# jgaeddert/liquid-usrp

Measured on AMD Instinct MI355X. Metric: complex Msamples/s through multichannelrx, higher is better.
Workload: dtype f32

## Files before the change

include/mcrx_hip.h:

```cpp
#ifndef MCRX_HIP_H
#define MCRX_HIP_H

#include <stddef.h>
#include <stdint.h>

#ifdef __cplusplus
extern "C" {
#endif

#define MCRX_OK          0
#define MCRX_EINVAL     -1
#define MCRX_ENOMEM     -2
#define MCRX_EHIP       -3
#define MCRX_EUNSUPP    -4
#define MCRX_EOVERFLOW  -5
#define MCRX_EBUSY      -6

#define MCRX_TILE 16

typedef struct mcrx_hip_s *mcrx_hip_t;

typedef struct {
    uint32_t struct_size;
    uint32_t max_payload_len;
    uint32_t max_frames;
    uint32_t payload_soft;
    uint32_t slab_blocks;
    uint32_t channel_first;
    uint32_t channel_count;
    uint32_t batch_samples;
    uint32_t single_channel;
    uint32_t serial;
    uint32_t chunk_blocks;
    uint32_t defer_samples;
    uint32_t front_end;
    uint32_t skip_framesyms;
    uint32_t worker_build;
    uint32_t acquisition;
    uint32_t scout_build;
    uint32_t conv_scratch;
    uint32_t input_format;
} mcrx_hip_config;

typedef struct {
    uint32_t channel;
    int32_t  header_valid;
    int32_t  payload_valid;
    uint32_t payload_len;
    uint8_t  header[8];
    float    evm, rssi, cfo;
    uint32_t mod_scheme, mod_bps, check, fec0, fec1;
    uint32_t num_framesyms;
    uint64_t end_sample;
    const uint8_t *payload;
    const float   *framesyms;
} mcrx_frame;

int  mcrx_hip_create(mcrx_hip_t *out, unsigned num_channels, unsigned M, unsigned cp_len,
                     unsigned taper_len, const unsigned char *p, const mcrx_hip_config *cfg);
int  mcrx_hip_destroy(mcrx_hip_t q);
int  mcrx_hip_reset(mcrx_hip_t q);
#define MCRX_POSITION_MAX (1ll << 48)
int  mcrx_hip_reset_at(mcrx_hip_t q, uint64_t chan_position);
unsigned mcrx_hip_num_channels(mcrx_hip_t q);

int  mcrx_hip_execute_host(mcrx_hip_t q, const float *iq, size_t nsamples);
int  mcrx_hip_execute_device(mcrx_hip_t q, const void *d_iq, size_t nsamples, void *stream);
int  mcrx_hip_execute_host_sc16(mcrx_hip_t q, const int16_t *iq, size_t nsamples);
int  mcrx_hip_execute_device_sc16(mcrx_hip_t q, const void *d_iq, size_t nsamples, void *stream);
unsigned mcrx_hip_input_format(mcrx_hip_t q);

int  mcrx_hip_flush(mcrx_hip_t q);
int  mcrx_hip_poll(mcrx_hip_t q);
int  mcrx_hip_discard(mcrx_hip_t q);
int  mcrx_hip_stream_wait(mcrx_hip_t q, void *stream);
uint64_t mcrx_hip_launches(mcrx_hip_t q);
unsigned mcrx_hip_history_tiles(mcrx_hip_t q);
int  mcrx_hip_stream_wait_launch(mcrx_hip_t q, uint64_t launch, void *stream);
int  mcrx_hip_spec_stats(mcrx_hip_t q, uint64_t *walked, uint64_t *adopted, int reset);
int  mcrx_hip_viterbi_stats(mcrx_hip_t q, uint64_t *frames, uint64_t *forward_repeats, uint64_t *traceback_repeats, int reset);
size_t mcrx_hip_frames_pending(mcrx_hip_t q);
int  mcrx_hip_next_frame(mcrx_hip_t q, mcrx_frame *out);
int  mcrx_hip_drain_count(mcrx_hip_t q, uint64_t *frames, uint64_t *valid, uint64_t *payload_bytes);
uint64_t mcrx_hip_frames_dropped(mcrx_hip_t q);

typedef struct {
    uint32_t struct_size;
    uint32_t nfft;
    uint32_t window;
} mcrx_hip_monitor_config;
int  mcrx_hip_monitor_enable(mcrx_hip_t q, const mcrx_hip_monitor_config *cfg);
int  mcrx_hip_monitor_disable(mcrx_hip_t q);
int  mcrx_hip_monitor_read(mcrx_hip_t q, double *level, float *peak, double *psd, uint64_t *nseg, uint64_t *nsamp, int reset);
unsigned mcrx_hip_monitor_nfft(mcrx_hip_t q);

int  mcrx_hip_channelize(mcrx_hip_t q, const void *d_iq, size_t nblocks, uint64_t first_sample,
                         const void *d_halo, void *d_out, unsigned groups, void *stream);
int  mcrx_hip_sync(mcrx_hip_t q, const void *d_chan, uint64_t first_sample, size_t nsamples, void *stream);

int  mcrx_hip_restart(mcrx_hip_t q, void *stream);

int  mcrx_hip_get_taps(mcrx_hip_t q, float *h, size_t n);
uint32_t mcrx_hip_nco_step(mcrx_hip_t q);
unsigned mcrx_hip_history_blocks(mcrx_hip_t q);
int  mcrx_hip_kernel_time_ms(mcrx_hip_t q, float *channelizer_ms, float *sync_ms);
#define MCRX_NKERNELS 5
int  mcrx_hip_kernel_stats(mcrx_hip_t q, double ms_total[MCRX_NKERNELS], uint64_t launches[MCRX_NKERNELS], int reset);
int  mcrx_hip_kernel_timing(mcrx_hip_t q, int on);

const char *mcrx_hip_last_error(void);

int  mcrx_hip_device(mcrx_hip_t q);
int  mcrx_hip_selftest_device_table(void);

typedef struct msresamp_hip_s *msresamp_hip_t;
int    msresamp_hip_create(msresamp_hip_t *out, float rate, float As);
int    msresamp_hip_destroy(msresamp_hip_t q);
int    msresamp_hip_reset(msresamp_hip_t q);
int    msresamp_hip_reset_at(msresamp_hip_t q, uint64_t input_position);
float  msresamp_hip_get_delay(msresamp_hip_t q);
size_t msresamp_hip_max_output(msresamp_hip_t q, size_t nin);
int    msresamp_hip_execute_device(msresamp_hip_t q, const void *d_in, size_t nin, void *d_out,
                                   size_t out_cap, size_t *nout, void *stream);
int      msresamp_hip_set_input_format(msresamp_hip_t q, unsigned format);
unsigned msresamp_hip_input_format(msresamp_hip_t q);
int      msresamp_hip_execute_device_sc16(msresamp_hip_t q, const void *d_in, size_t nin, void *d_out,
                                          size_t out_cap, size_t *nout, void *stream);
int      msresamp_hip_set_output_format(msresamp_hip_t q, unsigned format);
unsigned msresamp_hip_output_format(msresamp_hip_t q);
int      msresamp_hip_set_output_gain(msresamp_hip_t q, float gain);
float    msresamp_hip_output_gain(msresamp_hip_t q);
int      msresamp_hip_clipped(msresamp_hip_t q, uint64_t *samples, int reset);
int      msresamp_hip_time_first_stage(msresamp_hip_t q, int enable);
int      msresamp_hip_first_stage_ms(msresamp_hip_t q, float *ms);
const char *msresamp_hip_last_error(void);

typedef struct mcrx_hip_pfb2_s *mcrx_hip_pfb2_t;
int    mcrx_hip_pfb2_create(mcrx_hip_pfb2_t *out, unsigned num_channels, unsigned m, float As);
int    mcrx_hip_pfb2_destroy(mcrx_hip_pfb2_t q);
int    mcrx_hip_pfb2_get_taps(mcrx_hip_pfb2_t q, float *h, size_t n);
int    mcrx_hip_pfb2_analyze(mcrx_hip_pfb2_t q, const void *d_x, size_t lead_samples, size_t nsteps,
                             uint64_t first_step, void *d_out, void *stream);
const char *mcrx_hip_pfb2_last_error(void);

typedef struct mcrx_hip_pipeline_s *mcrx_hip_pipeline_t;
int      mcrx_hip_pipeline_unique_id(void *id128);
int      mcrx_hip_pipeline_create(mcrx_hip_pipeline_t *out, mcrx_hip_t rx, int rank, int world, const void *unique_id128,
                                  size_t sub_blocks, unsigned nbuf );
#define MCRX_STREAM_READY ((void *)(intptr_t)-1)
int      mcrx_hip_pipeline_push(mcrx_hip_pipeline_t p, const void *d_iq_sub, const void *d_halo, void *after_stream);
int      mcrx_hip_pipeline_push_host(mcrx_hip_pipeline_t p, const float *iq_with_halo);
int      mcrx_hip_pipeline_host_buffer(mcrx_hip_pipeline_t p, float **buf, size_t *nsamples);
int      mcrx_hip_pipeline_reset(mcrx_hip_pipeline_t p, int64_t extra_samples);
int      mcrx_hip_pipeline_comm_count(mcrx_hip_pipeline_t p);
int      mcrx_hip_pipeline_wait(mcrx_hip_pipeline_t p);
int      mcrx_hip_pipeline_time_exchange(mcrx_hip_pipeline_t p, int on);
int      mcrx_hip_pipeline_exchange_ms(mcrx_hip_pipeline_t p, double *total_ms, uint64_t *rounds, int reset);
uint64_t mcrx_hip_pipeline_bytes_sent_per_round(mcrx_hip_pipeline_t p);
int      mcrx_hip_pipeline_destroy(mcrx_hip_pipeline_t p);
const char *mcrx_hip_pipeline_last_error(void);

typedef struct mctx_hip_s *mctx_hip_t;
int    mctx_hip_create(mctx_hip_t *out, unsigned num_channels, unsigned M, unsigned cp_len,
                       unsigned taper_len, const unsigned char *p);
int    mctx_hip_destroy(mctx_hip_t q);
int      mctx_hip_set_output_format(mctx_hip_t q, unsigned format);
unsigned mctx_hip_output_format(mctx_hip_t q);
int      mctx_hip_clipped(mctx_hip_t q, uint64_t *samples, int reset);
int      mctx_hip_selftest_quantise(const float *in, int16_t *out, size_t n);
size_t mctx_hip_blocks_for(mctx_hip_t q, unsigned frames_per_channel, unsigned payload_len,
                           int mod, int fec0, int fec1);
int    mctx_hip_generate(mctx_hip_t q, void *d_iq, size_t nblocks, unsigned frames_per_channel,
                         unsigned payload_len, int mod, int fec0, int fec1, float gain, uint32_t seed,
                         uint8_t *hdr, uint8_t *pay, void *stream);
int    mctx_hip_generate_ragged(mctx_hip_t q, void *d_iq, size_t nblocks, unsigned max_frames, unsigned len_lo, unsigned len_hi,
                                unsigned gap_max, unsigned long_every, unsigned long_max, int mod, int fec0, int fec1,
                                float gain, uint32_t seed, uint32_t *count, uint8_t *hdr, uint32_t *len, uint8_t *pay,
                                uint64_t *start, void *stream);
typedef struct mctx_hip_traffic_s *mctx_hip_traffic_t;
int    mctx_hip_traffic_create(mctx_hip_t q, mctx_hip_traffic_t *out, unsigned ch_first, unsigned ch_count,
                               unsigned frames_per_channel, unsigned payload_len, int mod, int fec0, int fec1,
                               uint32_t seed, uint8_t *hdr, uint8_t *pay, void *stream);
int    mctx_hip_traffic_destroy(mctx_hip_traffic_t t);
int    mctx_hip_traffic_tiles(mctx_hip_traffic_t t, long long first_block, size_t nblocks, void *d_tiles, void *stream);
int    mctx_hip_synthesize_tiles(mctx_hip_t q, const void *d_tiles, unsigned groups, long long first_block,
                                 size_t nblocks, size_t lead_blocks, size_t keep_blocks, float gain, void *d_iq,
                                 void *stream);
size_t mctx_hip_frame_len(mctx_hip_t q, unsigned payload_len, int mod, int fec0, int fec1);
int    mctx_hip_frame(mctx_hip_t q, const uint8_t *header8, const uint8_t *payload, unsigned payload_len,
                      int mod, int fec0, int fec1, float gain, float *out, size_t out_cap_samples);
int    mctx_hip_stream_begin(mctx_hip_t q, unsigned max_payload_len);
int    mctx_hip_stream_ready(mctx_hip_t q, unsigned channel);
int    mctx_hip_stream_update(mctx_hip_t q, unsigned channel, const uint8_t *header8, const uint8_t *payload,
                              unsigned payload_len, int mod, int fec0, int fec1);
// ... 187 lines not shown
```

liquid-usrp_amd/__init__.py:

```python
import ctypes as C
import math
import os
import subprocess

import numpy as np

_HERE = os.path.dirname(os.path.abspath(__file__))
_LIBPATH = os.environ.get("MCRX_LIB") or os.path.join(_HERE, "lib", "libmcrx_hip.so")

MCRX_OK, MCRX_EINVAL, MCRX_ENOMEM, MCRX_EHIP, MCRX_EUNSUPP, MCRX_EOVERFLOW, MCRX_EBUSY = 0, -1, -2, -3, -4, -5, -6
TILE = 16
POSITION_MAX = 1 << 48
TX_TILE = 8

LIQUID_CRC_NONE, LIQUID_CRC_32 = 1, 6
LIQUID_FEC_NONE, LIQUID_FEC_HAMMING128, LIQUID_FEC_GOLAY2412, LIQUID_FEC_CONV_V27 = 1, 6, 7, 11
LIQUID_FEC_REP3, LIQUID_FEC_REP5, LIQUID_FEC_HAMMING74, LIQUID_FEC_HAMMING84 = 2, 3, 4, 5
LIQUID_MODEM_QAM16, LIQUID_MODEM_QAM64, LIQUID_MODEM_BPSK, LIQUID_MODEM_QPSK = 27, 29, 39, 40


def build(force=False):
    src = os.path.join(_HERE, "csrc")
    deps = [os.path.join(src, f) for f in os.listdir(src) if f.endswith((".hip", ".h", ".hpp"))]
    deps.append(os.path.join(_HERE, "..", "include", "mcrx_hip.h"))
    stale = (not os.path.exists(_LIBPATH)) or any(os.path.getmtime(d) > os.path.getmtime(_LIBPATH) for d in deps)
    if force or stale:
        subprocess.check_call(["make", "-C", src, "-s", "-j4"])
    return _LIBPATH


class Config(C.Structure):
    _fields_ = [("struct_size", C.c_uint32), ("max_payload_len", C.c_uint32), ("max_frames", C.c_uint32),
                ("payload_soft", C.c_uint32), ("slab_blocks", C.c_uint32), ("channel_first", C.c_uint32),
                ("channel_count", C.c_uint32), ("batch_samples", C.c_uint32), ("single_channel", C.c_uint32),
                ("serial", C.c_uint32), ("chunk_blocks", C.c_uint32), ("defer_samples", C.c_uint32), ("front_end", C.c_uint32), ("skip_framesyms", C.c_uint32),
                ("worker_build", C.c_uint32), ("acquisition", C.c_uint32), ("scout_build", C.c_uint32), ("conv_scratch", C.c_uint32),
                ("input_format", C.c_uint32)]


INPUT_FORMATS = {"cf32": 0, "sc16": 1}
OUTPUT_FORMATS = {"cf32": 0, "sc16": 1}


class FrameC(C.Structure):
    _fields_ = [("channel", C.c_uint32), ("header_valid", C.c_int32), ("payload_valid", C.c_int32),
                ("payload_len", C.c_uint32), ("header", C.c_uint8 * 8),
                ("evm", C.c_float), ("rssi", C.c_float), ("cfo", C.c_float),
                ("mod_scheme", C.c_uint32), ("mod_bps", C.c_uint32), ("check", C.c_uint32),
                ("fec0", C.c_uint32), ("fec1", C.c_uint32), ("num_framesyms", C.c_uint32),
                ("end_sample", C.c_uint64), ("payload", C.c_void_p), ("framesyms", C.c_void_p)]


_EXPORTS = {
    "mcrx_hip_create": (C.c_int, [C.POINTER(C.c_void_p), C.c_uint, C.c_uint, C.c_uint, C.c_uint, C.c_void_p, C.c_void_p]),
    "mcrx_hip_destroy": (C.c_int, [C.c_void_p]),
    "mcrx_hip_reset": (C.c_int, [C.c_void_p]),
    "mcrx_hip_reset_at": (C.c_int, [C.c_void_p, C.c_uint64]),
    "mcrx_hip_num_channels": (C.c_uint, [C.c_void_p]),
    "mcrx_hip_execute_host": (C.c_int, [C.c_void_p, C.c_void_p, C.c_size_t]),
    "mcrx_hip_execute_device": (C.c_int, [C.c_void_p, C.c_void_p, C.c_size_t, C.c_void_p]),
    "mcrx_hip_execute_host_sc16": (C.c_int, [C.c_void_p, C.c_void_p, C.c_size_t]),
    "mcrx_hip_execute_device_sc16": (C.c_int, [C.c_void_p, C.c_void_p, C.c_size_t, C.c_void_p]),
    "mcrx_hip_input_format": (C.c_uint, [C.c_void_p]),
    "mcrx_hip_flush": (C.c_int, [C.c_void_p]),
    "mcrx_hip_poll": (C.c_int, [C.c_void_p]),
    "mcrx_hip_discard": (C.c_int, [C.c_void_p]),
    "mcrx_hip_stream_wait": (C.c_int, [C.c_void_p, C.c_void_p]),
    "mcrx_hip_launches": (C.c_uint64, [C.c_void_p]),
    "mcrx_hip_history_tiles": (C.c_uint, [C.c_void_p]),
    "mcrx_hip_stream_wait_launch": (C.c_int, [C.c_void_p, C.c_uint64, C.c_void_p]),
    "mcrx_hip_spec_stats": (C.c_int, [C.c_void_p, C.POINTER(C.c_uint64), C.POINTER(C.c_uint64), C.c_int]),
    "mcrx_hip_viterbi_stats": (C.c_int, [C.c_void_p, C.POINTER(C.c_uint64), C.POINTER(C.c_uint64), C.POINTER(C.c_uint64), C.c_int]),
    "mcrx_hip_frames_pending": (C.c_size_t, [C.c_void_p]),
    "mcrx_hip_next_frame": (C.c_int, [C.c_void_p, C.POINTER(FrameC)]),
    "mcrx_hip_drain_count": (C.c_int, [C.c_void_p, C.POINTER(C.c_uint64), C.POINTER(C.c_uint64), C.POINTER(C.c_uint64)]),
    "mcrx_hip_frames_dropped": (C.c_uint64, [C.c_void_p]),
    "mcrx_hip_channelize": (C.c_int, [C.c_void_p, C.c_void_p, C.c_size_t, C.c_uint64, C.c_void_p, C.c_void_p, C.c_uint, C.c_void_p]),
    "mcrx_hip_sync": (C.c_int, [C.c_void_p, C.c_void_p, C.c_uint64, C.c_size_t, C.c_void_p]),
    "mcrx_hip_restart": (C.c_int, [C.c_void_p, C.c_void_p]),
    "mcrx_hip_get_taps": (C.c_int, [C.c_void_p, C.c_void_p, C.c_size_t]),
    "mcrx_hip_nco_step": (C.c_uint32, [C.c_void_p]),
    "mcrx_hip_history_blocks": (C.c_uint, [C.c_void_p]),
    "mcrx_hip_device": (C.c_int, [C.c_void_p]),
    "mcrx_hip_selftest_device_table": (C.c_int, []),
    "mcrx_hip_kernel_time_ms": (C.c_int, [C.c_void_p, C.POINTER(C.c_float), C.POINTER(C.c_float)]),
    "mcrx_hip_kernel_stats": (C.c_int, [C.c_void_p, C.POINTER(C.c_double), C.POINTER(C.c_uint64), C.c_int]),
    "mcrx_hip_kernel_timing": (C.c_int, [C.c_void_p, C.c_int]),
    "mcrx_hip_monitor_enable": (C.c_int, [C.c_void_p, C.c_void_p]),
    "mcrx_hip_monitor_disable": (C.c_int, [C.c_void_p]),
    "mcrx_hip_monitor_read": (C.c_int, [C.c_void_p, C.c_void_p, C.c_void_p, C.c_void_p, C.POINTER(C.c_uint64), C.POINTER(C.c_uint64), C.c_int]),
    "mcrx_hip_monitor_nfft": (C.c_uint, [C.c_void_p]),
    "mcrx_hip_last_error": (C.c_char_p, []),
    "msresamp_hip_create": (C.c_int, [C.POINTER(C.c_void_p), C.c_float, C.c_float]),
    "msresamp_hip_destroy": (C.c_int, [C.c_void_p]),
    "msresamp_hip_reset": (C.c_int, [C.c_void_p]),
    "msresamp_hip_reset_at": (C.c_int, [C.c_void_p, C.c_uint64]),
    "msresamp_hip_get_delay": (C.c_float, [C.c_void_p]),
    "msresamp_hip_max_output": (C.c_size_t, [C.c_void_p, C.c_size_t]),
    "msresamp_hip_execute_device": (C.c_int, [C.c_void_p, C.c_void_p, C.c_size_t, C.c_void_p, C.c_size_t,
                                              C.POINTER(C.c_size_t), C.c_void_p]),
    "msresamp_hip_set_input_format": (C.c_int, [C.c_void_p, C.c_uint]),
    "msresamp_hip_input_format": (C.c_uint, [C.c_void_p]),
    "msresamp_hip_execute_device_sc16": (C.c_int, [C.c_void_p, C.c_void_p, C.c_size_t, C.c_void_p, C.c_size_t,
                                                   C.POINTER(C.c_size_t), C.c_void_p]),
    "msresamp_hip_set_output_format": (C.c_int, [C.c_void_p, C.c_uint]),
    "msresamp_hip_output_format": (C.c_uint, [C.c_void_p]),
    "msresamp_hip_set_output_gain": (C.c_int, [C.c_void_p, C.c_float]),
    "msresamp_hip_output_gain": (C.c_float, [C.c_void_p]),
    "msresamp_hip_clipped": (C.c_int, [C.c_void_p, C.POINTER(C.c_uint64), C.c_int]),
    "msresamp_hip_time_first_stage": (C.c_int, [C.c_void_p, C.c_int]),
    "msresamp_hip_first_stage_ms": (C.c_int, [C.c_void_p, C.POINTER(C.c_float)]),
    "msresamp_hip_last_error": (C.c_char_p, []),
    "mcrx_hip_pfb2_create": (C.c_int, [C.POINTER(C.c_void_p), C.c_uint, C.c_uint, C.c_float]),
    "mcrx_hip_pfb2_destroy": (C.c_int, [C.c_void_p]),
    "mcrx_hip_pfb2_get_taps": (C.c_int, [C.c_void_p, C.c_void_p, C.c_size_t]),
    "mcrx_hip_pfb2_analyze": (C.c_int, [C.c_void_p, C.c_void_p, C.c_size_t, C.c_size_t, C.c_uint64, C.c_void_p, C.c_void_p]),
    "mcrx_hip_pfb2_last_error": (C.c_char_p, []),
    "mcrx_hip_pipeline_unique_id": (C.c_int, [C.c_void_p]),
    "mcrx_hip_pipeline_create": (C.c_int, [C.POINTER(C.c_void_p), C.c_void_p, C.c_int, C.c_int, C.c_void_p, C.c_size_t, C.c_uint]),
    "mcrx_hip_pipeline_push": (C.c_int, [C.c_void_p, C.c_void_p, C.c_void_p, C.c_void_p]),
    "mcrx_hip_pipeline_push_host": (C.c_int, [C.c_void_p, C.c_void_p]),
    "mcrx_hip_pipeline_wait": (C.c_int, [C.c_void_p]),
    "mcrx_hip_pipeline_host_buffer": (C.c_int, [C.c_void_p, C.POINTER(C.c_void_p), C.POINTER(C.c_size_t)]),
    "mcrx_hip_pipeline_reset": (C.c_int, [C.c_void_p, C.c_int64]),
    "mcrx_hip_pipeline_comm_count": (C.c_int, [C.c_void_p]),
    "mcrx_hip_pipeline_time_exchange": (C.c_int, [C.c_void_p, C.c_int]),
    "mcrx_hip_pipeline_exchange_ms": (C.c_int, [C.c_void_p, C.POINTER(C.c_double), C.POINTER(C.c_uint64), C.c_int]),
    "mcrx_hip_pipeline_bytes_sent_per_round": (C.c_uint64, [C.c_void_p]),
    "mcrx_hip_pipeline_destroy": (C.c_int, [C.c_void_p]),
    "mcrx_hip_pipeline_last_error": (C.c_char_p, []),
    "mctx_hip_create": (C.c_int, [C.POINTER(C.c_void_p), C.c_uint, C.c_uint, C.c_uint, C.c_uint, C.c_void_p]),
    "mctx_hip_destroy": (C.c_int, [C.c_void_p]),
    "mctx_hip_set_output_format": (C.c_int, [C.c_void_p, C.c_uint]),
    "mctx_hip_output_format": (C.c_uint, [C.c_void_p]),
    "mctx_hip_clipped": (C.c_int, [C.c_void_p, C.POINTER(C.c_uint64), C.c_int]),
    "mctx_hip_selftest_quantise": (C.c_int, [C.c_void_p, C.c_void_p, C.c_size_t]),
    "mctx_hip_blocks_for": (C.c_size_t, [C.c_void_p, C.c_uint, C.c_uint, C.c_int, C.c_int, C.c_int]),
    "mctx_hip_generate_ragged": (C.c_int, [C.c_void_p, C.c_void_p, C.c_size_t, C.c_uint, C.c_uint, C.c_uint, C.c_uint, C.c_uint, C.c_uint,
                                           C.c_int, C.c_int, C.c_int, C.c_float, C.c_uint32, C.c_void_p, C.c_void_p, C.c_void_p,
                                           C.c_void_p, C.c_void_p, C.c_void_p]),
    "mctx_hip_generate": (C.c_int, [C.c_void_p, C.c_void_p, C.c_size_t, C.c_uint, C.c_uint, C.c_int, C.c_int, C.c_int,
                                    C.c_float, C.c_uint32, C.c_void_p, C.c_void_p, C.c_void_p]),
    "mctx_hip_traffic_create": (C.c_int, [C.c_void_p, C.POINTER(C.c_void_p), C.c_uint, C.c_uint, C.c_uint, C.c_uint, C.c_int, C.c_int,
                                          C.c_int, C.c_uint32, C.c_void_p, C.c_void_p, C.c_void_p]),
    "mctx_hip_traffic_destroy": (C.c_int, [C.c_void_p]),
    "mctx_hip_traffic_tiles": (C.c_int, [C.c_void_p, C.c_longlong, C.c_size_t, C.c_void_p, C.c_void_p]),
    "mctx_hip_synthesize_tiles": (C.c_int, [C.c_void_p, C.c_void_p, C.c_uint, C.c_longlong, C.c_size_t, C.c_size_t, C.c_size_t,
                                            C.c_float, C.c_void_p, C.c_void_p]),
    "mctx_hip_frame_len": (C.c_size_t, [C.c_void_p, C.c_uint, C.c_int, C.c_int, C.c_int]),
    "mctx_hip_frame": (C.c_int, [C.c_void_p, C.c_void_p, C.c_void_p, C.c_uint, C.c_int, C.c_int, C.c_int, C.c_float,
                                 C.c_void_p, C.c_size_t]),
    "mctx_hip_stream_begin": (C.c_int, [C.c_void_p, C.c_uint]),
    "mctx_hip_stream_ready": (C.c_int, [C.c_void_p, C.c_uint]),
    "mctx_hip_stream_update": (C.c_int, [C.c_void_p, C.c_uint, C.c_void_p, C.c_void_p, C.c_uint, C.c_int, C.c_int, C.c_int]),
    "mctx_hip_stream_generate": (C.c_int, [C.c_void_p, C.c_void_p]),
    "mctx_hip_stream_reset": (C.c_int, [C.c_void_p]),
    "mctx_hip_last_error": (C.c_char_p, []),
    "mcrx_hip_chanemu_create": (C.c_int, [C.POINTER(C.c_void_p), C.c_void_p]),
    "mcrx_hip_chanemu_destroy": (C.c_int, [C.c_void_p]),
    "mcrx_hip_chanemu_reset": (C.c_int, [C.c_void_p]),
    "mcrx_hip_chanemu_reset_at": (C.c_int, [C.c_void_p, C.c_uint64]),
    "mcrx_hip_chanemu_position": (C.c_uint64, [C.c_void_p]),
    "mcrx_hip_chanemu_output_format": (C.c_uint, [C.c_void_p]),
    "mcrx_hip_chanemu_execute_device": (C.c_int, [C.c_void_p, C.c_void_p, C.c_size_t, C.c_void_p, C.c_void_p]),
    "mcrx_hip_chanemu_clipped": (C.c_int, [C.c_void_p, C.POINTER(C.c_uint64), C.c_int]),
    "mcrx_hip_chanemu_selftest_words": (C.c_int, [C.c_uint64, C.c_uint64, C.POINTER(C.c_uint32)]),
    "mcrx_hip_chanemu_last_error": (C.c_char_p, []),
    "mcrx_hip_chanfade_set": (C.c_int, [C.c_void_p, C.c_void_p]),
    "mcrx_hip_chanfade_on": (C.c_int, [C.c_void_p]),
    "mcrx_hip_chanfade_gains": (C.c_int, [C.c_void_p, C.c_uint64, C.c_uint32, C.c_void_p, C.c_void_p]),
    "mcrx_hip_chanfade_selftest": (C.c_int, [C.c_void_p, C.c_uint, C.POINTER(C.c_int64), C.POINTER(C.c_uint32), C.POINTER(C.c_float)]),
    "mcrx_hip_userchan_create": (C.c_int, [C.POINTER(C.c_void_p), C.c_uint, C.c_void_p, C.c_size_t]),
    "mcrx_hip_userchan_destroy": (C.c_int, [C.c_void_p]),
    "mcrx_hip_userchan_num_channels": (C.c_uint, [C.c_void_p]),
    "mcrx_hip_userchan_lead_blocks": (C.c_uint, [C.c_void_p]),
    "mcrx_hip_userchan_apply_tiles": (C.c_int, [C.c_void_p, C.c_void_p, C.c_longlong, C.c_size_t, C.c_size_t, C.c_void_p, C.c_void_p]),
    "mcrx_hip_userchan_last_error": (C.c_char_p, []),
    "mcrx_hip_userfade_set": (C.c_int, [C.c_void_p, C.c_void_p, C.c_void_p]),
    "mcrx_hip_userfade_on": (C.c_int, [C.c_void_p]),
    "mcrx_hip_userfade_selftest": (C.c_int, [C.c_void_p, C.c_void_p, C.c_uint, C.POINTER(C.c_int64), C.POINTER(C.c_uint32),
                                             C.POINTER(C.c_float)]),
    "mcrx_hip_userfade_gains": (C.c_int, [C.c_void_p, C.c_longlong, C.c_uint32, C.c_void_p, C.c_void_p]),
    "mcrx_hip_userclock_set": (C.c_int, [C.c_void_p, C.c_void_p, C.c_void_p]),
    "mcrx_hip_userclock_on": (C.c_int, [C.c_void_p]),
    "mcrx_hip_userclock_lead_blocks": (C.c_uint, [C.c_void_p]),
    "mcrx_hip_userclock_selftest": (C.c_int, [C.c_void_p, C.c_void_p, C.c_longlong, C.POINTER(C.c_int64), C.POINTER(C.c_float)]),
    "mcrx_hip_userclock_table": (C.c_int, [C.POINTER(C.c_float)]),
    "mcrx_hip_userclock_apply_tiles": (C.c_int, [C.c_void_p, C.c_void_p, C.c_longlong, C.c_size_t, C.c_size_t, C.c_void_p, C.c_void_p]),
    "mcrx_hip_rfchain_create": (C.c_int, [C.POINTER(C.c_void_p), C.c_void_p]),
    "mcrx_hip_rfchain_destroy": (C.c_int, [C.c_void_p]),
# ... 12 lines not shown
    "mcrx_hip_rfcal_update": (C.c_int, [C.c_void_p, C.c_void_p]),
    "mcrx_hip_rfcal_hold": (C.c_int, [C.c_void_p, C.c_int]),
    "mcrx_hip_rfcal_set": (C.c_int, [C.c_void_p, C.c_float, C.c_float, C.c_float, C.c_float, C.c_void_p]),
    "mcrx_hip_rfcal_read": (C.c_int, [C.c_void_p, C.c_void_p, C.c_void_p]),
    "mcrx_hip_rfcal_clipped": (C.c_int, [C.c_void_p, C.POINTER(C.c_uint64), C.c_int]),
    "mcrx_hip_rfcal_selftest": (C.c_int, [C.c_void_p, C.c_uint64, C.c_uint64, C.POINTER(C.c_uint64), C.POINTER(C.c_uint32), C.c_size_t,
                                          C.POINTER(C.c_uint64)]),
    "mcrx_hip_rfcal_last_error": (C.c_char_p, []),
    "mcrx_hip_cfr_create": (C.c_int, [C.POINTER(C.c_void_p), C.c_void_p]),
    "mcrx_hip_cfr_destroy": (C.c_int, [C.c_void_p]),
    "mcrx_hip_cfr_halo": (C.c_uint, [C.c_void_p]),
    "mcrx_hip_cfr_output_format": (C.c_uint, [C.c_void_p]),
    "mcrx_hip_cfr_execute_device": (C.c_int, [C.c_void_p, C.c_void_p, C.c_size_t, C.c_void_p, C.c_void_p]),
    "mcrx_hip_cfr_clipped": (C.c_int, [C.c_void_p, C.POINTER(C.c_uint64), C.c_int]),
    "mcrx_hip_cfr_stats": (C.c_int, [C.c_void_p, C.POINTER(C.c_uint64), C.POINTER(C.c_float), C.c_int]),
    "mcrx_hip_cfr_design": (C.c_int, [C.c_uint32, C.c_double, C.c_double, C.POINTER(C.c_float)]),
    "mcrx_hip_cfr_last_error": (C.c_char_p, []),
}

_lib = None


def exported_symbols():
    return sorted(_EXPORTS)


def lib():
    global _lib
    if _lib is None:
        if not os.path.exists(_LIBPATH):
            raise RuntimeError("libmcrx_hip.so is not built (run __graft_entry__.build()); "
                               "liquid_usrp_amd has no CPU fallback")
        try:
            import torch
        except ImportError:
            pass
        L = C.CDLL(_LIBPATH)
        for name, (res, args) in _EXPORTS.items():
            fn = getattr(L, name)
            fn.restype, fn.argtypes = res, args
        _lib = L
    return _lib


class McrxError(RuntimeError):
    pass


def _check(rc, allow=()):
    if rc != MCRX_OK and rc not in allow:
        msg = lib().mcrx_hip_last_error()
        raise McrxError("mcrx_hip error %d: %s" % (rc, msg.decode() if msg else ""))
    return rc


def _raise_rc(rc, name, last_error, einval_is_value_error=True):
    if rc == MCRX_OK:
        return
    msg = last_error()
    msg = msg.decode() if msg else ""
    if rc == MCRX_EINVAL and einval_is_value_error:
        raise ValueError(msg)
    raise McrxError("%s failed (%d): %s" % (name, rc, msg))


def _format_code(value, table, what):
    code = table.get(value) if isinstance(value, str) else next((c for c in table.values() if c == value), None)
    if code is None:
        raise ValueError("%s must be one of %s or %s, not %r" % (what, sorted(table), sorted(table.values()), value))
    return code


def _empty_samples(n, fmt, device):
    import torch
    if fmt == OUTPUT_FORMATS["sc16"]:
        return torch.empty((n, 2), dtype=torch.int16, device=device)
    return torch.empty(n, dtype=torch.complex64, device=device)


def _sc16_device_samples(x, what):
    import torch
    if x.dtype != torch.int16:
        raise TypeError("this %s takes int16 device tensors (interleaved re, im), not %s" % (what, x.dtype))
    if not x.is_contiguous():
        raise ValueError("device samples must be contiguous")
    if x.numel() % 2:
        raise ValueError("an sc16 buffer holds (re, im) pairs: odd number of int16")
    return int(x.numel()) // 2


class Frame(object):
    __slots__ = ("channel", "header", "header_valid", "payload", "payload_valid", "evm", "rssi", "cfo",
                 "framesyms", "mod_scheme", "mod_bps", "check", "fec0", "fec1", "end_sample")

    def __repr__(self):
        return "Frame(ch=%d hv=%d pv=%d len=%d evm=%.2f end=%d)" % (
            self.channel, self.header_valid, self.payload_valid, len(self.payload), self.evm, self.end_sample)


def _dptr(t):
    if t is None:
        return None
    if isinstance(t, int):
        return C.c_void_p(t)
    return C.c_void_p(t.data_ptr())


def _stream_ptr(stream):
    if stream is None:
        return None
    if isinstance(stream, int):
        return C.c_void_p(stream)
    return C.c_void_p(stream.cuda_stream)


class MonitorConfig(C.Structure):
    _fields_ = [("struct_size", C.c_uint32), ("nfft", C.c_uint32), ("window", C.c_uint32)]


MONITOR_WINDOWS = {"rect": 0, "rectangular": 0, "hann": 1, "hamming": 2}


def monitor_omega(num_channels, nfft, channel, kp):
    N = float(num_channels)
    return np.pi * (np.asarray(channel, np.float64) - (N - 1.0) / 2.0) / N + 2.0 * np.pi * np.asarray(kp, np.float64) / (nfft * 2.0 * N)


class MonitorReading(object):

    def __init__(self, level, peak, psd, nseg, nsamp, num_channels, channel_first=0):
        self.level, self.peak, self.psd = np.asarray(level, np.float64), np.asarray(peak, np.float32), np.asarray(psd, np.float64)
        self.nseg, self.nsamp, self.N, self.channel_first = int(nseg), int(nsamp), int(num_channels), int(channel_first)

    def level_db(self):
        return 10.0 * np.log10(np.maximum(self.level, 1e-300))

    def occupied(self, threshold_db):
        return self.level_db() > threshold_db

    def wideband(self):
        nch, nfft = self.psd.shape
        kp = np.arange(-nfft // 2 + 1, nfft // 2 + 1)
        row = self.psd[:, kp % nfft].reshape(-1)
        ch = self.channel_first + np.arange(nch)
        return row, monitor_omega(self.N, nfft, ch[:, None], kp[None, :]).reshape(-1)


class multichannelrx(object):

    def __init__(self, num_channels, M, cp_len, taper_len, p=None, userdata=None, callback=None, **cfg):
        self._h = C.c_void_p()
        self.N, self.K, self.M, self.cp = num_channels, 2 * num_channels, M, cp_len
        parr = None if p is None else np.ascontiguousarray(np.frombuffer(bytes(bytearray(p)), np.uint8))
        c = Config()
        c.struct_size = C.sizeof(Config)
        c.payload_soft = 1
        for k, v in cfg.items():
            setattr(c, k, _format_code(v, INPUT_FORMATS, "input_format") if k == "input_format" else v)
        rc = lib().mcrx_hip_create(C.byref(self._h), num_channels, M, cp_len, taper_len,
                                   None if parr is None else parr.ctypes.data, C.addressof(c))
        if rc != MCRX_OK:
            self._h = C.c_void_p()
            _raise_rc(rc, "mcrx_hip_create", lib().mcrx_hip_last_error)
        self.userdata = list(userdata) if userdata is not None else [None] * num_channels
        self.callback = list(callback) if callback is not None else [None] * num_channels
        self.frames = []
        self.channel_first = int(c.channel_first)
        self.nch = int(c.channel_count) if c.channel_count else num_channels - self.channel_first
        self.input_format = int(c.input_format)

    def GetNumChannels(self):
        return self.N

    def Execute(self, x, num_samples=None, stream=None):
        sc16 = self.input_format == INPUT_FORMATS["sc16"]
        if hasattr(x, "is_cuda") and x.is_cuda:
            import torch
            if sc16:
                n = _sc16_device_samples(x, "receiver")
                n = n if num_samples is None else int(num_samples)
                _check(lib().mcrx_hip_execute_device_sc16(self._h, _dptr(x), n, _stream_ptr(stream)))
                return
            if x.dtype == torch.int16:
                raise TypeError("int16 samples need a receiver made with input_format=\"sc16\"")
            n = int(x.numel()) if num_samples is None else int(num_samples)
            _check(lib().mcrx_hip_execute_device(self._h, _dptr(x), n, _stream_ptr(stream)))
            return
        if sc16:
            a = np.asarray(x)
            if a.dtype != np.int16:
                raise TypeError("this receiver takes int16 samples (interleaved re, im), not %s" % a.dtype)
            a = np.ascontiguousarray(a)
            if a.size % 2:
                raise ValueError("an sc16 buffer holds (re, im) pairs: odd number of int16")
            n = a.size // 2 if num_samples is None else int(num_samples)
            _check(lib().mcrx_hip_execute_host_sc16(self._h, a.ctypes.data, n), allow=(MCRX_EOVERFLOW,))
            self._deliver(flush=False)
            return
        if getattr(x, "dtype", None) == np.int16:
            raise TypeError("int16 samples need a receiver made with input_format=\"sc16\"")
        a = np.ascontiguousarray(x, np.complex64)
        n = a.size if num_samples is None else int(num_samples)
        _check(lib().mcrx_hip_execute_host(self._h, a.ctypes.data, n), allow=(MCRX_EOVERFLOW,))
        self._deliver(flush=False)

    def Reset(self):
        _check(lib().mcrx_hip_reset(self._h))
        self._deliver(flush=False)

    def reset_at(self, pos):
        rc = lib().mcrx_hip_reset_at(self._h, int(pos))
        if rc == MCRX_EINVAL:
            raise ValueError(lib().mcrx_hip_last_error().decode())
        _check(rc)
        self._deliver(flush=False)

    def Flush(self):
        rc = lib().mcrx_hip_flush(self._h)
        _check(rc, allow=(MCRX_EOVERFLOW,))
        self._deliver(flush=False)
        return rc

    def Poll(self, deliver=True):
        rc = lib().mcrx_hip_poll(self._h)
        _check(rc, allow=(MCRX_EOVERFLOW,))
        if deliver:
            self._deliver(flush=False)
        return rc

    def Discard(self):
        _check(lib().mcrx_hip_discard(self._h))

    def frames_pending(self):
        return int(lib().mcrx_hip_frames_pending(self._h))

    def drain_count(self):
        n, ok, nb = C.c_uint64(0), C.c_uint64(0), C.c_uint64(0)
        _check(lib().mcrx_hip_drain_count(self._h, C.byref(n), C.byref(ok), C.byref(nb)))
        return int(n.value), int(ok.value), int(nb.value)

    def stream_wait(self, stream=None, launch=None):
        if launch is None:
            _check(lib().mcrx_hip_stream_wait(self._h, _stream_ptr(stream)))
        else:
            _check(lib().mcrx_hip_stream_wait_launch(self._h, launch, _stream_ptr(stream)))

    def spec_stats(self, reset=False):
        a, b = C.c_uint64(0), C.c_uint64(0)
        _check(lib().mcrx_hip_spec_stats(self._h, C.byref(a), C.byref(b), 1 if reset else 0))
        return int(a.value), int(b.value)

    def viterbi_stats(self, reset=False):
        a, b, c = C.c_uint64(0), C.c_uint64(0), C.c_uint64(0)
        _check(lib().mcrx_hip_viterbi_stats(self._h, C.byref(a), C.byref(b), C.byref(c), 1 if reset else 0))
        return int(a.value), int(b.value), int(c.value)

    def _deliver(self, flush):
        f = FrameC()
        while lib().mcrx_hip_next_frame(self._h, C.byref(f)) == 1:
            fr = Frame()
            fr.channel = int(f.channel)
            fr.header = bytes(bytearray(f.header))
            fr.header_valid, fr.payload_valid = int(f.header_valid), int(f.payload_valid)
            fr.payload = C.string_at(f.payload, f.payload_len) if f.payload and f.payload_len else b""
            fr.evm, fr.rssi, fr.cfo = float(f.evm), float(f.rssi), float(f.cfo)
            if f.framesyms and f.num_framesyms:
                buf = (C.c_float * (2 * f.num_framesyms)).from_address(f.framesyms)
                fr.framesyms = np.frombuffer(buf, np.float32).copy().view(np.complex64)
            else:
                fr.framesyms = np.zeros(0, np.complex64)
            fr.mod_scheme, fr.mod_bps = int(f.mod_scheme), int(f.mod_bps)
            fr.check, fr.fec0, fr.fec1 = int(f.check), int(f.fec0), int(f.fec1)
            fr.end_sample = int(f.end_sample)
            self.frames.append(fr)
            cb = self.callback[fr.channel] if fr.channel < len(self.callback) else None
            if cb is not None:
                cb(fr.header, fr.header_valid, fr.payload, len(fr.payload), fr.payload_valid, fr,
                   self.userdata[fr.channel])

    def taps(self):
        h = np.zeros(14 * self.K, np.float32)
        _check(lib().mcrx_hip_get_taps(self._h, h.ctypes.data, h.size))
        return h

    def nco_step(self):
        return int(lib().mcrx_hip_nco_step(self._h))

    def history_blocks(self):
        return int(lib().mcrx_hip_history_blocks(self._h))

    def channelize(self, d_iq, nblocks, first_sample, d_out, groups=1, d_halo=None, stream=None):
        _check(lib().mcrx_hip_channelize(self._h, _dptr(d_iq), nblocks, first_sample, _dptr(d_halo),
                                         _dptr(d_out), groups, _stream_ptr(stream)))

    def sync(self, d_chan, first_sample, nsamples, stream=None):
        _check(lib().mcrx_hip_sync(self._h, _dptr(d_chan), first_sample & 0xFFFFFFFFFFFFFFFF, nsamples, _stream_ptr(stream)))
        return int(lib().mcrx_hip_launches(self._h)) - 1

    @property
    def hist_tiles(self):
        return int(lib().mcrx_hip_history_tiles(self._h))

    def restart(self, stream=None):
        _check(lib().mcrx_hip_restart(self._h, _stream_ptr(stream)))

    def kernel_time_ms(self):
        a, b = C.c_float(0), C.c_float(0)
        _check(lib().mcrx_hip_kernel_time_ms(self._h, C.byref(a), C.byref(b)))
# ... 1261 lines not shown
```

liquid-usrp_amd/csrc/kernels.h:

```cpp
#pragma once
#include <hip/hip_runtime.h>
#include <stdint.h>
#include "acq_shared.h"
#include "sync_plan.hpp"

namespace mcrx {

#define MCRX_TILE_S 16
#define MCRX_TILE_SH 4
#define MCRX_HDR_ENC 36
#define MCRX_HDR_DEC 14

struct ChanArgs {
    const void *x;
    const void *halo;
    const float *taps;
    float2 *out;
    uint32_t nblocks;
    uint32_t slab_blocks;
    uint32_t first_sample_lo;
    uint32_t dtheta;
    uint32_t ntiles;
    uint32_t cg;
    uint32_t col_shift;
// ... 5 lines not shown
int channelizer_carries(unsigned K);
uint32_t channelizer_auto_slab(unsigned K, size_t nblocks, unsigned ncu);
hipError_t channelizer_launch(unsigned K, unsigned P, unsigned in_fmt, const ChanArgs &a, hipStream_t st);

#ifndef MCRX_S1_BACKOFF_CORRECTION
#define MCRX_S1_BACKOFF_CORRECTION 0
#endif
#ifndef MCRX_S1_METRIC_G0_NORMALISED
#define MCRX_S1_METRIC_G0_NORMALISED 1
#endif
enum { SY_SEEK = 0, SY_S0A, SY_S0B, SY_S1, SY_RX };
enum { FX_HEADER = 0, FX_PAYLOAD };

struct CodingDev {
    const uint32_t *crc_byte;
    const uint32_t *crc_zadv;
    const uint8_t *qam16_nb;
    const uint8_t *qam64_nb;
};

struct SyncConsts {
    int M, M2, cp, L, backoff, M_pilot, M_data, Nen, M_S0, M_S1;
    int E;
    int log2M;
    float detect_thresh, sync_thresh;
    const uint8_t *sctype;
    const float *S0, *S1;
    const float2 *s0t;
    const float *smk, *smn;
    float2 backoff_rot;
    const float *Pfit;
    const int16_t *data_rank, *pilot_rank, *en_rank;
    const uint8_t *pilot_seq;
    const uint16_t *hdr_map;
    const float2 *dft_tw;
    CodingDev cod;
    uint32_t max_payload_len, max_enc_len, max_syms;
    const uint32_t *crc_pos;
    uint32_t crc_pos_n;
    const uint32_t *il_off;
    const uint16_t *il_map;
    uint32_t il_n;
    int payload_soft;
};

struct ChanState {
    int32_t state; uint32_t timer;
    int64_t cur;
    uint32_t nco_theta_ref, nco_dtheta; int64_t nco_t_ref;
    float g0; float2 s_hat_0;
    uint32_t num_symbols, pilot_count;
    float phi_prime, p1_prime;
    int32_t fstate; uint32_t header_symbol_index, payload_symbol_index;
    float evm_hat, evm;
    uint32_t payload_len, mod_scheme, bps, check, fec0, fec1, enc_len, mod_len;
    int32_t header_valid;
    uint32_t hw[4];
    uint32_t period_hint;
    int64_t last_fresh;
    uint32_t burst_hint;
    uint32_t burst_pad;
};

struct FrameRec {
    uint32_t channel; int32_t header_valid, payload_valid; uint32_t payload_len;
    uint8_t header[8];
    float evm, rssi, cfo;
    uint32_t mod_scheme, mod_bps, check, fec0, fec1, num_framesyms;
    int64_t end_sample;
    uint64_t payload_off, syms_off;
};

struct PayloadJob {
    ChanState s;
    uint32_t ch;
    uint32_t pad;
    uint64_t arena_off;
    uint64_t syms_off;
};

struct SpecSlot {
    int64_t start;
    int64_t t_last;
    int32_t status;
    uint32_t pad;
};

struct SyncArgs {
    SyncConsts c;
    const float2 *chan;
    uint32_t chan_stride, chan_off;
    int64_t buf_first;
    int64_t end;
    uint32_t nch;
    uint32_t ch_first;
    ChanState *st;
    uint8_t *hbits;
    float2 *R;
    uint8_t *soft;
    uint8_t *tmpa, *tmpb;
    float2 *syms;
    FrameRec *rec; uint8_t *arena; uint8_t *sarena;
    uint32_t *nrec;
    unsigned long long *arena_used;
    uint64_t arena_cap, sarena_cap;
    uint32_t max_rec;
    int scout;
    PayloadJob *jobs; uint32_t *njobs; uint32_t max_jobs;
    uint32_t *gen_list;
    uint32_t dec_lds_soft;
    uint32_t *njobs_next;
    float2 *jR;
    uint8_t *jsoft;
    uint8_t *jtmp;
    int debug;
    uint2 *vit_scratch;
    uint32_t vit_rows, vit_waves;
    uint32_t *vit_passes;
    uint32_t *qam_list;
    uint32_t *qam_next;
    uint32_t *live, *live_next;
    uint32_t frames_hint;
    uint32_t live_off;
    uint32_t *list_hint;
    uint32_t grid_hint[3];
    uint32_t payload_lds_pad;
    int seek_burst;
    SpecSlot *spec; float2 *spec_R;
    int64_t *pred; uint32_t *pred_n;
    uint32_t spec_cap;
    uint32_t spec_stride;
    uint32_t nseg;
    uint32_t seg_jobs;
    int no_syms;
    int split_rest;
    int dec_phase;
    int seg_walker;
    int seg_phase;
    int64_t *anchor;
    int64_t *seekst;
    uint32_t *spec_hint;
    uint32_t *walk_hint;
    uint32_t *hint;
    uint32_t enc_hint;
    int round_idx;
    int burst_limit;
    int stop_after_walk;
    int64_t defer_limit;
    int tail_only;
    uint32_t *stats;
    int no_fast;
    int payload_fr, payload_lean, payload_xb;
    uint32_t vit_off;
};
hipError_t sync_launch(const SyncArgs &a, hipStream_t st);
hipError_t sync_launch_tail(const SyncArgs &a, hipStream_t st);
hipError_t ilmap_build_launch(const uint32_t *d_lens, const uint32_t *d_offs, uint32_t nlen, uint8_t *d_lo, uint8_t *d_hi, uint16_t *d_map, hipStream_t st);
hipError_t sync_launch_walk(const SyncArgs &a, hipStream_t st);
hipError_t sync_launch_lean(const SyncArgs &a, hipStream_t st);
int acq_lean_waves(const SyncConsts &c);
hipError_t sync_launch_spec(const SyncArgs &a, hipStream_t st);
hipError_t sync_launch_payload(const SyncArgs &a, SyncStage stage, hipStream_t st);
bool sync_payload_splits(const SyncArgs &a);
hipError_t sync_reset_launch(ChanState *st, uint32_t nch, int64_t cur, float2 *hist0, float2 *hist1, size_t hist_n,
                             uint32_t *nrec, unsigned long long *arena_used, uint32_t *pred_n, hipStream_t stream);

struct MonArgs {
    const float2 *chan;
    uint32_t stride, off, t0, ntiles;
    uint32_t nch, nfft, window;
    uint32_t carry_len, carry_cap;
    const float2 *carry_in; float2 *carry_out;
    uint32_t nsplit;
    double *part_psd, *part_level; float *part_peak;
    double *psd, *level; float *peak;
};
hipError_t monitor_launch(const MonArgs &a, hipStream_t st);

}
```

liquid-usrp_amd/csrc/mcrx_hip.hip:

```cpp
#include "../../include/mcrx_hip.h"
#include "acq_plan.hpp"
#include "config_read.hpp"
#include "design.hpp"
#include "devel.h"
#include "devmath.h"
#include "devscope.hpp"
#include "kernels.h"
#include "rx_plan.hpp"
#include "sc16.hpp"
#include "txcode.hpp"

#include <algorithm>
#include <chrono>
#include <cstdio>
#include <cstdlib>
#include <cstring>
#include <mutex>
#include <string>
#include <vector>

using namespace mcrx;

#define MCRX_GENS 4

static thread_local std::string g_err;
static void set_err(const char *what, hipError_t e, const char *file, int line)
{
    char buf[512];
    snprintf(buf, sizeof(buf), "%s: %s (%s:%d)", what, hipGetErrorString(e), file, line);
    g_err = buf;
}
static int fail(int code, const char *msg) { g_err = msg; return code; }
#define HIPCHK(x) do { hipError_t e_ = (x); if (e_ != hipSuccess) { set_err(#x, e_, __FILE__, __LINE__); return MCRX_EHIP; } } while (0)
#define RC(x) do { int rc_ = (x); if (rc_ != MCRX_OK) return rc_; } while (0)

extern "C" const char *mcrx_hip_last_error(void) { return g_err.c_str(); }

static std::mutex g_cod_mu;
static bool g_cod_ready = false;
static CodingDev g_cod;

template <class T> static int upload_raw(T **dst, const T *src, size_t n)
{
    HIPCHK(hipMalloc((void **)dst, std::max<size_t>(n, 1) * sizeof(T)));
    if (n) HIPCHK(hipMemcpy(*dst, src, n * sizeof(T), hipMemcpyHostToDevice));
    return MCRX_OK;
}
static int coding_tables(CodingDev *out)
{
    std::lock_guard<std::mutex> lk(g_cod_mu);
    if (!g_cod_ready) {
        CodingTables *t = new CodingTables();
        uint8_t *f, *g; uint32_t *d, *e;
        RC(upload_raw(&d, t->crc_byte, 256));
        RC(upload_raw(&e, &t->crc_zadv[0][0][0], 16 * 4 * 256));
        RC(upload_raw(&f, &t->qam16_nb[0][0], 64));
        RC(upload_raw(&g, &t->qam64_nb[0][0], 256));
        g_cod.crc_byte = d; g_cod.crc_zadv = e;
        g_cod.qam16_nb = f; g_cod.qam64_nb = g;
        delete t;
        g_cod_ready = true;
    }
    *out = g_cod;
    return MCRX_OK;
}

template <class T>
__global__ void hist_update_kernel(const T *old_hist, const T *x, uint64_t nx, T *new_hist, uint64_t nh)
{
    uint64_t i = (uint64_t)blockIdx.x * blockDim.x + threadIdx.x;
    if (i >= nh) return;
    uint64_t pos = nx + i;
    new_hist[i] = (pos < nh) ? old_hist[pos] : x[pos - nh];
}

__global__ void nco_mix_kernel(const float2 *x, float2 *y, uint64_t n, uint32_t first_lo, uint32_t dtheta)
{
    const uint64_t i = (uint64_t)blockIdx.x * blockDim.x + threadIdx.x;
    if (i >= n) return;
    y[i] = mix_down_hw(x[i], (first_lo + (uint32_t)i) * dtheta);
}
__global__ void halfband_adapter_kernel(const float2 *Y, uint32_t M, uint32_t N, uint32_t ntiles, const float *h1, float2 *out)
{
    const uint32_t c = blockIdx.x * blockDim.x + threadIdx.x, tile = blockIdx.y;
    if (c >= N || tile >= ntiles) return;
    float h[14];
#pragma unroll
    for (int i = 0; i < 14; i++) h[i] = h1[i];
    constexpr int TS = MCRX_TILE_S;
    const long long k0 = (long long)tile * TS;
    float2 ev[13 + TS];
#pragma unroll
    for (int i = 0; i < 13 + TS; i++) ev[i] = Y[(2 * (k0 - 13 + i)) * (long long)M + c];
    float4 *dst = reinterpret_cast<float4 *>(out + ((size_t)tile * N + c) * TS);
    float2 y[TS];
#pragma unroll
    for (int t = 0; t < TS; t++) {
        float2 acc = make_float2(0.f, 0.f);
#pragma unroll
        for (int i = 0; i < 14; i++) { acc.x += h[i] * ev[t + i].x; acc.y += h[i] * ev[t + i].y; }
        const float2 d = Y[(2 * (k0 + t) - 13) * (long long)M + c];
        y[t] = make_float2(0.5f * (d.x + acc.x), 0.5f * (d.y + acc.y));
    }
#pragma unroll
    for (int t = 0; t < TS; t += 2) dst[t / 2] = make_float4(y[t].x, y[t].y, y[t + 1].x, y[t + 1].y);
}

struct HostArena {
    uint8_t *p = nullptr; size_t size = 0, cap = 0;
    int grow_to(size_t n)
    {
        if (n <= cap) { size = n; return MCRX_OK; }
        size_t ncap = std::max<size_t>(n, cap + cap / 2);
        uint8_t *np = nullptr;
        if (hipHostMalloc((void **)&np, ncap, hipHostMallocDefault) != hipSuccess) return MCRX_ENOMEM;
        if (size) memcpy(np, p, size);
        if (p) (void)hipHostFree(p);
        p = np; cap = ncap; size = n;
        return MCRX_OK;
    }
    void clear() { size = 0; }
    void release() { if (p) (void)hipHostFree(p); p = nullptr; size = cap = 0; }
};

struct mcrx_hip_s : RxPlan {
    int device = -1;
    unsigned N = 0, M = 0, cp = 0, taper = 0;
    OfdmDesign od;
    mcrx_hip_config cfg{};
    std::vector<float> taps;
    uint32_t dtheta = 0, ncu = 256;
    const float *d_taps = nullptr;
    SyncConsts sc{};
    std::vector<void *> owned; std::vector<hipEvent_t> owned_events; std::vector<hipStream_t> owned_streams;
    ChanState *d_st = nullptr; uint8_t *d_hbits = nullptr; float2 *d_R = nullptr;
    uint8_t *d_soft = nullptr, *d_tmpa = nullptr, *d_tmpb = nullptr; float2 *d_syms = nullptr;
    FrameRec *d_rec[MCRX_GENS] = {}; uint8_t *d_arena[MCRX_GENS] = {}, *d_sarena[MCRX_GENS] = {};
    uint32_t *d_nrec[MCRX_GENS] = {}; unsigned long long *d_arena_used[MCRX_GENS] = {};
    int gen = 0; bool gen_used[MCRX_GENS] = {}, gen_closed[MCRX_GENS] = {}, gen_abandoned[MCRX_GENS] = {};
    int debug = 0, no_fast = 0, seek_burst = 1; bool free_run = false;
    hipStream_t acq_stream = nullptr;
    uint64_t gen_close_seq[MCRX_GENS] = {}, close_counter = 0;
    hipEvent_t ev_gen[MCRX_GENS] = {};
    hipEvent_t ev_clean[MCRX_GENS] = {};
    bool clean_pending[MCRX_GENS] = {};
    PayloadJob *d_jobs[MCRX_SLOTS] = {}; uint32_t *d_njobs = nullptr; float2 *d_jR[MCRX_SLOTS] = {};
    uint32_t *d_gen[MCRX_SLOTS] = {}, *d_qam[MCRX_SLOTS] = {}, *d_live[MCRX_SLOTS] = {};
    uint2 *d_vit_scratch = nullptr; uint32_t *d_vit_passes = nullptr;
    uint64_t seq = 0;
    uint32_t *d_stats = nullptr;
    hipStream_t s_scout = nullptr, s_work = nullptr, s_copy = nullptr;
    hipStream_t s_side = nullptr; hipEvent_t ev_side[MCRX_SLOTS] = {}, ev_side_last = nullptr; bool side_last = false;

    hipEvent_t ev_ready[MCRX_SLOTS] = {}, ev_scout[MCRX_SLOTS] = {}, ev_done[MCRX_SLOTS] = {}, ev_in = nullptr, ev_consumed = nullptr, ev_tmp[4] = {};
    int last_slot = -1; size_t last_ntiles = 0;
    bool carried = false; uint64_t carried_seq = 0;
    uint32_t spec_stride = MCRX_SPEC_MAX;
    SpecSlot *d_spec = nullptr; float2 *d_spec_R = nullptr; int64_t *d_anchor = nullptr, *d_seekst = nullptr;
    uint32_t *h_hint = nullptr, *d_hint = nullptr;
    uint8_t *d_jsoft[MCRX_SLOTS] = {}, *d_jtmp[MCRX_SLOTS] = {};
    bool scout_tables = true, il_tried = false;
    bool acq_prio = true;
    AcqPolicy acq;
    uint64_t total_samples = 0;
    uint64_t stage_first = 0;
    int64_t chan_samples = 0;
    char *d_hist[2] = { nullptr, nullptr }; int hist_cur = 0;
    char *d_in = nullptr;
    char *h_stage = nullptr; size_t stage_fill = 0;
    float2 *d_chan[MCRX_SLOTS] = {}; size_t chan_cap_tiles = 0;
    mcrx_hip_pfb2_t pfb2 = nullptr; const float *d_h1 = nullptr;
    float2 *d_pfin[2] = { nullptr, nullptr }, *d_pfout[2] = { nullptr, nullptr }; size_t pf_cap_blocks = 0; int pf_cur = 0;
    uint64_t pf_in_valid = 0, pf_steps = 0; size_t pf_last_blocks = 0; bool pf_have_last = false;
    hipStream_t stream = nullptr;
    char *d_direct[2] = { nullptr, nullptr }; size_t direct_cap = 0; int direct_idx = 0; bool direct_used[2] = { false, false };
    hipStream_t copy_stream = nullptr; hipEvent_t ev_dcopy[2] = { nullptr, nullptr }, ev_ddone[2] = { nullptr, nullptr };
    uint64_t pending_bound = 0;
    uint64_t drain_touch = 0;
    double t_copy = 0, t_harvest = 0, t_run = 0, t_wait = 0, t_d2h = 0, b_d2h = 0, t_grow = 0, t_cnt = 0, t_post = 0;
    std::vector<hipEvent_t> evring[MCRX_NKERNELS];
    size_t ev_used[MCRX_NKERNELS] = {};
    double ev_ms_total[MCRX_NKERNELS] = {}; uint64_t ev_count[MCRX_NKERNELS] = {};
    float ev_last[MCRX_NKERNELS] = {};

    bool ev_on = false;
    hipEvent_t ev_base = nullptr; bool ev_dump = false;
    int ev_begin(int which, hipStream_t st)
    {
        if (!ev_on) return MCRX_OK;
        if (ev_dump && !ev_base) { RC(new_event(&ev_base, hipEventDefault)); HIPCHK(hipEventRecord(ev_base, st)); }
        if (ev_used[which] + 2 > evring[which].size()) RC(ev_resolve(which, evring[which].size() / 2));
        HIPCHK(hipEventRecord(evring[which][ev_used[which]], st));
        return MCRX_OK;
    }
    int ev_end(int which, hipStream_t st)
    {
        if (!ev_on) return MCRX_OK;
        HIPCHK(hipEventRecord(evring[which][ev_used[which] + 1], st));
        ev_used[which] += 2;
        return MCRX_OK;
    }
    int ev_resolve(int which, size_t upto = ~(size_t)0)
    {
        const size_t n = std::min(upto & ~(size_t)1, ev_used[which]);
        for (size_t i = 0; i < n; i += 2) {
            float ms = 0;
            HIPCHK(hipEventSynchronize(evring[which][i + 1]));
            HIPCHK(hipEventElapsedTime(&ms, evring[which][i], evring[which][i + 1]));
            if (ev_dump && ev_base) {
                float t0 = 0;
                if (hipEventElapsedTime(&t0, ev_base, evring[which][i]) == hipSuccess) fprintf(stderr, "[evt] %d %.1f %.1f\n", which, t0 * 1e3f, (t0 + ms) * 1e3f);
                else (void)hipGetLastError();
            }
            ev_ms_total[which] += ms; ev_count[which]++; ev_last[which] = ms;
        }
        std::rotate(evring[which].begin(), evring[which].begin() + n, evring[which].end());
        ev_used[which] -= n;
        return MCRX_OK;
    }
    struct Monitor {
        bool on = false, allocated = false, clear_pending = false, used = false;
        uint32_t nfft = 0, window = 0, max_split = 1;
        double wss = 1.0;
        float2 *d_carry[2] = { nullptr, nullptr }; int carry_cur = 0; uint32_t carry_len = 0;
        double *d_sums = nullptr;
        size_t sums_bytes = 0;
        double *d_part = nullptr;
        int64_t next = 0, origin = 0;
        uint64_t nseg = 0, nsamp = 0;
        hipStream_t s_mon = nullptr; hipEvent_t ev_in = nullptr, ev_out = nullptr, ev_last = nullptr;
    } mon;
    std::vector<FrameRec> recs; HostArena arena_host, sarena_host; size_t next_frame = 0;
    uint64_t dropped = 0;

    template <class T> int upload(const T **dst, const T *src, size_t n)
    {
        T *p = nullptr;
        RC(upload_raw(&p, src, n));
        owned.push_back(p); *dst = p;
        return MCRX_OK;
    }
    template <class T> int alloc_raw(T **dst, size_t n)
    {
        HIPCHK(hipMalloc((void **)dst, std::max<size_t>(n, 1) * sizeof(T)));
        owned.push_back(*dst);
        return MCRX_OK;
    }
    template <class T> int alloc(T **dst, size_t n)
    {
        HIPCHK(hipMalloc((void **)dst, std::max<size_t>(n, 1) * sizeof(T)));
        HIPCHK(hipMemset(*dst, 0, std::max<size_t>(n, 1) * sizeof(T)));
        owned.push_back(*dst);
        return MCRX_OK;
    }
    int new_event(hipEvent_t *e, unsigned flags)
    {
        HIPCHK(hipEventCreateWithFlags(e, flags));
        owned_events.push_back(*e);
        return MCRX_OK;
    }
    int new_stream(hipStream_t *st, unsigned flags = hipStreamDefault, const int *prio = nullptr)
    {
        HIPCHK(prio ? hipStreamCreateWithPriority(st, flags, *prio) : flags ? hipStreamCreateWithFlags(st, flags) : hipStreamCreate(st));
        owned_streams.push_back(*st);
        return MCRX_OK;
    }
};

static unsigned pow2ceil(unsigned v) { unsigned p = 1; while (p < v) p <<= 1; return p; }

struct IlShared { int dev; uint32_t max_payload, cap; uint16_t *d_map; uint32_t *d_off; uint32_t n; int refs; };
static std::mutex g_il_mu;
static std::vector<IlShared> g_il;

static int il_tables_acquire(uint32_t max_payload, uint32_t max_enc, const uint16_t **map, const uint32_t **off, uint32_t *n, hipStream_t st)
{
    *map = nullptr; *off = nullptr; *n = 0;
    int dev = 0;
    HIPCHK(hipGetDevice(&dev));
    const uint32_t cap = std::min<uint32_t>(max_enc, 56u * 1024u / 8u);
    auto find_shared = [&]() -> bool {
        for (auto &t : g_il)
            if (t.dev == dev && t.max_payload == max_payload && t.cap == cap) { t.refs++; *map = t.d_map; *off = t.d_off; *n = t.n; return true; }
        return false;
    };
    { std::lock_guard<std::mutex> lk(g_il_mu); if (find_shared()) return MCRX_OK; }
    std::vector<uint32_t> offv(cap + 1, ~0u), lens, offs;
    uint64_t total = 0;
    static const int outer[3] = { FEC_HAMMING128, FEC_GOLAY2412, FEC_CONV_V27 };
    for (int oc = 0; oc < 3; oc++)
        for (uint32_t np = 0; np <= max_payload; np++) {
            const uint32_t e = packet_enc_len(np, CRC_32, FEC_NONE, outer[oc]);
            if (e == 0 || e > cap || offv[e] != ~0u || e >= 65536u) continue;
            offv[e] = (uint32_t)total; lens.push_back(e); offs.push_back((uint32_t)total); total += e;
        }
    if (lens.empty() || total * 8 >= (1ull << 32)) return MCRX_OK;
    uint16_t *d_map = nullptr; uint8_t *d_lo = nullptr, *d_hi = nullptr; uint32_t *d_lens = nullptr, *d_offs = nullptr, *d_off = nullptr;
    hipError_t e = hipSuccess;
    auto step = [&](hipError_t r) { if (e == hipSuccess) e = r; return e == hipSuccess; };
    if (step(hipMalloc((void **)&d_map, (size_t)total * 8 * sizeof(uint16_t))) &&
        step(hipMalloc((void **)&d_lo, (size_t)total * 8)) && step(hipMalloc((void **)&d_hi, (size_t)total * 8)) &&
// ... 354 lines not shown
    if (q->h_stage) (void)hipHostFree(q->h_stage);
    if (q->h_hint) (void)hipHostFree(q->h_hint);
    q->arena_host.release(); q->sarena_host.release();
    for (hipEvent_t e : q->owned_events) (void)hipEventDestroy(e);
    for (size_t i = q->owned_streams.size(); i-- > 0;) (void)hipStreamDestroy(q->owned_streams[i]);
    delete q;
    return MCRX_OK;
}

extern "C" unsigned mcrx_hip_num_channels(mcrx_hip_t q) { return q ? q->N : 0; }
extern "C" unsigned mcrx_hip_input_format(mcrx_hip_t q) { return q ? q->in_fmt : 0; }
extern "C" uint32_t mcrx_hip_nco_step(mcrx_hip_t q) { return q ? q->dtheta : 0; }
extern "C" unsigned mcrx_hip_history_blocks(mcrx_hip_t q) { return q ? q->hist_blocks : 0; }
extern "C" int mcrx_hip_get_taps(mcrx_hip_t q, float *h, size_t n)
{
    if (!q || !h || n < q->taps.size()) return fail(MCRX_EINVAL, "taps buffer too small");
    memcpy(h, q->taps.data(), q->taps.size() * sizeof(float));
    return MCRX_OK;
}

static int launch_channelizer(mcrx_hip_t q, const void *x, size_t nblocks, uint64_t first_sample,
                              const void *halo, float2 *out, unsigned groups, size_t ntiles_stride, hipStream_t st,
                              float2 *out2 = nullptr, size_t out2_first_tile = 0, void *hist_out = nullptr)
{
    if (nblocks == 0) return MCRX_OK;
    if (nblocks % MCRX_TILE) return fail(MCRX_EINVAL, "nblocks must be a multiple of MCRX_TILE (16)");
    if (groups == 0 || q->N % groups) return fail(MCRX_EINVAL, "groups must divide the channel count");
    ChanArgs a;
    a.x = x; a.halo = halo; a.taps = q->d_taps; a.out = out;
    a.nblocks = (uint32_t)nblocks;
    a.slab_blocks = q->slab_blocks ? q->slab_blocks : channelizer_auto_slab(q->K, nblocks, q->ncu);
    a.first_sample_lo = (uint32_t)first_sample; a.dtheta = q->dtheta;
    a.ntiles = (uint32_t)ntiles_stride; a.cg = q->N / groups; a.col_shift = q->col_shift;
    if (out2 && groups != 1) return fail(MCRX_EINVAL, "a second copy of the last tiles needs a one-group launch");
    a.out2 = out2; a.out2_first = (uint32_t)(out2_first_tile * a.cg * (MCRX_TILE / 2)); a.hist_out = hist_out;
    RC(q->ev_begin(0, st));
    HIPCHK(channelizer_launch(q->K, q->chan_P, q->in_fmt, a, st));
    RC(q->ev_end(0, st));
    return MCRX_OK;
}
static int sync_lazy_allocs(mcrx_hip_t q, const AcqPlan &plan)
{
    if (!q->il_tried) {
        q->il_tried = true;
        if (q->scout_tables && devel_env("MCRX_NO_ILMAP") == nullptr &&
            il_tables_acquire(q->max_payload, q->max_enc, &q->sc.il_map, &q->sc.il_off, &q->sc.il_n, q->stream) != MCRX_OK) {
            (void)hipGetLastError();
            q->sc.il_map = nullptr; q->sc.il_off = nullptr; q->sc.il_n = 0;
            if (q->debug) fprintf(stderr, "[mcrx] de-interleaver gather tables not built (%s): decoding without them\n", mcrx_hip_last_error());
        }
    }
    if (!q->d_vit_scratch && q->vit_mode == 0 && q->vit_rows && plan.want_k7) {
        const size_t vit_bytes = (size_t)q->vit_waves * q->vit_rows * 64 * sizeof(uint2);
        if (hipMalloc((void **)&q->d_vit_scratch, vit_bytes) != hipSuccess) {
            (void)hipGetLastError(); q->d_vit_scratch = nullptr; q->vit_mode = 2;
            if (q->debug) fprintf(stderr, "[mcrx] the K = 7 decoder's scratch (%zu MB) could not be allocated: the block decoder stays\n", vit_bytes >> 20);
        } else q->owned.push_back(q->d_vit_scratch);
    }
    if (plan.spec_stride > q->spec_stride) {
        uint32_t ns = q->spec_stride; while (ns < plan.spec_stride) ns *= 2;
        SpecSlot *nb = nullptr;
        HIPCHK(hipDeviceSynchronize());
        RC(q->alloc(&nb, (size_t)q->nch * ns));
        q->d_spec = nb; q->spec_stride = ns;
    }
    return MCRX_OK;
}

static SyncArgs sync_args(mcrx_hip_t q, const float2 *chan, unsigned stride, unsigned off, int64_t buf_first, int64_t end, const AcqPlan &plan)
{
    const unsigned slot = (unsigned)(q->seq % q->nslots), next = (unsigned)((q->seq + 1) % q->nslots);
    const int g = q->gen;
    SyncArgs a{};
    a.c = q->sc; a.chan = chan; a.chan_stride = stride; a.chan_off = off;
    a.buf_first = buf_first; a.end = end; a.nch = q->nch; a.ch_first = q->ch_first;
    a.st = q->d_st; a.hbits = q->d_hbits; a.R = q->d_R; a.soft = q->d_soft; a.tmpa = q->d_tmpa; a.tmpb = q->d_tmpb;
    a.syms = q->d_syms; a.rec = q->d_rec[g]; a.arena = q->d_arena[g]; a.sarena = q->d_sarena[g];
    a.nrec = q->d_nrec[g]; a.arena_used = q->d_arena_used[g];
    a.arena_cap = q->arena_cap; a.sarena_cap = q->sarena_cap; a.max_rec = q->max_rec;
    a.debug = q->debug; a.no_fast = q->no_fast; a.seek_burst = q->seek_burst;
    a.payload_fr = q->payload_fr; a.payload_lean = q->payload_lean; a.payload_xb = q->payload_xb;
    a.payload_lds_pad = q->acq_mode == 2 ? q->walk_lds_pad : q->round_lds_pad;
    a.scout = q->scout ? 1 : 0;
    a.jobs = q->d_jobs[slot]; a.njobs = q->d_njobs + slot; a.njobs_next = q->d_njobs + next; a.max_jobs = q->max_jobs;
    a.gen_list = q->d_gen[slot];
    a.vit_scratch = q->d_vit_scratch; a.vit_rows = q->vit_rows; a.vit_waves = q->vit_waves; a.vit_passes = q->d_vit_passes;
    a.qam_list = q->d_qam[slot]; a.qam_next = q->d_qam[next];
    a.live = q->d_live[slot]; a.live_next = q->d_live[next];
    a.jR = q->d_jR[slot]; a.jsoft = q->d_jsoft[slot]; a.jtmp = q->d_jtmp[slot];
    a.stats = q->d_stats;
    a.hint = q->d_hint;
    if (q->h_hint && q->d_hint) a.list_hint = q->d_hint + HINT_LIST_BASE;
    a.frames_hint = plan.frames_hint; a.enc_hint = plan.enc_hint;
    for (int i = 0; i < 3; i++) a.grid_hint[i] = plan.grid_hint[i];
    a.spec = q->d_spec; a.spec_stride = q->spec_stride; a.spec_R = q->d_spec_R;
    a.seg_jobs = plan.seg_jobs; a.seekst = q->d_seekst; a.seg_walker = q->seg_walker;
    if (q->spec) { a.nseg = plan.nseg; a.spec_cap = plan.spec_cap; a.walk_hint = q->d_hint + HINT_WALK_BASE; a.anchor = q->d_anchor; }
    a.no_syms = q->cfg.skip_framesyms == 2 ? 1 : 0;
    a.defer_limit = (int64_t)q->defer;
    return a;
}

static int launch_acquisition(mcrx_hip_t q, SyncArgs &a, const AcqPlan &plan, hipStream_t st, hipStream_t sa)
{
    const unsigned slot = (unsigned)(q->seq % q->nslots), next = (unsigned)((q->seq + 1) % q->nslots);
    const int g = q->gen;
    if (q->pipelined && q->scout) {
        HIPCHK(hipEventRecord(q->ev_ready[slot], st));
        HIPCHK(hipStreamWaitEvent(sa, q->ev_ready[slot], 0));
        if (q->seq + 1 >= q->nslots) HIPCHK(hipStreamWaitEvent(sa, q->ev_done[next], 0));
    }
    if (!q->scout) HIPCHK(hipMemsetAsync(a.njobs, 0, sizeof(uint32_t), sa));
    q->acq_stream = sa;
    if (q->clean_pending[g]) { HIPCHK(hipStreamWaitEvent(sa, q->ev_clean[g], 0)); q->clean_pending[g] = false; }
    RC(q->ev_begin(1, sa));
    if (q->spec) {
        SyncArgs t = a;
        t.tail_only = 1; t.spec_cap = 0; t.nseg = 0; t.seg_jobs = 1; t.walk_hint = nullptr; t.anchor = nullptr; t.stats = nullptr;
        HIPCHK(sync_launch_tail(t, sa));
        if (a.debug & 4) fprintf(stderr, "[host] launch %llu: %u segments per channel, %.1f frames per channel and push expected\n", (unsigned long long)q->seq, plan.nseg, q->acq.frames_per_push);
        for (int i = 0; i < plan.nphase; i++) { a.seg_phase = plan.phase[i].seg_phase; a.seg_jobs = plan.phase[i].seg_jobs; HIPCHK(sync_launch_spec(a, sa)); }
        a.seg_phase = 0; a.seg_jobs = plan.seg_jobs;
        if (q->lean_build == 1) HIPCHK(sync_launch_walk(a, sa)); else HIPCHK(sync_launch_lean(a, sa));
        HIPCHK(sync_launch_tail(t, sa));
    } else {
        HIPCHK(sync_launch(a, sa));
    }
    RC(q->ev_end(1, sa));
    return MCRX_OK;
}

static int launch_workers(mcrx_hip_t q, SyncArgs &a, hipStream_t sa, hipStream_t &sw)
{
    const unsigned slot = (unsigned)(q->seq % q->nslots);
    RC(q->ev_begin(2, sa));
    HIPCHK(sync_launch_payload(a, SYNC_PLACE, sa));
    RC(q->ev_end(2, sa));
    if (sw != sa) {
        HIPCHK(hipEventRecord(q->ev_scout[slot], sa));
        HIPCHK(hipStreamWaitEvent(sw, q->ev_scout[slot], 0));
    }
    const bool side = sw == q->s_work && q->s_side && q->h_hint && q->d_hint && q->seq >= 8;
    const bool split = side && q->acq.list_seen[0] == 0 && q->acq.list_seen[2] == 0 &&
                       a.frames_hint != ~0u && a.frames_hint < 2048u && sync_payload_splits(a);
    const bool gen_side = !split && side && q->acq.list_seen[2] != 0 && !devel_env("MCRX_NO_GEN_SIDE");
    hipStream_t sd = sw;
    if (split) { a.split_rest = 1; a.dec_phase = 1; sd = q->s_side; }
    else if (gen_side) sd = q->s_side;
    else if (q->side_last) HIPCHK(hipStreamWaitEvent(sw, q->ev_side_last, 0));
    RC(q->ev_begin(3, sw));
    HIPCHK(sync_launch_payload(a, SYNC_WORKERS, sw));
    RC(q->ev_end(3, sw));
    RC(q->ev_begin(4, sw));
    HIPCHK(sync_launch_payload(a, SYNC_DECODE, sw));
    if (split) {
        HIPCHK(hipEventRecord(q->ev_side[slot], sw));
        HIPCHK(hipStreamWaitEvent(sd, q->ev_side[slot], 0));
        HIPCHK(sync_launch_payload(a, SYNC_BEHIND, sd));
        a.dec_phase = 2;
        HIPCHK(sync_launch_payload(a, SYNC_DECODE, sd));
    } else if (gen_side) {
        HIPCHK(hipEventRecord(q->ev_side[slot], sw));
        HIPCHK(hipStreamWaitEvent(sd, q->ev_side[slot], 0));
    }
    HIPCHK(sync_launch_payload(a, SYNC_DECODE_GENERAL, sd));
    RC(q->ev_end(4, sd));
    if (split || gen_side) HIPCHK(hipEventRecord(q->ev_side_last, sd));
    q->side_last = split || gen_side;
    sw = sd;
    return MCRX_OK;
}

static int launch_sync(mcrx_hip_t q, const float2 *chan, unsigned stride, unsigned off, int64_t buf_first, int64_t end, hipStream_t st)
{
    const unsigned slot = (unsigned)(q->seq % q->nslots);
    const int g = q->gen;
    const bool own_streams = q->pipelined && q->scout;
    q->mon.used = false;
    if (q->mon.on) RC(launch_monitor(q, chan, stride, off, buf_first, end, st));
    if (own_streams && q->spec && q->seq >= q->nslots && slot == 0 && !q->free_run) HIPCHK(hipEventSynchronize(q->ev_done[slot]));
    const bool have_hints = q->h_hint && q->d_hint;
    uint32_t hints[HINT_WORDS] = {};
    if (have_hints) for (int i = 0; i < HINT_WORDS; i++) hints[i] = ((volatile uint32_t *)q->h_hint)[i];
    const AcqInputs in = { (uint64_t)(end - buf_first), q->hist_tiles, q->nch, q->max_jobs, q->acq_mode, q->seg_walker,
                           q->seg_walker ? 0 : acq_lean_waves(q->sc), have_hints, q->spec };
    const AcqPlan plan = acq_plan(q->acq, hints, in);
    RC(sync_lazy_allocs(q, plan));
    SyncArgs a = sync_args(q, chan, stride, off, buf_first, end, plan);
    hipStream_t sa = own_streams ? q->s_scout : st, sw = own_streams ? q->s_work : st;
    RC(launch_acquisition(q, a, plan, st, sa));
    if (q->scout) RC(launch_workers(q, a, sa, sw));
    if (q->mon.used) {
        HIPCHK(hipEventRecord(q->mon.ev_out, q->mon.s_mon));
        HIPCHK(hipStreamWaitEvent(sw, q->mon.ev_out, 0));
    }
    HIPCHK(hipEventRecord(q->ev_done[slot], sw));
    HIPCHK(hipEventRecord(q->ev_gen[g], sw));
    q->gen_used[g] = true;
    q->seq++;
    return MCRX_OK;
}

extern "C" int mcrx_hip_channelize(mcrx_hip_t q, const void *d_iq, size_t nblocks, uint64_t first_sample,
                                   const void *d_halo, void *d_out, unsigned groups, void *stream)
{
    DevScope dev_scope_(q ? q->device : -1);
    if (q && q->bypass) return fail(MCRX_EUNSUPP, "single_channel handle has no channelizer");
    if (q && q->oversampled) return fail(MCRX_EUNSUPP, "front_end = 2 (the oversampled front end stage by stage) runs inside execute_host / execute_device only");
    if (!q || !d_iq || !d_out) return fail(MCRX_EINVAL, "null argument");
    hipStream_t st = stream ? (hipStream_t)stream : q->stream;
    return launch_channelizer(q, d_iq, nblocks, first_sample, d_halo,
                              (float2 *)d_out, groups, nblocks / MCRX_TILE, st);
}
extern "C" int mcrx_hip_sync(mcrx_hip_t q, const void *d_chan, uint64_t first_sample, size_t nsamples, void *stream)
{
    DevScope dev_scope_(q ? q->device : -1);
    if (!q || !d_chan) return fail(MCRX_EINVAL, "null argument");
    if ((int64_t)first_sample + (int64_t)nsamples >= MCRX_POSITION_MAX) return fail(MCRX_EINVAL, "channel-rate positions must stay below MCRX_POSITION_MAX = 2^48");
    hipStream_t st = stream ? (hipStream_t)stream : q->stream;
    return launch_sync(q, (const float2 *)d_chan, q->nch, 0, (int64_t)first_sample, (int64_t)(first_sample + nsamples), st);
}
extern "C" int mcrx_hip_restart(mcrx_hip_t q, void *stream)
{
    DevScope dev_scope_(q ? q->device : -1);
    if (!q) return fail(MCRX_EINVAL, "null handle");
    return restart_async(q, stream ? (hipStream_t)stream : q->stream, true);
}
extern "C" int mcrx_hip_kernel_time_ms(mcrx_hip_t q, float *ch_ms, float *sy_ms)
{
    DevScope dev_scope_(q ? q->device : -1);
    if (!q) return fail(MCRX_EINVAL, "null handle");
    for (int w = 0; w < MCRX_NKERNELS; w++) RC(q->ev_resolve(w));
    if (ch_ms) *ch_ms = q->ev_last[0];
    if (sy_ms) *sy_ms = q->ev_last[1] + q->ev_last[2] + q->ev_last[3] + q->ev_last[4];
    return MCRX_OK;
}
extern "C" int mcrx_hip_kernel_stats(mcrx_hip_t q, double ms_total[MCRX_NKERNELS], uint64_t launches[MCRX_NKERNELS], int reset)
{
    DevScope dev_scope_(q ? q->device : -1);
    if (!q) return fail(MCRX_EINVAL, "null handle");
    for (int w = 0; w < MCRX_NKERNELS; w++) {
        RC(q->ev_resolve(w));
        if (ms_total) ms_total[w] = q->ev_ms_total[w];
        if (launches) launches[w] = q->ev_count[w];
        if (reset) { q->ev_ms_total[w] = 0; q->ev_count[w] = 0; }
    }
    return MCRX_OK;
}

extern "C" int mcrx_hip_kernel_timing(mcrx_hip_t q, int on)
{
    if (!q) return -1;
    const int was = q->ev_on ? 1 : 0;
    q->ev_on = on != 0;
    return was;
}

static int ensure_chan(mcrx_hip_t q, size_t tiles)
{
    if (tiles <= q->chan_cap_tiles) return MCRX_OK;
    HIPCHK(hipDeviceSynchronize());
    float2 *nb[MCRX_SLOTS] = {};
    const size_t n = tiles * (size_t)q->N * MCRX_TILE, tile_elems = (size_t)q->N * MCRX_TILE;
    for (unsigned i = 0; i < q->nslots; i++) {
        HIPCHK(hipMalloc((void **)&nb[i], n * sizeof(float2)));
        HIPCHK(hipMemset(nb[i], 0, n * sizeof(float2)));
    }
    if (q->last_slot >= 0)
        HIPCHK(hipMemcpy(nb[q->last_slot] + q->last_ntiles * tile_elems, q->d_chan[q->last_slot] + q->last_ntiles * tile_elems,
                         (size_t)q->hist_tiles * tile_elems * sizeof(float2), hipMemcpyDeviceToDevice));
    for (int i = 0; i < MCRX_SLOTS; i++) { if (q->d_chan[i]) (void)hipFree(q->d_chan[i]); q->d_chan[i] = nb[i]; }
    q->chan_cap_tiles = tiles;
    q->carried = false;
    return MCRX_OK;
}

static int run_oversampled(mcrx_hip_t q, const float2 *x, size_t nblocks, uint64_t first_abs, float2 *tiles, hipStream_t sc)
{
    const size_t M = q->K, N = q->N, lead = (size_t)28 * N, hsteps = 32, nsteps = 2 * nblocks, nin = nblocks * q->K;
    if (nblocks > q->pf_cap_blocks) {
        HIPCHK(hipDeviceSynchronize());
        float2 *ni[2] = { nullptr, nullptr }, *no[2] = { nullptr, nullptr };
        for (int i = 0; i < 2; i++) {
            HIPCHK(hipMalloc((void **)&ni[i], (lead + nblocks * q->K) * sizeof(float2)));
            HIPCHK(hipMalloc((void **)&no[i], (hsteps + 2 * nblocks) * M * sizeof(float2)));
            HIPCHK(hipMemset(ni[i], 0, lead * sizeof(float2)));
            HIPCHK(hipMemset(no[i], 0, hsteps * M * sizeof(float2)));
        }
        if (q->pf_have_last) {
            const int c = q->pf_cur;
            HIPCHK(hipMemcpy(ni[c] + q->pf_last_blocks * q->K, q->d_pfin[c] + q->pf_last_blocks * q->K, lead * sizeof(float2), hipMemcpyDeviceToDevice));
            HIPCHK(hipMemcpy(no[c] + 2 * q->pf_last_blocks * M, q->d_pfout[c] + 2 * q->pf_last_blocks * M, hsteps * M * sizeof(float2), hipMemcpyDeviceToDevice));
        }
        for (int i = 0; i < 2; i++) {
            if (q->d_pfin[i]) (void)hipFree(q->d_pfin[i]);
            if (q->d_pfout[i]) (void)hipFree(q->d_pfout[i]);
            q->d_pfin[i] = ni[i]; q->d_pfout[i] = no[i];
        }
        q->pf_cap_blocks = nblocks;
    }
    const int prev = q->pf_cur, cur = prev ^ 1;
    float2 *in = q->d_pfin[cur], *out = q->d_pfout[cur];
    if (q->pf_have_last) {
        HIPCHK(hipMemcpyAsync(in, q->d_pfin[prev] + q->pf_last_blocks * q->K, lead * sizeof(float2), hipMemcpyDeviceToDevice, sc));
        HIPCHK(hipMemcpyAsync(out, q->d_pfout[prev] + 2 * q->pf_last_blocks * M, hsteps * M * sizeof(float2), hipMemcpyDeviceToDevice, sc));
    } else {
// ... 544 lines not shown
```

liquid-usrp_amd/csrc/ofdmsync.hip:

```cpp
#include "devmath.h"
#include "kernels.h"
#include <utility>

namespace mcrx {

#define WV 64
#ifndef SY_PART
#define SY_PART -1
#endif
#ifndef SY_PROFILE
#define SY_PROFILE 0
#endif
#ifndef H128_EARLY_OUT
#define H128_EARLY_OUT 1
#endif
#ifndef SY_RANK
#define SY_RANK 1
#endif
#ifndef SY_SEG_BURST
#define SY_SEG_BURST 1
#endif
#define SY_PROF(a) (SY_PROFILE && ((a).debug & 2) != 0)
#ifdef MCRX_DEVEL
#define MCRX_DEVEL_ABLATE(a) ((unsigned)(a).debug >> 8 << 6)
// ... 2425 lines not shown
                    cur[e] = cadd(u, v); cur[e + J] = rot_down(csub(u, v), rev);
                }
            }
        }
#define SY_QSTAGE(ST, H)                                                                           \
        if constexpr (H < G) {                                                                     \
            _Pragma("unroll") for (int e = 0; e < E; e++) {                                        \
                const float sx = bfly_leg<H>(cur[e].x, sgc[ST]), sy = bfly_leg<H>(cur[e].y, sgc[ST]);  \
                if (H == 1) cur[e] = make_float2(sx, sy);                                          \
                else cur[e] = make_float2(sx * twc[ST].x - sy * twc[ST].y, sx * twc[ST].y + sy * twc[ST].x); \
            }                                                                                      \
        }
        SY_QSTAGE(0, 32) SY_QSTAGE(1, 16) SY_QSTAGE(2, 8) SY_QSTAGE(3, 4) SY_QSTAGE(4, 2) SY_QSTAGE(5, 1)
#undef SY_QSTAGE
#pragma unroll
        for (int e = 0; e < E; e++) {
            cur[e] = cmul(cur[e], R[e]);
            if (pr[e] >= 0) qpil[16 * g + pr[e]] = cur[e];
        }
        wave_sync_lds();
        float2 P = qpil[16 * g + (i < Mp ? i : 0)];
        uint32_t pi_ = pc + (uint32_t)(i < 16 ? i : 0); pi_ = pi_ >= 255u ? pi_ - 255u : pi_;
        const bool pneg = pseq[pi_ < 255u ? pi_ : 0u] == 0;
        wave_sync_lds();
        if (pneg) { P.x = -P.x; P.y = -P.y; }
        const float v = atan2_fast(P.y, P.x);
        const float prev = dpp_mov<0x111, false>(v, v);
        const float turns = rintf((v - prev) * 0.15915494309189535f);
        const float y = fmaf(-TWO_PI_F, row_scan_fast(turns), v);
        const float p0 = group_total(row_scan_fast(pf0 * y));
        float p1 = group_total(row_scan_fast(pf1 * y));
        pc += (uint32_t)Mp; pc = pc >= 255u ? pc - 255u : pc;
        p1 = 0.3f * p1 + (1.0f - 0.3f) * p1_prime;
        p1_prime = p1;
        const float p0r = p0 * 0.15915494309189535f;
        const bool full = (psi + (uint32_t)Md) * bps <= nbits;
        float2 Z[E];
#pragma unroll
        for (int e = 0; e < E; e++) Z[e] = rot_down(cur[e], fmaf(p1, fxr[e], p0r));
        unsigned long long pending = __ballot(live);
        while (pending) {
            const int src = __builtin_ctzll(pending);
            const uint32_t umod = (uint32_t)__builtin_amdgcn_readlane((int)mod, src), ubps = (uint32_t)__builtin_amdgcn_readlane((int)bps, src);
            const bool sel = live && mod == umod;
            pending &= ~__ballot(sel);
            const uint8_t *unbt = reinterpret_cast<const uint8_t *>(umod == 27 ? qnb16 : qnb64);
#pragma unroll
            for (int e = 0; e < E; e++) {
                const uint32_t idx = psi + (uint32_t)dr[e];
                const bool ok = sel && dr[e] >= 0 && idx < mod_len;
                uint8_t sb[6];
                const unsigned hs = demod_soft(unbt, umod, Z[e], sb);
                if (!soft_mode) {
#pragma unroll
                    for (int kb = 0; kb < 6; kb++) sb[kb] = (uint8_t)(((hs >> ((ubps - 1 - kb) & 7)) & 1) ? 255 : 0);
                }
                if (!ok) continue;
                syms[idx] = Z[e];
                uint8_t *dst = soft + (size_t)idx * ubps;
                if (full) {
                    if (ubps == 2)      *reinterpret_cast<uint16_t *>(dst) = (uint16_t)(sb[0] | (sb[1] << 8));
                    else if (ubps == 1) dst[0] = sb[0];
                    else {
                        *reinterpret_cast<uint16_t *>(dst) = (uint16_t)(sb[0] | (sb[1] << 8));
                        *reinterpret_cast<uint16_t *>(dst + 2) = (uint16_t)(sb[2] | (sb[3] << 8));
                        if (ubps == 6) *reinterpret_cast<uint16_t *>(dst + 4) = (uint16_t)(sb[4] | (sb[5] << 8));
                    }
                } else {
                    for (unsigned kb = 0; kb < ubps; kb++) if (idx * ubps + kb < nbits) dst[kb] = sb[kb];
                }
            }
        }
        psi += (uint32_t)Md;
        float dphi = p0 - phi_prime;
        dphi -= TWO_PI_F * rintf(dphi * 0.15915494309189535f);
        phi_prime = p0;
        const uint32_t dnew = dth + uni((uint32_t)__float2int_rn(dphi * (1e-3f * 683565275.5764316f)));
        th_ws += (uint32_t)(L - cb) * dth + (uint32_t)cb * dnew;
        if (live) dth = dnew;
        r_ws += L;
#pragma unroll
        for (int e = 0; e < E; e++) cur[e] = nxt[e];
    }
    if (i == 0 && active) a.jobs[j].s.nco_dtheta = dth;
}

#include "payload_lean.hpp"

#ifndef DK_FUSED
#define DK_FUSED 1
#endif
#ifndef DK_NT_LOAD
#define DK_NT_LOAD 1
#endif
extern __shared__ __attribute__((aligned(16))) unsigned long long dk_soft[];
#define DKP(e) ((e) ^ (((e) >> 5) & 31u))
__device__ __forceinline__ unsigned il_cols_below(unsigned s0, unsigned len, unsigned Ncol, unsigned rem)
{
    auto span = [&](unsigned a0, unsigned b0) { const unsigned lo = a0 < rem ? a0 : rem, hi = b0 < rem ? b0 : rem; return hi - lo; };
    return (s0 + len <= Ncol) ? span(s0, s0 + len) : span(s0, Ncol) + span(0u, s0 + len - Ncol);
}
__device__ __forceinline__ void divmod_small(unsigned a, unsigned b, unsigned &q, unsigned &r)
{
    q = (unsigned)((float)a * __builtin_amdgcn_rcpf((float)b));
    int rr = (int)a - (int)(q * b);
    if (rr < 0) { q--; rr += (int)b; }
    if (rr >= (int)b) { q++; rr -= (int)b; }
    r = (unsigned)rr;
}
__device__ void il_pass_lds(unsigned n, unsigned Mi, unsigned Ncol, unsigned mask, unsigned dummy)
{
    const unsigned n2 = n / 2, c0 = n / 3;
    unsigned long long m64 = 0;
#pragma unroll
    for (int k = 0; k < 8; k++) if ((mask >> (7 - k)) & 1) m64 |= 0xFFull << (8 * k);
    unsigned R, rem, cnt0 = 0, t0, s1, c0r;
    divmod_small(n2, Ncol, R, rem);
    if (c0 < n2) divmod_small(n2 - c0 + Ncol - 1, Ncol, cnt0, t0);
    divmod_small(c0, Ncol, t0, c0r);
    s1 = c0r + 1; s1 -= s1 >= Ncol ? Ncol : 0u;
    const unsigned sa = s1 < rem ? rem - s1 : 0u, sb = Ncol - (s1 > rem ? s1 : rem), sw = rem < s1 ? rem : s1;
    const unsigned B1 = sa * (R + 1), B2 = B1 + sb * R, B3 = B2 + sw * (R + 1);
    constexpr int UN = 4;
    for (unsigned i0 = threadIdx.x; i0 < n2; i0 += UN * DK_T) {
        unsigned ea[UN], eb[UN];
        unsigned long long va[UN], vb[UN];
#pragma unroll
        for (int u = 0; u < UN; u++) {
            const unsigned i = i0 + u * DK_T;
            const unsigned ip = i - cnt0;
            const bool g1 = ip < B1, g2 = ip < B2, g3 = ip < B3;
            unsigned d = (g1 || (!g2 && g3)) ? R + 1 : R;
            d = d ? d : 1u;
            const unsigned off = g1 ? ip : g2 ? ip - B1 : g3 ? ip - B2 : ip - B3;
            const unsigned lbase = g1 ? 0u : g2 ? sa : g3 ? sa + sb : sa + sb + sw;
            unsigned q, m; divmod_small(off, d, q, m);
            const unsigned len = lbase + q;
            unsigned cm = s1 + len; cm -= cm >= Ncol ? Ncol : 0u;
            const bool first = i < cnt0;
            const unsigned j = first ? i * Ncol + c0 : m * Ncol + cm;
            const bool ok = i < n2 && j < n2 && (first || (len < Ncol && m < Mi));
            ea[u] = ok ? DKP(2 * i) : dummy;
            eb[u] = ok ? DKP(2 * j + 1) : dummy;
            va[u] = dk_soft[ea[u]]; vb[u] = dk_soft[eb[u]];
        }
#pragma unroll
        for (int u = 0; u < UN; u++) {
            dk_soft[ea[u]] = (va[u] & ~m64) | (vb[u] & m64);
            dk_soft[eb[u]] = (vb[u] & ~m64) | (va[u] & m64);
        }
    }
    __syncthreads();
}
__device__ uint32_t crc32_tree(const CodingDev cod, uint32_t tab_off, uint32_t msg_off, uint32_t n)
{
    const uint32_t *lds_tab = reinterpret_cast<const uint32_t *>(reinterpret_cast<const uint8_t *>(dk_soft) + tab_off);
    const uint8_t *p = reinterpret_cast<const uint8_t *>(dk_soft) + msg_off;
    const int r = lane_id();
    uint32_t C = 1, lc = 0;
    while (64u * C < n) { C <<= 1; lc++; }
    const int64_t hi = (int64_t)n - (int64_t)r * C, lo0 = hi - (int64_t)C;
    const int64_t lo = lo0 < 0 ? 0 : lo0;
    const uint32_t rmax = n ? (n + C - 1) / C - 1 : 0;
    uint32_t s = ((uint32_t)r == rmax) ? 0xFFFFFFFFu : 0u;
    for (int64_t i = lo; i < hi; i++) s = (s >> 8) ^ lds_tab[(s ^ p[i]) & 0xff];
#pragma unroll
    for (int k = 0; k < 6; k++) {
        const uint32_t v = (uint32_t)__shfl_down((int)s, 1 << k, WV);
        if ((r & ((2 << k) - 1)) == 0 && r + (1 << k) < WV) {
            const uint32_t *A = cod.crc_zadv + (size_t)(lc + k) * 1024;
            s ^= A[v & 0xff] ^ A[256 + ((v >> 8) & 0xff)] ^ A[512 + ((v >> 16) & 0xff)] ^ A[768 + (v >> 24)];
        }
    }
    return ~(uint32_t)__shfl((int)s, 0, WV);
}
__device__ __forceinline__ void decode_frame(SyncArgs &a, const uint32_t j, uint32_t lds_soft_bytes, uint32_t msg_bytes)
{
    const uint32_t ch = a.jobs[j].ch;
    if (ch >= a.nch || a.jobs[j].arena_off == ~0ull) return;
    const SyncConsts &c = a.c;
    const uint32_t n_msg = a.jobs[j].s.payload_len, crc = a.jobs[j].s.check, fec0 = a.jobs[j].s.fec0, fec1 = a.jobs[j].s.fec1;
    const uint32_t e1 = a.jobs[j].s.enc_len;
    uint8_t *soft = a.jsoft + (size_t)j * 8 * c.max_enc_len;
    const uint32_t crc_len = (crc == 6) ? 4u : 0u, n0 = n_msg + crc_len;
    const bool prof = SY_PROF(a) && j == 7;
    long long tk[8]; int ntk = 0;
#define DK_TICK() if (prof) tk[ntk++] = (long long)__builtin_readcyclecounter();
    DK_TICK()
    const bool lds_path = c.payload_soft && fec0 == 1 && (fec1 == 6 || fec1 == 7 || fec1 == 1) && 8u * e1 <= lds_soft_bytes && !(a.no_fast & 8);
    if (!lds_path) {
        const uint32_t moff = (c.il_off && e1 < c.il_n) ? c.il_off[e1] : ~0u;
        const bool conv_pre = c.payload_soft && fec1 == 11 && a.vit_scratch && moff != ~0u && 8u * e1 <= lds_soft_bytes && !(a.no_fast & 8) &&
                              vf::rows_for(8u * fec_enc_len_d(fec0, n0) + 6u) <= a.vit_rows;
        const bool conv_go = conv_pre;
        if (c.payload_soft && fec1 == 11 && !a.vit_scratch && a.hint && threadIdx.x == 0) a.hint[HINT_K7_SEEN] = 1u;
        if (conv_go) {
            const unsigned long long *g64 = reinterpret_cast<const unsigned long long *>(soft);
            for (uint32_t i = threadIdx.x; i < e1; i += DK_T) dk_soft[DKP(i)] = g64[i];
            __syncthreads();
            const uint4 *mp = reinterpret_cast<const uint4 *>(c.il_map + (size_t)moff * 8);
            const uint8_t *sb = reinterpret_cast<const uint8_t *>(dk_soft);
            unsigned long long *o64 = reinterpret_cast<unsigned long long *>(soft);
            for (uint32_t i = threadIdx.x; i < e1; i += DK_T) {
                const uint4 m = mp[i];
                const uint32_t lo = (uint32_t)sb[m.x & 0xffffu] | ((uint32_t)sb[m.x >> 16] << 8) | ((uint32_t)sb[m.y & 0xffffu] << 16) | ((uint32_t)sb[m.y >> 16] << 24);
                const uint32_t hi = (uint32_t)sb[m.z & 0xffffu] | ((uint32_t)sb[m.z >> 16] << 8) | ((uint32_t)sb[m.w & 0xffffu] << 16) | ((uint32_t)sb[m.w >> 16] << 24);
                o64[i] = (unsigned long long)lo | ((unsigned long long)hi << 32);
            }
        }
        if (threadIdx.x == 0 && a.gen_list) {
            uint32_t *gl = as_global(a.gen_list);
            uint32_t tag = j;
            if (conv_go) {
                tag |= 0x80000000u;
            }
            gl[1u + atomicAdd(gl, 1u)] = tag;
        }
        return;
    }
    if (lds_path) {
        const uint32_t moff_h = (fec1 == 6 && c.il_off && e1 < c.il_n) ? c.il_off[e1] : ~0u;
        const bool fused = DK_FUSED && moff_h != ~0u;
        constexpr int SU = 4;
        const uint2 *mp2 = reinterpret_cast<const uint2 *>(c.il_map + (size_t)(fused ? moff_h : 0u) * 8);
        uint2 pm[SU][3];
        if (fused) {
#pragma unroll
            for (int u = 0; u < SU; u++) {
                const uint32_t i = threadIdx.x + u * DK_T, ii = i < n0 ? i : 0u;
#pragma unroll
                for (int k = 0; k < 3; k++) pm[u][k] = mp2[3u * ii + k];
            }
        }
        const unsigned long long *g64 = reinterpret_cast<const unsigned long long *>(soft);
        for (uint32_t b0 = 0; b0 < e1; b0 += 8 * DK_T) {
            unsigned long long v[8];
#pragma unroll
#if DK_NT_LOAD
            for (int u = 0; u < 8; u++) { const uint32_t i = b0 + u * DK_T + threadIdx.x; v[u] = __builtin_nontemporal_load(g64 + (i < e1 ? i : 0)); }
#else
            for (int u = 0; u < 8; u++) { const uint32_t i = b0 + u * DK_T + threadIdx.x; v[u] = g64[i < e1 ? i : 0]; }
#endif
#pragma unroll
            for (int u = 0; u < 8; u++) { const uint32_t i = b0 + u * DK_T + threadIdx.x; if (i < e1) dk_soft[DKP(i)] = v[u]; }
        }
        __syncthreads();
        DK_TICK()
        unsigned long long *cur = dk_soft;
        uint8_t *msg = reinterpret_cast<uint8_t *>(dk_soft) + 2 * lds_soft_bytes;
        if (fused) {
            const uint8_t *sb = reinterpret_cast<const uint8_t *>(dk_soft);
            for (uint32_t b0 = 0; b0 < n0; b0 += SU * DK_T) {
                if (b0) {
#pragma unroll
                    for (int u = 0; u < SU; u++) {
                        const uint32_t i = b0 + threadIdx.x + u * DK_T, ii = i < n0 ? i : 0u;
#pragma unroll
                        for (int k = 0; k < 3; k++) pm[u][k] = mp2[3u * ii + k];
                    }
                }
#pragma unroll
                for (int u = 0; u < SU; u++) {
                    const uint32_t i = b0 + threadIdx.x + u * DK_T;
                    if (i >= n0) break;
                    uint32_t w[3];
#pragma unroll
                    for (int k = 0; k < 3; k++) {
                        const uint2 m = pm[u][k];
                        w[k] = (uint32_t)sb[m.x & 0xffffu] | ((uint32_t)sb[m.x >> 16] << 8) | ((uint32_t)sb[m.y & 0xffffu] << 16) | ((uint32_t)sb[m.y >> 16] << 24);
                    }
                    msg[i] = (uint8_t)h128_dec_soft_words(w[0], w[1], w[2]);
                }
            }
        } else if (fec1 != 1) {
            const uint32_t moff = (c.il_off && e1 < c.il_n) ? c.il_off[e1] : ~0u;
            if (moff != ~0u) {
                const uint4 *mp = reinterpret_cast<const uint4 *>(c.il_map + (size_t)moff * 8);
                const uint8_t *sb = reinterpret_cast<const uint8_t *>(dk_soft);
                unsigned long long *dst = dk_soft + lds_soft_bytes / 8;
                for (uint32_t i0 = threadIdx.x; i0 < e1; i0 += 8 * DK_T) {
                    uint4 mm[8];
#pragma unroll
                    for (int u = 0; u < 8; u++) { const uint32_t i = i0 + u * DK_T; mm[u] = mp[i < e1 ? i : 0]; }
#pragma unroll
                    for (int u = 0; u < 8; u++) {
                        const uint32_t i = i0 + u * DK_T;
                        if (i >= e1) break;
                        const uint4 m = mm[u];
                        const uint32_t lo = (uint32_t)sb[m.x & 0xffffu] | ((uint32_t)sb[m.x >> 16] << 8) | ((uint32_t)sb[m.y & 0xffffu] << 16) | ((uint32_t)sb[m.y >> 16] << 24);
                        const uint32_t hi = (uint32_t)sb[m.z & 0xffffu] | ((uint32_t)sb[m.z >> 16] << 8) | ((uint32_t)sb[m.w & 0xffffu] << 16) | ((uint32_t)sb[m.w >> 16] << 24);
                        dst[DKP(i)] = (unsigned long long)lo | ((unsigned long long)hi << 32);
                    }
                }
                cur = dst;
                __syncthreads();
            } else {
                unsigned Mi, Ni; il_dims(e1, Mi, Ni);
                const unsigned dummy = 2 * (lds_soft_bytes / 8) + msg_bytes / 8;
                il_pass_lds(e1, Mi, Ni + 8, 0x33, dummy);
                il_pass_lds(e1, Mi, Ni + 4, 0x55, dummy);
                il_pass_lds(e1, Mi, Ni + 2, 0x0f, dummy);
                il_pass_lds(e1, Mi, Ni, 0xff, dummy);
            }
        }
        DK_TICK()
        const uint32_t *w32 = reinterpret_cast<const uint32_t *>(cur);
        auto word = [&](uint32_t w) { return w32[2u * DKP(w >> 1) + (w & 1u)]; };
        auto slice = [&](uint32_t g) -> unsigned {
            const unsigned long long v = cur[DKP(g)];
            unsigned b = 0;
#pragma unroll
            for (int kb = 0; kb < 8; kb++) b = (b << 1) | ((((unsigned)(v >> (8 * kb)) & 0xffu) > 127u) ? 1u : 0u);
            return b;
        };
        if (fused) {
        } else if (fec1 == 6) {
            for (uint32_t i = threadIdx.x; i < n0; i += DK_T) msg[i] = (uint8_t)h128_dec_soft_words(word(3 * i), word(3 * i + 1), word(3 * i + 2));
        } else if (fec1 == 7) {
            const uint32_t G = n0 / 3, rr = n0 % 3;
            for (uint32_t g = threadIdx.x; g < G; g += DK_T) {
                const unsigned s0 = golay_dec_sym((slice(6 * g) << 16) | (slice(6 * g + 1) << 8) | slice(6 * g + 2));
                const unsigned s1 = golay_dec_sym((slice(6 * g + 3) << 16) | (slice(6 * g + 4) << 8) | slice(6 * g + 5));
                msg[3 * g]     = (uint8_t)((s0 >> 4) & 0xff);
                msg[3 * g + 1] = (uint8_t)(((s0 << 4) & 0xf0) | ((s1 >> 8) & 0x0f));
                msg[3 * g + 2] = (uint8_t)(s1 & 0xff);
            }
            if (threadIdx.x < rr) {
                const uint32_t b = 6 * G + 3 * threadIdx.x;
                msg[3 * G + threadIdx.x] = (uint8_t)(golay_dec_sym((slice(b) << 16) | (slice(b + 1) << 8) | slice(b + 2)) & 0xff);
            }
        } else {
            for (uint32_t i = threadIdx.x; i < n0; i += DK_T) msg[i] = (uint8_t)slice(i);
        }
        __syncthreads();
        DK_TICK()
        {
            uint32_t *dst = reinterpret_cast<uint32_t *>(a.arena + a.jobs[j].arena_off);
            const uint32_t *src = reinterpret_cast<const uint32_t *>(msg);
            for (uint32_t i = threadIdx.x; i < (n_msg + 3) / 4; i += DK_T) dst[i] = src[i];
        }
        const bool by_pos = crc_len && c.crc_pos && n_msg >= 4 && n_msg <= c.crc_pos_n;
        if (by_pos) {
            uint32_t acc = 0;
            for (uint32_t i0 = threadIdx.x; i0 < n_msg; i0 += 8 * DK_T) {
                uint32_t t[8];
#pragma unroll
                for (int u = 0; u < 8; u++) {
                    const uint32_t i = i0 + u * DK_T, ii = i < n_msg ? i : n_msg - 1;
                    const uint32_t b = (uint32_t)msg[ii] ^ (ii < 4 ? 0xffu : 0u);
                    t[u] = c.crc_pos[(size_t)(n_msg - 1 - ii) * 256 + b];
                }
#pragma unroll
                for (int u = 0; u < 8; u++) if (i0 + u * DK_T < n_msg) acc ^= t[u];
            }
            acc = wave_xor_u32(acc);
            if ((threadIdx.x & (WV - 1)) == 0) reinterpret_cast<uint32_t *>(dk_soft)[256 + threadIdx.x / WV] = acc;
        }
        reinterpret_cast<uint32_t *>(dk_soft)[threadIdx.x] = c.cod.crc_byte[threadIdx.x];
        __syncthreads();
        if (threadIdx.x >= WV) return;
    }
    bool valid = true;
    if (crc_len) {
        const uint8_t *msg = reinterpret_cast<const uint8_t *>(dk_soft) + 2 * lds_soft_bytes;
        const uint32_t key = ((uint32_t)msg[n_msg] << 24) | ((uint32_t)msg[n_msg + 1] << 16) |
                             ((uint32_t)msg[n_msg + 2] << 8) | (uint32_t)msg[n_msg + 3];
        const bool by_pos = c.crc_pos && n_msg >= 4 && n_msg <= c.crc_pos_n;
        if (by_pos) {
            const uint32_t *part = reinterpret_cast<const uint32_t *>(dk_soft) + 256;
            uint32_t tot = 0;
#pragma unroll
            for (int wv = 0; wv < DK_T / WV; wv++) tot ^= part[wv];
            valid = ~tot == key;
        } else valid = crc32_tree(c.cod, 0u, 2 * lds_soft_bytes, n_msg) == key;
    }
    DK_TICK()
    Walker<1> w(a, ch);
    const PayloadJob job = a.jobs[j];
    if (!w.bind_job(j, job)) return;
    const int64_t nsym = (int64_t)((w.s.mod_len + (uint32_t)c.M_data - 1) / (uint32_t)c.M_data);
    w.emit(w.s.cur + (int64_t)w.s.timer - 1 + (nsym - 1) * (int64_t)c.L, true, valid, false, false);
    DK_TICK()
    if (prof && threadIdx.x == 0) printf("[prof] decode wg7 cycles: stage %lld  passes %lld  h128 %lld  crc %lld  emit %lld\n", tk[1]-tk[0], tk[2]-tk[1], tk[3]-tk[2], tk[4]-tk[3], tk[5]-tk[4]);
#undef DK_TICK
}
__global__ __launch_bounds__(DK_T) void decode_kernel(SyncArgs a, uint32_t lds_soft_bytes, uint32_t msg_bytes)
{
    launder(a);
    uint32_t nl = a.live[0];
    if (nl > a.max_jobs) nl = a.max_jobs;
    for (uint32_t k = blockIdx.x; k < nl; k += gridDim.x) {
        const uint32_t j = a.live[1u + k];
        if (a.dec_phase && j < a.max_jobs) {
            const uint32_t mod = a.jobs[j].s.mod_scheme;
            const bool main_frame = k < a.live_off && (mod == 39 || mod == 40);
            if (main_frame != (a.dec_phase == 1)) continue;
        }
        decode_frame(a, j, lds_soft_bytes, msg_bytes);
        __syncthreads();
    }
}

__global__ __launch_bounds__(WV) __attribute__((amdgpu_num_vgpr(128))) void decode_general_kernel(SyncArgs a)
{
    launder(a);
    __shared__ uint16_t vf_ck[2 * 64 * 64];
    const uint32_t *gl = as_global(a.gen_list);
    uint32_t ng = gl[0];
    if (blockIdx.x == 0 && threadIdx.x == 0 && a.list_hint) a.list_hint[2] = ng;
    if (ng > a.max_jobs) ng = a.max_jobs;
    const SyncConsts &c = a.c;
    const bool have_rows = a.vit_scratch && blockIdx.x < a.vit_waves;
    uint2 *rows = a.vit_scratch + (have_rows ? (size_t)blockIdx.x * a.vit_rows * 64u : 0u);
    for (uint32_t k = blockIdx.x; k < ng; k += gridDim.x) {
        const bool pre_done = (gl[1 + k] & 0x80000000u) != 0;
        const uint32_t j = gl[1 + k] & 0x7fffffffu;
        const uint32_t ch = a.jobs[j].ch;
        if (ch >= a.nch || a.jobs[j].arena_off == ~0ull) continue;
        const uint32_t n_msg = a.jobs[j].s.payload_len, crc = a.jobs[j].s.check, fec0 = a.jobs[j].s.fec0, fec1 = a.jobs[j].s.fec1;
        const size_t tstride = (size_t)c.max_enc_len + 16;
        uint8_t *soft = a.jsoft + (size_t)j * 8 * c.max_enc_len;
        uint8_t *tmpa = a.jtmp + (size_t)j * 2 * tstride, *tmpb = tmpa + tstride;
        if (pre_done) {
            const uint32_t e0 = fec_enc_len_d(fec0, n_msg + ((crc == 6) ? 4u : 0u));
            if (have_rows) vf::decode_frame(soft, e0, tmpa, rows, vf_ck, a.vit_passes);
            else conv27_decode_wave(VitSym{ soft, false }, e0, tmpa, reinterpret_cast<uint16_t *>(tmpb), dk_soft);
            __syncthreads();
        }
        const bool valid = packet_decode(c.cod, c.payload_soft != 0, false, n_msg, crc, fec0, fec1, soft, tmpa, tmpb, dk_soft, MCRX_DEVEL_ABLATE(a), pre_done);
        Walker<1> w(a, ch);
        const PayloadJob job = a.jobs[j];
        if (!w.bind_job(j, job)) continue;
        const int64_t nsym = (int64_t)((w.s.mod_len + (uint32_t)c.M_data - 1) / (uint32_t)c.M_data);
        w.emit(w.s.cur + (int64_t)w.s.timer - 1 + (nsym - 1) * (int64_t)c.L, true, valid, false, true);
        __syncthreads();
    }
}

__global__ __launch_bounds__(WV) void place_jobs_kernel(SyncArgs a)
{
    launder(a);
    if (threadIdx.x != 0) return;
    if (a.gen_list) as_global(a.gen_list)[0] = 0;
    uint32_t nj = *a.njobs;
    if (nj > a.max_jobs) nj = a.max_jobs;
    if (a.njobs_next) *a.njobs_next = 0;
    if (a.qam_next) as_global(a.qam_next)[0] = 0;
    if (a.live_next) as_global(a.live_next)[0] = 0;
    { uint32_t nl = a.live[0]; if (nl > a.max_jobs) a.live[0] = a.max_jobs; }
    if (a.qam_list) {
        uint32_t nq = a.qam_list[0];
        if (nq > a.max_jobs) { nq = a.max_jobs; a.qam_list[0] = nq; }
        if (a.list_hint) a.list_hint[0] = nq;
    }
    if (a.stats) {
        const uint32_t maxenc = a.stats[7];
        a.stats[7] = 0;
        if (a.hint && maxenc) *a.hint = maxenc;
    }
    if (a.walk_hint && a.stats) {
        volatile uint32_t *h = a.walk_hint;
        h[0] = a.stats[0]; h[1] = a.stats[1]; h[2] = a.stats[4]; h[3] = a.stats[5]; h[4] = a.stats[2];
        const uint32_t tot = a.stats[0] + a.stats[1], prev = a.stats[6] <= tot ? a.stats[6] : 0u;
        a.stats[6] = tot;
        h[5] = tot - prev;
        __threadfence_system();
    }
}

__global__ __launch_bounds__(WV) void ilmap_build_kernel(const uint32_t *lens, const uint32_t *offs, uint8_t *lo, uint8_t *hi, uint16_t *map)
{
    const uint32_t e = lens[blockIdx.x];
    const size_t o = (size_t)offs[blockIdx.x] * 8;
    uint8_t *xl = lo + o, *xh = hi + o;
    for (uint32_t i = threadIdx.x; i < 8 * e; i += WV) { xl[i] = (uint8_t)((i >> 3) & 0xff); xh[i] = (uint8_t)((i >> 3) >> 8); }
    __syncthreads();
    deinterleave<true>(xl, e, 4);
    deinterleave<true>(xh, e, 4);
    __syncthreads();
    for (uint32_t i = threadIdx.x; i < 8 * e; i += WV) { const unsigned src = xl[i] | ((unsigned)xh[i] << 8); map[o + i] = (uint16_t)(8u * DKP(src) + (i & 7u)); }
}
hipError_t ilmap_build_launch(const uint32_t *d_lens, const uint32_t *d_offs, uint32_t nlen, uint8_t *d_lo, uint8_t *d_hi, uint16_t *d_map, hipStream_t st)
{
    if (!nlen) return hipSuccess;
    hipLaunchKernelGGL(ilmap_build_kernel, dim3(nlen), dim3(WV), 0, st, d_lens, d_offs, d_lo, d_hi, d_map);
    return hipGetLastError();
}

__global__ void sync_reset_kernel(ChanState *st, uint32_t nch, int64_t cur, float4 *z0, float4 *z1, size_t nz,
                                  uint32_t *nrec, unsigned long long *arena_used, uint32_t *pred_n)
{
    const size_t i = (size_t)blockIdx.x * blockDim.x + threadIdx.x;
    if (i < nz) { const float4 z = make_float4(0.f, 0.f, 0.f, 0.f); if (z0) z0[i] = z; if (z1) z1[i] = z; }
    if (i == 0) { if (nrec) { nrec[0] = 0; nrec[1] = 0; } if (arena_used) { arena_used[0] = 0; arena_used[1] = 0; } }
    if (i >= nch) return;
    if (pred_n) pred_n[i] = 0;
    ChanState z;
    memset(&z, 0, sizeof(z));
    z.state = SY_SEEK; z.cur = cur; z.g0 = 1.0f; z.fstate = FX_HEADER;
    st[i] = z;
}

hipError_t sync_reset_launch(ChanState *st, uint32_t nch, int64_t cur, float2 *hist0, float2 *hist1, size_t hist_n,
                             uint32_t *nrec, unsigned long long *arena_used, uint32_t *pred_n, hipStream_t stream)
{
    const size_t nz = hist_n / 2;
    const size_t n = nz > nch ? nz : nch;
    hipLaunchKernelGGL(sync_reset_kernel, dim3((unsigned)((n + 255) / 256)), dim3(256), 0, stream, st, nch, cur,
                       reinterpret_cast<float4 *>(hist0), reinterpret_cast<float4 *>(hist1), nz, nrec, arena_used, pred_n);
    return hipGetLastError();
}

#endif

hipError_t sy_launch_acq_e1(const SyncLaunch &l, const SyncArgs &a, hipStream_t st);
hipError_t sy_launch_acq_e2(const SyncLaunch &l, const SyncArgs &a, hipStream_t st);
template <int EE>
static hipError_t sy_launch_acq_width(const SyncLaunch &l, const SyncArgs &a, hipStream_t st)
{
    if (sync_kernel_in(l.k, SK_SPEC_E1)) hipLaunchKernelGGL((sync_spec_kernel<EE>), dim3(l.grid), dim3(l.block), l.lds, st, a);
    else if (sync_kernel_in(l.k, SK_TAIL_E1, 2)) hipLaunchKernelGGL((sync_tail_kernel<EE>), dim3(l.grid), dim3(l.block), l.lds, st, a);
    else if (sync_kernel_in(l.k, SK_LEAN_E1, 2)) hipLaunchKernelGGL((sync_lean_kernel<EE>), dim3(l.grid), dim3(l.block), l.lds, st, a);
    else return hipErrorInvalidValue;
    return hipSuccess;
}
template <int EE>
static hipError_t sy_launch_width(const SyncLaunch &l, const SyncArgs &a, hipStream_t st)
{
    const dim3 g(l.grid), b(l.block);
    switch (l.k - sync_width_index(EE)) {
    case SK_SYNC_E1:            hipLaunchKernelGGL((sync_kernel<EE>), g, b, l.lds, st, a); break;
    case SK_SPEC_E1: case SK_TAIL_E1: case SK_LEAN_E1:
        if constexpr (EE == 1) return sy_launch_acq_e1(l, a, st);
        else if constexpr (EE == 2) return sy_launch_acq_e2(l, a, st);
        else if (!sync_kernel_in(l.k, SK_SPEC_E1)) return hipErrorInvalidValue;
        else hipLaunchKernelGGL((sync_spec_kernel<EE>), g, b, l.lds, st, a);
        break;
    case SK_WALK_E1:
        if constexpr (EE <= 2) hipLaunchKernelGGL((sync_walk_kernel<EE>), g, b, l.lds, st, a);
        else return hipErrorInvalidValue;
        break;
    case SK_PAYLOAD_FAST_E1:    hipLaunchKernelGGL((payload_kernel<EE, true>), g, b, l.lds, st, a); break;
    case SK_PAYLOAD_GENERAL_E1: hipLaunchKernelGGL((payload_kernel<EE, false>), g, b, l.lds, st, a); break;
    default: return hipErrorInvalidValue;
    }
    return hipSuccess;
}
hipError_t sy_launch_e1(const SyncLaunch &l, const SyncArgs &a, hipStream_t st);
hipError_t sy_launch_e2(const SyncLaunch &l, const SyncArgs &a, hipStream_t st);
hipError_t sy_launch_e4(const SyncLaunch &l, const SyncArgs &a, hipStream_t st);
hipError_t sy_launch_e8(const SyncLaunch &l, const SyncArgs &a, hipStream_t st);
hipError_t sy_launch_e16(const SyncLaunch &l, const SyncArgs &a, hipStream_t st);
#if SY_PART < 0 || SY_PART == 0
hipError_t sy_launch_e1(const SyncLaunch &l, const SyncArgs &a, hipStream_t st) { return sy_launch_width<1>(l, a, st); }
hipError_t sy_launch_e2(const SyncLaunch &l, const SyncArgs &a, hipStream_t st) { return sy_launch_width<2>(l, a, st); }
#endif
#if SY_PART < 0 || SY_PART == 1
hipError_t sy_launch_e4(const SyncLaunch &l, const SyncArgs &a, hipStream_t st) { return sy_launch_width<4>(l, a, st); }
hipError_t sy_launch_e8(const SyncLaunch &l, const SyncArgs &a, hipStream_t st) { return sy_launch_width<8>(l, a, st); }
#endif
#if SY_PART < 0 || SY_PART == 2
hipError_t sy_launch_e16(const SyncLaunch &l, const SyncArgs &a, hipStream_t st) { return sy_launch_width<16>(l, a, st); }
#endif
#if SY_PART < 0 || SY_PART == 3
hipError_t sy_launch_acq_e1(const SyncLaunch &l, const SyncArgs &a, hipStream_t st) { return sy_launch_acq_width<1>(l, a, st); }
hipError_t sy_launch_acq_e2(const SyncLaunch &l, const SyncArgs &a, hipStream_t st) { return sy_launch_acq_width<2>(l, a, st); }
#endif

hipError_t acq_lean_launch(const SyncLaunch &l, const SyncArgs &a, hipStream_t st);
#if SY_PART < 0 || SY_PART == 4
#include "acq_lean.hpp"
hipError_t acq_lean_launch(const SyncLaunch &l, const SyncArgs &a, hipStream_t st)
{
    if (l.k == SK_ACQ_LEAN_M48) hipLaunchKernelGGL((acq_lean_kernel<63, 48>), dim3(l.grid), dim3(l.block), l.lds, st, a);
    else hipLaunchKernelGGL((acq_lean_kernel<63, 64>), dim3(l.grid), dim3(l.block), l.lds, st, a);
    return hipSuccess;
}
#endif

hipError_t payload_wide_launch(const SyncLaunch &l, const SyncArgs &a, hipStream_t st);
#if SY_PART < 0 || SY_PART == 1
#include "payload_wide.hpp"
hipError_t payload_wide_launch(const SyncLaunch &l, const SyncArgs &a, hipStream_t st)
{
    if (l.k == SK_WIDE_E2) hipLaunchKernelGGL((payload_wide_kernel<63, 2>), dim3(l.grid), dim3(l.block), l.lds, st, a);
    else hipLaunchKernelGGL((payload_wide_kernel<63, 4>), dim3(l.grid), dim3(l.block), l.lds, st, a);
    return hipSuccess;
}
#endif

#if SY_PART <= 0
static hipError_t sy_issue(const SyncLaunch &l, const SyncArgs &a, hipStream_t st, uint32_t soft_lds = 0, uint32_t msg_lds = 0)
{
    const dim3 g(l.grid), b(l.block);
    switch (l.k) {
    case SK_PLACE:              hipLaunchKernelGGL(place_jobs_kernel, g, b, l.lds, st, a); break;
    case SK_DECODE:             hipLaunchKernelGGL(decode_kernel, g, b, l.lds, st, a, soft_lds, msg_lds); break;
    case SK_DECODE_GENERAL:     hipLaunchKernelGGL(decode_general_kernel, g, b, l.lds, st, a); break;
    case SK_PLEAN_M48:          hipLaunchKernelGGL((payload_lean_kernel<63, 48>), g, b, l.lds, st, a); break;
    case SK_PLEAN_REST_M48:     hipLaunchKernelGGL((payload_lean_rest_kernel<63, 48>), g, b, l.lds, st, a); break;
    case SK_MULTI_4:            hipLaunchKernelGGL(payload_multi_kernel<4>, g, b, l.lds, st, a); break;
    case SK_MULTI_2:            hipLaunchKernelGGL(payload_multi_kernel<2>, g, b, l.lds, st, a); break;
    case SK_MULTI_1:            hipLaunchKernelGGL(payload_multi_kernel<1>, g, b, l.lds, st, a); break;
    case SK_PLEAN_XB0:          hipLaunchKernelGGL(payload_lean_kernel<0>, g, b, l.lds, st, a); break;
    case SK_PLEAN_REST_XB0:     hipLaunchKernelGGL(payload_lean_rest_kernel<0>, g, b, l.lds, st, a); break;
    case SK_PLEAN_XB63:         hipLaunchKernelGGL(payload_lean_kernel<63>, g, b, l.lds, st, a); break;
    case SK_PLEAN_REST_XB63:    hipLaunchKernelGGL(payload_lean_rest_kernel<63>, g, b, l.lds, st, a); break;
    case SK_ACQ_LEAN_M48: case SK_ACQ_LEAN_M64: return acq_lean_launch(l, a, st);
    case SK_WIDE_E2: case SK_WIDE_E4:           return payload_wide_launch(l, a, st);
    default:
        switch (a.c.E) {
        case 1:  return sy_launch_e1(l, a, st);
        case 2:  return sy_launch_e2(l, a, st);
        case 4:  return sy_launch_e4(l, a, st);
        case 8:  return sy_launch_e8(l, a, st);
        case 16: return sy_launch_e16(l, a, st);
        default: return hipErrorInvalidValue;
        }
    }
    return hipSuccess;
}

static SyncDesign sy_design(const SyncConsts &c) { return { c.M, c.E, c.log2M, c.M_pilot, c.Nen, c.max_enc_len, c.max_payload_len }; }
int acq_lean_waves(const SyncConsts &c) { return sync_lean_waves(sy_design(c)); }

static hipError_t sy_acquire(SyncAcq what, const SyncArgs &a0, hipStream_t st)
{
    const SyncAcqPlan p = sync_acq_plan(what, { sy_design(a0.c), a0.nch, a0.nseg, a0.spec_cap, a0.seg_phase, a0.seg_walker });
    if (p.status != SYNC_LAUNCH) return p.status == SYNC_NOTHING ? hipSuccess : hipErrorInvalidValue;
    SyncArgs a = a0;
    a.vit_off = p.vit_off;
    const hipError_t e = sy_issue(p.l, a, st);
    return e != hipSuccess ? e : hipGetLastError();
}
hipError_t sync_launch(const SyncArgs &a, hipStream_t st) { return sy_acquire(SYNC_ACQ_SCOUT, a, st); }
hipError_t sync_launch_lean(const SyncArgs &a, hipStream_t st) { return sy_acquire(SYNC_ACQ_LEAN, a, st); }
hipError_t sync_launch_walk(const SyncArgs &a, hipStream_t st) { return sy_acquire(SYNC_ACQ_WALK, a, st); }
hipError_t sync_launch_tail(const SyncArgs &a, hipStream_t st) { return sy_acquire(SYNC_ACQ_TAIL, a, st); }
hipError_t sync_launch_spec(const SyncArgs &a, hipStream_t st) { return sy_acquire(SYNC_ACQ_SPEC, a, st); }

static SyncPayloadInputs sy_payload_inputs(const SyncArgs &a)
{
    SyncPayloadInputs in = {};
    in.d = sy_design(a.c);
    in.nch = a.nch; in.max_jobs = a.max_jobs; in.frames_hint = a.frames_hint; in.grid_hint0 = a.grid_hint[0]; in.grid_hint2 = a.grid_hint[2];
    in.vit_waves = a.vit_waves; in.enc_hint = a.enc_hint; in.payload_lds_pad = a.payload_lds_pad;
    in.have_qam_list = a.qam_list != nullptr; in.have_vit_scratch = a.vit_scratch != nullptr;
    in.scout = a.scout; in.no_fast = a.no_fast; in.payload_fr = a.payload_fr; in.payload_lean = a.payload_lean; in.payload_xb = a.payload_xb;
    in.split_rest = a.split_rest; in.dec_phase = a.dec_phase;
    return in;
}
bool sync_payload_splits(const SyncArgs &a) { return sync_payload_splits(sy_payload_inputs(a)); }

hipError_t sync_launch_payload(const SyncArgs &a0, SyncStage stage, hipStream_t st)
{
    const SyncPayloadPlan p = sync_payload_plan(sy_payload_inputs(a0), stage);
    if (p.status != SYNC_LAUNCH) return p.status == SYNC_NOTHING ? hipSuccess : hipErrorInvalidValue;
    SyncArgs a = a0;
    a.live_off = p.live_off; a.split_rest = p.split_rest; a.dec_phase = p.dec_phase; a.dec_lds_soft = p.dec_lds_soft; a.vit_off = p.vit_off;
    if (p.clear_gen_list) a.gen_list = nullptr;
    for (int i = 0; i < p.n; i++) {
        const hipError_t e = sy_issue(p.l[i], a, st, p.soft_lds, p.msg_lds);
        if (e != hipSuccess) return e;
    }
    return hipGetLastError();
}
#endif

}
```

liquid-usrp_amd/csrc/rx_plan.hpp:

```cpp
#pragma once
#include "../../include/mcrx_hip.h"
#include "acq_shared.h"
#include "sync_plan.hpp"
#include "config_read.hpp"

#include <algorithm>
#include <cstdlib>

#define MCRX_SLOTS 8

namespace mcrx {

struct RxDevel {
    const char *serial = nullptr, *slots = nullptr, *no_scout = nullptr, *no_spec = nullptr;
    const char *payload_fr = nullptr, *payload_lean = nullptr, *payload_xb = nullptr;
    const char *acq_mode = nullptr, *lean_build = nullptr;
    const char *walk_lds_pad = nullptr, *payload_lds_pad = nullptr;
};

struct RxInputs {
    unsigned N, M, cp, taper;
    mcrx_hip_config ec;
    unsigned M_data, M_pilot;
    RxDevel devel;
};

struct RxPlan {
    unsigned K = 0;
    bool bypass = false;
    uint32_t in_fmt = 0; size_t ss = 8;
    uint32_t max_payload = 0, max_enc = 0, max_syms = 0;
    unsigned ch_first = 0, nch = 0;
    uint32_t max_rec = 0;
    uint64_t min_frame = 1;
    uint64_t arena_cap = 0, sarena_cap = 0;
    bool pipelined = true;
    uint32_t slab_blocks = 0;
    bool oversampled = false;
    unsigned chan_P = 14, hist_blocks = 13, col_shift = 0;
    uint64_t defer = 0; unsigned hist_tiles = 0;
    int payload_xb = 63, payload_lean = 1, payload_fr = 1;
    int acq_mode = 0;
    bool spec = false;
    int lean_build = 1;
    int seg_walker = 1;
    bool scout = true;
    uint32_t round_lds_pad = 0;
    uint32_t walk_lds_pad = 13312;
    unsigned nslots = 5;
    uint32_t max_jobs = 0;
    uint32_t vit_rows = 0, vit_waves = 0, vit_mode = 0;
    bool lean = false;
    size_t stage_cap = 0;
    size_t hist_bytes = 0;
    bool side_stream = false;
};

static inline int devel_int(const char *v, int dflt) { return v ? atoi(v) : dflt; }

#define MCRX_REFUSE(code, msg) do { *err = (msg); return (code); } while (0)

static inline int plan_frames(const RxInputs &in, RxPlan &r, const char **err)
{
    const unsigned N = in.N, M = in.M, cp = in.cp;
    const mcrx_hip_config &cfg = in.ec;
    r.max_payload = cfg.max_payload_len ? cfg.max_payload_len : 2048;
    r.max_enc = 4 * (r.max_payload + 4) + 16;
    if (r.max_enc < 256) r.max_enc = 256;
    r.max_enc = (r.max_enc + 15) & ~15u;
    r.max_syms = 8 * r.max_enc;
    r.ch_first = cfg.channel_first;
    if (r.ch_first >= N || (uint64_t)r.ch_first + cfg.channel_count > N) MCRX_REFUSE(MCRX_EINVAL, "channel shard outside [0, N)");
    r.nch = cfg.channel_count ? cfg.channel_count : N - r.ch_first;
    r.max_rec = cfg.max_frames ? cfg.max_frames : 16 * r.nch + 64;
    r.min_frame = (uint64_t)(3 + (288 + in.M_data - 1) / in.M_data + 2) * (M + cp);
    if (!cfg.max_frames) {
        const uint64_t batch = cfg.batch_samples ? cfg.batch_samples : ((uint64_t)1 << 20);
        const uint64_t per_ch = (batch / r.K + 8) / r.min_frame + 2;
        r.max_rec = (uint32_t)std::max<uint64_t>(r.max_rec, std::min<uint64_t>(per_ch * r.nch, 1u << 22));
        const uint64_t per_rec = ((((uint64_t)r.max_payload + 15) & ~15ull) + 64ull * (2ull * (r.max_payload + 4) + 8)) +
                                 10ull * r.max_enc + 32 + 8ull * M;
        const uint64_t bulk = std::min<uint64_t>((((uint64_t)16 << 20) / r.K + 8) / r.min_frame + 3, ((uint64_t)2 << 30) / per_rec / r.nch);
        r.max_rec = (uint32_t)std::max<uint64_t>(r.max_rec, bulk * r.nch);
    }
    r.arena_cap = (uint64_t)r.max_rec * (((uint64_t)r.max_payload + 15) & ~15ull);
    r.sarena_cap = (uint64_t)r.max_rec * (8ull * 8ull * (2ull * (r.max_payload + 4) + 8));
    if (r.sarena_cap > (8ull << 30)) r.sarena_cap = 8ull << 30;
    return MCRX_OK;
}

static inline int plan_builds(const mcrx_hip_config &cfg, const RxDevel &dv, RxPlan &r, const char **err)
{
    const uint32_t wb = cfg.worker_build, aq = cfg.acquisition, sb = cfg.scout_build;
    if (wb > 5 || aq > 5) MCRX_REFUSE(MCRX_EINVAL, "worker_build / acquisition out of range");
    if (wb == 1) r.payload_xb = 0;
    if (wb >= 2) { r.payload_lean = 0; r.payload_fr = wb == 2 ? 1 : wb == 3 ? 2 : wb == 4 ? 4 : 0; }
    if ((aq >= 1 && aq <= 3) || aq == 5) r.acq_mode = (int)aq;
    r.spec = aq != 4;
    if (sb > 2) MCRX_REFUSE(MCRX_EINVAL, "scout_build out of range");
    if (sb == 1) r.lean_build = 0;
    if (sb == 2) r.seg_walker = 0;
    if (dv.serial) r.pipelined = false;
    r.scout = dv.no_scout == nullptr;
    if (!r.scout || dv.no_spec) r.spec = false;
    r.payload_fr = devel_int(dv.payload_fr, r.payload_fr);
    r.payload_lean = devel_int(dv.payload_lean, r.payload_lean) != 0;
    r.payload_xb = devel_int(dv.payload_xb, r.payload_xb);
    r.acq_mode = devel_int(dv.acq_mode, r.acq_mode);
    r.lean_build = devel_int(dv.lean_build, r.lean_build);
    r.walk_lds_pad = (uint32_t)devel_int(dv.walk_lds_pad, (int)r.walk_lds_pad);
    r.round_lds_pad = (uint32_t)devel_int(dv.payload_lds_pad, (int)r.round_lds_pad);
    if (dv.slots) r.nslots = (unsigned)std::max(2, std::min(MCRX_SLOTS, atoi(dv.slots)));
    if (!r.pipelined) r.nslots = 2;
    return MCRX_OK;
}

inline int rx_plan(const RxInputs &in, RxPlan *out, const char **err)
{
    const unsigned N = in.N, M = in.M, cp = in.cp;
    const mcrx_hip_config &cfg = in.ec;
    RxPlan r;
    r.bypass = cfg.single_channel != 0;
    r.K = r.bypass ? 1 : 2 * N;
    r.in_fmt = cfg.input_format; r.ss = r.in_fmt == 1 ? 4 : 8;
    if (int rc = plan_frames(in, r, err)) return rc;
    r.pipelined = !cfg.serial;
    r.slab_blocks = cfg.slab_blocks ? ((cfg.slab_blocks + MCRX_TILE - 1) & ~(uint32_t)(MCRX_TILE - 1)) : 0;
    const uint32_t front_end = r.bypass ? 0 : cfg.front_end;
    if (front_end > 2) MCRX_REFUSE(MCRX_EINVAL, "front_end must be 0, 1 or 2");
    r.oversampled = front_end == 2;
    if (front_end && ((r.K & (r.K - 1)) || r.K > 1024 || r.K < 2)) MCRX_REFUSE(MCRX_EUNSUPP, "the oversampled front end needs a power-of-two channel count <= 512");
    if (front_end == 1) { r.chan_P = 28; r.hist_blocks = 27; r.col_shift = r.K / 2 + 1; }
    r.defer = cfg.defer_samples;
    r.hist_tiles = (unsigned)((r.defer + M + cp + 8 + MCRX_TILE - 1) / MCRX_TILE + 1);
    if (int rc = plan_builds(cfg, in.devel, r, err)) return rc;
    unsigned E = 1; while (E < (M + 63) / 64) E <<= 1;
    unsigned log2M = 0;
    if ((M & (M - 1)) == 0) while ((1u << log2M) < M) log2M++;
    r.lean = sync_fast_design({ (int)M, (int)E, (int)log2M, (int)in.M_pilot, 0, 0, 0 });
    if (r.scout) {
        r.max_jobs = 2 * r.max_rec + 4 * r.nch + 1024;
        if (cfg.payload_soft) {
            r.vit_rows = vf::rows_for(4u * r.max_enc + 6u);
            r.vit_waves = (uint32_t)std::max<uint64_t>(64, std::min<uint64_t>(r.max_rec, 2048));
            r.vit_mode = cfg.conv_scratch;
            if (r.vit_mode > 2) MCRX_REFUSE(MCRX_EINVAL, "conv_scratch must be 0, 1 or 2");
        }
    }
    r.spec = r.spec && r.lean;
    r.hist_bytes = ((size_t)r.hist_blocks * r.K * r.ss + 15) & ~(size_t)15;
    const size_t tile_samples = (size_t)MCRX_TILE * r.K;
    const size_t want = cfg.batch_samples ? cfg.batch_samples : ((size_t)1 << 20);
    r.stage_cap = std::max<size_t>(1, (want + tile_samples - 1) / tile_samples) * tile_samples;
    r.side_stream = r.pipelined && r.nch <= 32 && cfg.channel_count == 0;
    *out = r;
    return MCRX_OK;
}

#undef MCRX_REFUSE

}
```

liquid-usrp_amd/csrc/sync_plan.hpp:

```cpp
#pragma once
#include <stddef.h>
#include <stdint.h>
#include "acq_shared.h"

#define SY_MAXM 1024
#define SY_LDS_BYTES(M) ((((size_t)(M) * 8 + (size_t)(M) * 12 + 256 + 3 * MCRX_HDR_SYMS + 32 + 4 * MCRX_SPEC_MAX + 256) + 15) & ~(size_t)15)
#define VIT_B 960u
#define DK_T 256
#define SY_WALK_WPB 1
#ifndef ACQ_LEAN_WAVES
#define ACQ_LEAN_WAVES 3
#endif
#ifndef SY_REST_FLOOR
#define SY_REST_FLOOR 256u
#endif
#ifndef SY_GEN_FLOOR
#define SY_GEN_FLOOR 128u
#endif

namespace mcrx {

struct SyncDesign { int M, E, log2M, M_pilot, Nen; uint32_t max_enc_len, max_payload_len; };
constexpr int SY_WAVE = 64;

inline int sync_width_index(int E) { return E == 1 ? 0 : E == 2 ? 1 : E == 4 ? 2 : E == 8 ? 3 : E == 16 ? 4 : -1; }
inline bool sync_pilots_in_row(const SyncDesign &d) { return d.M_pilot <= 16; }
inline bool sync_fast_design(const SyncDesign &d) { return ((d.log2M >= 6 && d.M == SY_WAVE * d.E) || (d.M == 48 && d.E == 1)) && d.M_pilot <= SY_WAVE; }
inline bool sync_lean_workers(const SyncDesign &d) { return sync_fast_design(d) && (d.M == SY_WAVE || d.M == 48) && sync_pilots_in_row(d); }
inline bool sync_wide_workers(const SyncDesign &d) { return (d.E == 2 || d.E == 4) && d.log2M >= 7 && d.M == SY_WAVE * d.E && d.M_pilot >= 1 && d.M_pilot <= SY_WAVE; }
inline int sync_lean_waves(const SyncDesign &d) { return ((d.M == 64 || d.M == 48) && d.E == 1 && sync_pilots_in_row(d) && d.M_pilot >= 1 && d.Nen <= 64) ? ACQ_LEAN_WAVES : 0; }

enum SyncKernel {
    SK_NONE = 0,
    SK_SYNC_E1, SK_SYNC_E2, SK_SYNC_E4, SK_SYNC_E8, SK_SYNC_E16,
    SK_SPEC_E1, SK_SPEC_E2, SK_SPEC_E4, SK_SPEC_E8, SK_SPEC_E16,
    SK_PAYLOAD_FAST_E1, SK_PAYLOAD_FAST_E2, SK_PAYLOAD_FAST_E4, SK_PAYLOAD_FAST_E8, SK_PAYLOAD_FAST_E16,
    SK_PAYLOAD_GENERAL_E1, SK_PAYLOAD_GENERAL_E2, SK_PAYLOAD_GENERAL_E4, SK_PAYLOAD_GENERAL_E8, SK_PAYLOAD_GENERAL_E16,
    SK_TAIL_E1, SK_TAIL_E2, SK_LEAN_E1, SK_LEAN_E2, SK_WALK_E1, SK_WALK_E2,
    SK_ACQ_LEAN_M48, SK_ACQ_LEAN_M64,
    SK_MULTI_1, SK_MULTI_2, SK_MULTI_4,
    SK_PLEAN_XB0, SK_PLEAN_XB63, SK_PLEAN_M48,
    SK_PLEAN_REST_XB0, SK_PLEAN_REST_XB63, SK_PLEAN_REST_M48,
    SK_WIDE_E2, SK_WIDE_E4,
    SK_PLACE, SK_DECODE, SK_DECODE_GENERAL,
    SK_COUNT
};
inline bool sync_kernel_in(SyncKernel k, SyncKernel family, int n = 5) { return k >= family && k < family + n; }
inline bool sync_kernel_decodes(SyncKernel k) { return sync_kernel_in(k, SK_SYNC_E1) || sync_kernel_in(k, SK_PAYLOAD_GENERAL_E1) || sync_kernel_in(k, SK_TAIL_E1, 2); }

struct SyncLaunch { SyncKernel k = SK_NONE; unsigned grid = 0, block = SY_WAVE; size_t lds = 0; };
enum SyncStatus { SYNC_LAUNCH = 0, SYNC_NOTHING, SYNC_INVALID };

inline SyncLaunch sync_width_launch(SyncKernel family, const SyncDesign &d, unsigned grid, uint32_t *vit_off)
{
    SyncLaunch l;
    l.k = (SyncKernel)(family + sync_width_index(d.E)); l.grid = grid; l.lds = SY_LDS_BYTES(d.M);
    *vit_off = 0;
    if (sync_kernel_decodes(l.k)) {
        *vit_off = (uint32_t)((l.lds + 15) & ~(size_t)15);
        l.lds = *vit_off + (size_t)VIT_B * 8;
    }
    return l;
}

enum SyncAcq { SYNC_ACQ_SCOUT = 0, SYNC_ACQ_LEAN, SYNC_ACQ_WALK, SYNC_ACQ_TAIL, SYNC_ACQ_SPEC };
struct SyncAcqInputs { SyncDesign d; uint32_t nch, nseg, spec_cap; int seg_phase, seg_walker; };
struct SyncAcqPlan { SyncStatus status = SYNC_NOTHING; SyncLaunch l; uint32_t vit_off = 0; };

inline SyncAcqPlan sync_acq_plan(SyncAcq what, const SyncAcqInputs &in)
{
    SyncAcqPlan r;
    const SyncDesign &d = in.d;
    if (in.nch == 0 || (what == SYNC_ACQ_SPEC && (in.spec_cap == 0 || in.nseg == 0))) return r;
    r.status = SYNC_INVALID;
    if (what != SYNC_ACQ_TAIL && what != SYNC_ACQ_SPEC && d.M > SY_MAXM) return r;
    if (what == SYNC_ACQ_SPEC && sync_lean_waves(d) && !in.seg_walker) {
        r.l.k = d.M == 48 ? SK_ACQ_LEAN_M48 : SK_ACQ_LEAN_M64;
    } else {
        if (sync_width_index(d.E) < 0) return r;
        static const SyncKernel narrow[5] = { SK_SYNC_E1, SK_LEAN_E1, SK_WALK_E1, SK_TAIL_E1, SK_SPEC_E1 };
        r.l = sync_width_launch(d.E <= 2 || what == SYNC_ACQ_SPEC ? narrow[what] : SK_SYNC_E1, d, 0, &r.vit_off);
    }
    r.l.grid = what == SYNC_ACQ_SPEC && in.seg_phase != 1 ? in.nch * in.nseg : in.nch;
    if (sync_kernel_in(r.l.k, SK_WALK_E1, 2)) {
        r.l.grid = (in.nch + SY_WALK_WPB - 1) / SY_WALK_WPB; r.l.block = SY_WAVE * SY_WALK_WPB;
        r.l.lds = SY_WALK_WPB * SY_LDS_BYTES(d.E * SY_WAVE);
    }
    r.status = SYNC_LAUNCH;
    return r;
}

enum SyncStage { SYNC_PLACE = 0, SYNC_WORKERS = 1, SYNC_DECODE = 2, SYNC_DECODE_GENERAL = 3, SYNC_BEHIND = 4 };
struct SyncPayloadInputs {
    SyncDesign d;
    uint32_t nch, max_jobs, frames_hint, grid_hint0, grid_hint2, vit_waves, enc_hint, payload_lds_pad;
    bool have_qam_list, have_vit_scratch;
    int scout, no_fast, payload_fr, payload_lean, payload_xb, split_rest, dec_phase;
};
struct SyncPayloadPlan {
    SyncStatus status = SYNC_NOTHING;
    int n = 0; SyncLaunch l[2];
    uint32_t soft_lds = 0, msg_lds = 0;
    uint32_t live_off = 0, dec_lds_soft = 0, vit_off = 0; int split_rest = 0, dec_phase = 0; bool clear_gen_list = false;
};

inline bool sync_fast_path(const SyncPayloadInputs &in) { return sync_fast_design(in.d) && !(in.no_fast & 1); }
inline bool sync_lean_path(const SyncPayloadInputs &in) { return sync_fast_path(in) && !(in.no_fast & 6); }
inline bool sync_payload_splits(const SyncPayloadInputs &in)
{
    return in.scout && sync_lean_path(in) && sync_lean_workers(in.d) && in.payload_fr == 1 && in.payload_lean;
}

inline uint32_t sync_decode_soft_lds(const SyncPayloadInputs &in)
{
    const uint32_t enc_cap = in.enc_hint ? ((in.enc_hint + 127u) & ~127u) : in.d.max_enc_len;
    size_t soft_lds = (size_t)8 * (enc_cap < in.d.max_enc_len ? enc_cap : in.d.max_enc_len);
    if (soft_lds > 56 * 1024) soft_lds = 56 * 1024;
    if (soft_lds < 4096) soft_lds = 4096;
    return (uint32_t)soft_lds;
}

inline void sync_worker_launches(const SyncPayloadInputs &in, SyncStage stage, unsigned ngrid, SyncPayloadPlan &r)
{
    const SyncDesign &d = in.d;
    const unsigned nj = in.max_jobs;
    const int fr = in.payload_fr;
    const bool narrow = sync_lean_path(in) && sync_lean_workers(d);
    if (narrow && in.payload_lean && (d.M == 48 ? fr == 1 : fr > 0 && fr != 2 && fr != 4)) {
        unsigned nq = in.grid_hint0 == ~0u ? nj : 2u * in.grid_hint0;
        nq = nq < SY_REST_FLOOR ? SY_REST_FLOOR : (nq > nj ? nj : nq);
        const SyncKernel k = d.M == 48 ? SK_PLEAN_M48 : in.payload_xb == 0 ? SK_PLEAN_XB0 : SK_PLEAN_XB63;
        if (stage != SYNC_BEHIND) { r.l[r.n].k = k; r.l[r.n].grid = ngrid; r.n++; }
        if (stage == SYNC_BEHIND || !r.split_rest) { r.l[r.n].k = (SyncKernel)(k + 3); r.l[r.n].grid = in.have_qam_list ? nq : nj; r.n++; }
        r.l[0].lds = r.l[1].lds = in.payload_lds_pad;
    } else if (narrow && d.M == SY_WAVE && fr > 0) {
        const unsigned f = fr == 4 ? 4 : fr == 2 ? 2 : 1;
        r.l[0].k = f == 4 ? SK_MULTI_4 : f == 2 ? SK_MULTI_2 : SK_MULTI_1; r.l[0].grid = (nj + f - 1) / f; r.l[0].lds = f == 1 ? in.payload_lds_pad : 0;
        r.n = 1;
    } else if (sync_lean_path(in) && sync_wide_workers(d) && in.payload_lean && fr == 1) {
        r.l[0].k = d.E == 2 ? SK_WIDE_E2 : SK_WIDE_E4; r.l[0].grid = ngrid; r.n = 1;
    } else if (sync_width_index(d.E) < 0) r.status = SYNC_INVALID;
    else { r.l[0] = sync_width_launch(sync_fast_path(in) ? SK_PAYLOAD_FAST_E1 : SK_PAYLOAD_GENERAL_E1, d, nj, &r.vit_off); r.n = 1; }
}

inline SyncPayloadPlan sync_payload_plan(const SyncPayloadInputs &in, SyncStage stage)
{
    SyncPayloadPlan r;
    if (in.nch == 0 || !in.scout || in.max_jobs == 0) return r;
    const unsigned nj = in.max_jobs;
    unsigned ngrid = in.frames_hint == ~0u ? nj : in.frames_hint + in.frames_hint / 4 + 64;
    if (ngrid > nj) ngrid = nj;
    const bool fast = sync_fast_path(in);
    r.live_off = sync_payload_splits(in) ? ngrid : 0;
    if (stage == SYNC_BEHIND && !r.live_off) return r;
    if (r.live_off) { r.split_rest = in.split_rest; r.dec_phase = in.dec_phase; }
    r.dec_lds_soft = fast ? sync_decode_soft_lds(in) : 0u;
    r.clear_gen_list = !fast;
    if ((stage == SYNC_DECODE || stage == SYNC_DECODE_GENERAL) && !fast) return r;
    r.status = SYNC_LAUNCH; r.n = 1;
    if (stage == SYNC_PLACE) { r.l[0].k = SK_PLACE; r.l[0].grid = 1; }
    else if (stage == SYNC_DECODE) {
        r.soft_lds = r.dec_lds_soft; r.msg_lds = (uint32_t)(((size_t)in.d.max_payload_len + 4 + 15) & ~(size_t)15);
        r.l[0].k = SK_DECODE; r.l[0].grid = ngrid; r.l[0].block = DK_T; r.l[0].lds = 2 * (size_t)r.soft_lds + r.msg_lds + 16;
    } else if (stage == SYNC_DECODE_GENERAL) {
        unsigned ggrid = in.grid_hint2 ? (nj < 4096 ? nj : 4096) : SY_GEN_FLOOR;
        if (in.have_vit_scratch && ggrid > in.vit_waves) ggrid = in.vit_waves;
        r.l[0].k = SK_DECODE_GENERAL; r.l[0].grid = ggrid; r.l[0].lds = (size_t)VIT_B * 8;
    } else { r.n = 0; sync_worker_launches(in, stage, ngrid, r); }
    return r;
}

}
```

Before: 192,400.

## Make decode kernel persistent with double-buffered LDS staging of next frame

Restructures decode_kernel into a persistent loop whose grid is capped at the number of workgroups that can be resident, computed from occupancy and register queries. While the current frame is decoded, the next frame's job metadata and soft bits are prefetched into the other LDS half, so global loads overlap with compute. Job fields are made wave-uniform via readfirstlane. The trade-offs are fewer workgroups, more register and LDS pressure, and added host-side occupancy queries whenever the LDS size changes.

```diff
diff --git a/include/mcrx_hip.h b/include/mcrx_hip.h
--- a/include/mcrx_hip.h
+++ b/include/mcrx_hip.h
@@ -40,6 +40,7 @@
     uint32_t scout_build;
     uint32_t conv_scratch;
     uint32_t input_format;
+    uint32_t decoder_build;
 } mcrx_hip_config;
 
 typedef struct {
diff --git a/liquid-usrp_amd/__init__.py b/liquid-usrp_amd/__init__.py
--- a/liquid-usrp_amd/__init__.py
+++ b/liquid-usrp_amd/__init__.py
@@ -36,6 +36,10 @@
                 ("serial", C.c_uint32), ("chunk_blocks", C.c_uint32), ("defer_samples", C.c_uint32), ("front_end", C.c_uint32), ("skip_framesyms", C.c_uint32),
                 ("worker_build", C.c_uint32), ("acquisition", C.c_uint32), ("scout_build", C.c_uint32), ("conv_scratch", C.c_uint32),
                 ("input_format", C.c_uint32)]
+
+
+class ConfigV2(C.Structure):
+    _fields_ = Config._fields_ + [("decoder_build", C.c_uint32)]
 
 
 INPUT_FORMATS = {"cf32": 0, "sc16": 1}
@@ -354,8 +358,8 @@
         self._h = C.c_void_p()
         self.N, self.K, self.M, self.cp = num_channels, 2 * num_channels, M, cp_len
         parr = None if p is None else np.ascontiguousarray(np.frombuffer(bytes(bytearray(p)), np.uint8))
-        c = Config()
-        c.struct_size = C.sizeof(Config)
+        c = ConfigV2()
+        c.struct_size = C.sizeof(ConfigV2)
         c.payload_soft = 1
         for k, v in cfg.items():
             setattr(c, k, _format_code(v, INPUT_FORMATS, "input_format") if k == "input_format" else v)
diff --git a/liquid-usrp_amd/csrc/kernels.h b/liquid-usrp_amd/csrc/kernels.h
--- a/liquid-usrp_amd/csrc/kernels.h
+++ b/liquid-usrp_amd/csrc/kernels.h
@@ -181,6 +181,7 @@
     int no_fast;
     int payload_fr, payload_lean, payload_xb;
     uint32_t vit_off;
+    uint32_t dec_resident;
 };
 hipError_t sync_launch(const SyncArgs &a, hipStream_t st);
 hipError_t sync_launch_tail(const SyncArgs &a, hipStream_t st);
@@ -190,6 +191,7 @@
 int acq_lean_waves(const SyncConsts &c);
 hipError_t sync_launch_spec(const SyncArgs &a, hipStream_t st);
 hipError_t sync_launch_payload(const SyncArgs &a, SyncStage stage, hipStream_t st);
+hipError_t sync_decode_resident(const SyncArgs &a, uint32_t *lds, uint32_t *resident);
 bool sync_payload_splits(const SyncArgs &a);
 hipError_t sync_reset_launch(ChanState *st, uint32_t nch, int64_t cur, float2 *hist0, float2 *hist1, size_t hist_n,
                              uint32_t *nrec, unsigned long long *arena_used, uint32_t *pred_n, hipStream_t stream);
diff --git a/liquid-usrp_amd/csrc/mcrx_hip.hip b/liquid-usrp_amd/csrc/mcrx_hip.hip
--- a/liquid-usrp_amd/csrc/mcrx_hip.hip
+++ b/liquid-usrp_amd/csrc/mcrx_hip.hip
@@ -147,6 +147,7 @@
     PayloadJob *d_jobs[MCRX_SLOTS] = {}; uint32_t *d_njobs = nullptr; float2 *d_jR[MCRX_SLOTS] = {};
     uint32_t *d_gen[MCRX_SLOTS] = {}, *d_qam[MCRX_SLOTS] = {}, *d_live[MCRX_SLOTS] = {};
     uint2 *d_vit_scratch = nullptr; uint32_t *d_vit_passes = nullptr;
+    uint32_t dec_res_lds = 0, dec_res_n = 0;
     uint64_t seq = 0;
     uint32_t *d_stats = nullptr;
     hipStream_t s_scout = nullptr, s_work = nullptr, s_copy = nullptr;
@@ -807,6 +808,12 @@
     HIPCHK(sync_launch_payload(a, SYNC_WORKERS, sw));
     RC(q->ev_end(3, sw));
     RC(q->ev_begin(4, sw));
+    a.dec_resident = 0;
+    if (q->decoder_build != 1) {
+        HIPCHK(sync_decode_resident(a, &q->dec_res_lds, &q->dec_res_n));
+        a.dec_resident = q->dec_res_n;
+        if (q->decoder_build >= 2 && (a.dec_resident == 0 || a.dec_resident > q->decoder_build)) a.dec_resident = q->decoder_build;
+    }
     HIPCHK(sync_launch_payload(a, SYNC_DECODE, sw));
     if (split) {
         HIPCHK(hipEventRecord(q->ev_side[slot], sw));
diff --git a/liquid-usrp_amd/csrc/ofdmsync.hip b/liquid-usrp_amd/csrc/ofdmsync.hip
--- a/liquid-usrp_amd/csrc/ofdmsync.hip
+++ b/liquid-usrp_amd/csrc/ofdmsync.hip
@@ -2601,11 +2601,10 @@
     }
     __syncthreads();
 }
-__device__ uint32_t crc32_tree(const CodingDev cod, uint32_t tab_off, uint32_t msg_off, uint32_t n)
+__device__ uint32_t crc32_tree(const CodingDev cod, uint32_t tab_off, uint32_t msg_off, uint32_t n, const int r)
 {
     const uint32_t *lds_tab = reinterpret_cast<const uint32_t *>(reinterpret_cast<const uint8_t *>(dk_soft) + tab_off);
     const uint8_t *p = reinterpret_cast<const uint8_t *>(dk_soft) + msg_off;
-    const int r = lane_id();
     uint32_t C = 1, lc = 0;
     while (64u * C < n) { C <<= 1; lc++; }
     const int64_t hi = (int64_t)n - (int64_t)r * C, lo0 = hi - (int64_t)C;
@@ -2623,230 +2622,329 @@
     }
     return ~(uint32_t)__shfl((int)s, 0, WV);
 }
-__device__ __forceinline__ void decode_frame(SyncArgs &a, const uint32_t j, uint32_t lds_soft_bytes, uint32_t msg_bytes)
-{
-    const uint32_t ch = a.jobs[j].ch;
-    if (ch >= a.nch || a.jobs[j].arena_off == ~0ull) return;
+struct DkJob { uint32_t j, ch, n_msg, crc, fec0, fec1, e1, mod; unsigned long long arena_off; };
+enum { DK_SKIP = 0, DK_GENERAL = 1, DK_LDS = 2 };
+__device__ __forceinline__ uint32_t dk_uni(uint32_t v) { return (uint32_t)__builtin_amdgcn_readfirstlane((int)v); }
+__device__ __forceinline__ DkJob dk_job_request(const SyncArgs &a, uint32_t j, bool there)
+{
+    const PayloadJob &p = a.jobs[there ? j : 0u];
+    DkJob r;
+    r.j = there ? j : ~0u; r.ch = p.ch; r.arena_off = p.arena_off;
+    r.n_msg = p.s.payload_len; r.crc = p.s.check; r.fec0 = p.s.fec0; r.fec1 = p.s.fec1; r.e1 = p.s.enc_len; r.mod = p.s.mod_scheme;
+    return r;
+}
+__device__ __forceinline__ DkJob dk_job_uniform(const DkJob &v)
+{
+    DkJob r;
+    r.j = dk_uni(v.j); r.ch = dk_uni(v.ch); r.n_msg = dk_uni(v.n_msg); r.crc = dk_uni(v.crc); r.fec0 = dk_uni(v.fec0); r.fec1 = dk_uni(v.fec1);
+    r.e1 = dk_uni(v.e1); r.mod = dk_uni(v.mod);
+    r.arena_off = (unsigned long long)dk_uni((uint32_t)v.arena_off) | ((unsigned long long)dk_uni((uint32_t)(v.arena_off >> 32)) << 32);
+    return r;
+}
+__device__ __forceinline__ int dk_class(const SyncArgs &a, const DkJob &m, uint32_t k, uint32_t lds_soft_bytes)
+{
+    if (m.j == ~0u) return DK_SKIP;
+    if (a.dec_phase) {
+        const bool main_frame = k < a.live_off && (m.mod == 39 || m.mod == 40);
+        if (main_frame != (a.dec_phase == 1)) return DK_SKIP;
+    }
+    if (m.ch >= a.nch || m.arena_off == ~0ull) return DK_SKIP;
+    const bool lds_path = a.c.payload_soft && m.fec0 == 1 && (m.fec1 == 6 || m.fec1 == 7 || m.fec1 == 1) && 8u * m.e1 <= lds_soft_bytes && !(a.no_fast & 8);
+    return lds_path ? DK_LDS : DK_GENERAL;
+}
+__device__ __forceinline__ uint32_t dk_moff_request(const SyncConsts &c, const DkJob &m, int cls)
+{
+    const bool have = cls == DK_LDS && m.fec1 == 6 && c.il_off && m.e1 < c.il_n;
+    const uint32_t v = c.il_off ? c.il_off[have ? m.e1 : 0u] : ~0u;
+    return have ? v : ~0u;
+}
+__device__ __forceinline__ void dk_general(SyncArgs &a, const DkJob &m, uint32_t lds_soft_bytes, uint32_t tid)
+{
     const SyncConsts &c = a.c;
-    const uint32_t n_msg = a.jobs[j].s.payload_len, crc = a.jobs[j].s.check, fec0 = a.jobs[j].s.fec0, fec1 = a.jobs[j].s.fec1;
-    const uint32_t e1 = a.jobs[j].s.enc_len;
+    const uint32_t j = m.j, e1 = m.e1, fec0 = m.fec0, fec1 = m.fec1;
+    const uint32_t n0 = m.n_msg + ((m.crc == 6) ? 4u : 0u);
     uint8_t *soft = a.jsoft + (size_t)j * 8 * c.max_enc_len;
-    const uint32_t crc_len = (crc == 6) ? 4u : 0u, n0 = n_msg + crc_len;
-    const bool prof = SY_PROF(a) && j == 7;
-    long long tk[8]; int ntk = 0;
+    const uint32_t moff = (c.il_off && e1 < c.il_n) ? dk_uni(c.il_off[e1]) : ~0u;
+    const bool conv_go = c.payload_soft && fec1 == 11 && a.vit_scratch && moff != ~0u && 8u * e1 <= lds_soft_bytes && !(a.no_fast & 8) &&
+                         vf::rows_for(8u * fec_enc_len_d(fec0, n0) + 6u) <= a.vit_rows;
+    if (c.payload_soft && fec1 == 11 && !a.vit_scratch && a.hint && tid == 0) a.hint[HINT_K7_SEEN] = 1u;
+    if (conv_go) {
+        const unsigned long long *g64 = reinterpret_cast<const unsigned long long *>(soft);
+        for (uint32_t i = tid; i < e1; i += DK_T) dk_soft[DKP(i)] = g64[i];
+        __syncthreads();
+        const uint4 *mp = reinterpret_cast<const uint4 *>(c.il_map + (size_t)moff * 8);
+        const uint8_t *sb = reinterpret_cast<const uint8_t *>(dk_soft);
+        unsigned long long *o64 = reinterpret_cast<unsigned long long *>(soft);
+        for (uint32_t i = tid; i < e1; i += DK_T) {
+            const uint4 m4 = mp[i];
+            const uint32_t lo = (uint32_t)sb[m4.x & 0xffffu] | ((uint32_t)sb[m4.x >> 16] << 8) | ((uint32_t)sb[m4.y & 0xffffu] << 16) | ((uint32_t)sb[m4.y >> 16] << 24);
+            const uint32_t hi = (uint32_t)sb[m4.z & 0xffffu] | ((uint32_t)sb[m4.z >> 16] << 8) | ((uint32_t)sb[m4.w & 0xffffu] << 16) | ((uint32_t)sb[m4.w >> 16] << 24);
+            o64[i] = (unsigned long long)lo | ((unsigned long long)hi << 32);
+        }
+    }
+    if (tid == 0 && a.gen_list) {
+        uint32_t *gl = as_global(a.gen_list);
+        gl[1u + atomicAdd(gl, 1u)] = conv_go ? (j | 0x80000000u) : j;
+    }
+}
+struct DkRec { int32_t header_valid; uint32_t hw0, hw1; float evm, g0; uint32_t nco_dtheta, mod_scheme, bps, check, fec0, fec1, mod_len, payload_len, timer, pad; int64_t cur; uint64_t syms_off; };
+__device__ __forceinline__ DkRec dk_rec_request(const SyncArgs &a, uint32_t j)
+{
+    const PayloadJob &p = a.jobs[j];
+    DkRec r;
+    r.header_valid = p.s.header_valid; r.hw0 = p.s.hw[0]; r.hw1 = p.s.hw[1]; r.evm = p.s.evm; r.g0 = p.s.g0; r.nco_dtheta = p.s.nco_dtheta;
+    r.mod_scheme = p.s.mod_scheme; r.bps = p.s.bps; r.check = p.s.check; r.fec0 = p.s.fec0; r.fec1 = p.s.fec1; r.mod_len = p.s.mod_len;
+    r.payload_len = p.s.payload_len; r.timer = p.s.timer; r.pad = p.pad; r.cur = p.s.cur; r.syms_off = p.syms_off;
+    return r;
+}
+__device__ __forceinline__ void dk_emit(const SyncArgs &a, const DkJob &m, const DkRec &q, bool payload_valid, uint32_t tid)
+{
+    const SyncConsts &c = a.c;
+    if (tid != 0) return;
+    uint32_t md = (uint32_t)c.M_data;
+    asm volatile("" : "+s"(md));
+    const int64_t nsym = (int64_t)((q.mod_len + md - 1) / md);
+    const int64_t t_ev = q.cur + (int64_t)q.timer - 1 + (nsym - 1) * (int64_t)c.L;
+    uint32_t idx = q.pad;
+    if (idx >= a.max_rec) { atomicAdd(a.nrec + 1, 1u); idx = 0xFFFFFFFFu; }
+    if (idx == 0xFFFFFFFFu) return;
+    FrameRec r;
+    r.channel = a.ch_first + m.ch; r.header_valid = q.header_valid; r.payload_valid = payload_valid ? 1 : 0;
+    r.payload_len = q.payload_len;
+    for (int i = 0; i < 8; i++) r.header[i] = (uint8_t)(((i < 4 ? q.hw0 : q.hw1) >> (8 * (i & 3))) & 0xffu);
+    r.evm = q.evm; r.rssi = -10.0f * log10f(q.g0);
+    r.cfo = u32rad(q.nco_dtheta) / TWO_PI_F;
+    r.mod_scheme = q.mod_scheme; r.mod_bps = q.bps;
+    r.check = q.check; r.fec0 = q.fec0; r.fec1 = q.fec1;
+    r.num_framesyms = q.mod_len; r.end_sample = t_ev;
+    r.payload_off = m.arena_off; r.syms_off = q.syms_off;
+    a.rec[idx] = r;
+}
+
+__global__ __launch_bounds__(DK_T, 4) void decode_kernel(SyncArgs a, uint32_t lds_soft_bytes, uint32_t msg_bytes)
+{
+    launder(a);
+    const SyncConsts &c = a.c;
+    uint32_t nl = dk_uni(a.live[0]);
+    if (nl > a.max_jobs) nl = a.max_jobs;
+    const uint32_t grid = gridDim.x;
+    uint32_t k = blockIdx.x;
+    if (k >= nl) return;
+    constexpr int SU = 4;
+    uint8_t *const msg = reinterpret_cast<uint8_t *>(dk_soft) + 2 * lds_soft_bytes;
+    uint32_t jn_v = k + grid < nl ? a.live[1u + k + grid] : ~0u;
+    DkJob cur;
+    { const uint32_t j0 = a.live[1u + k]; cur = dk_job_uniform(dk_job_request(a, j0, j0 < a.max_jobs)); }
+    int cls = dk_class(a, cur, k, lds_soft_bytes);
+    uint32_t moff = dk_uni(dk_moff_request(c, cur, cls));
+    bool staged = false;
+    uint32_t half = 0;
+    for (;;) {
+        uint32_t tid = threadIdx.x;
+        asm volatile("" : "+v"(tid));
+        const uint32_t kn = k + grid, k2 = kn + grid;
+        const uint32_t j2_v = k2 < nl ? a.live[1u + k2] : ~0u;
+        const DkJob nreq = dk_job_request(a, jn_v, kn < nl && jn_v < a.max_jobs);
+        const bool prof = SY_PROF(a) && cur.j == 7;
+        long long tk[8]; int ntk = 0;
 #define DK_TICK() if (prof) tk[ntk++] = (long long)__builtin_readcyclecounter();
-    DK_TICK()
-    const bool lds_path = c.payload_soft && fec0 == 1 && (fec1 == 6 || fec1 == 7 || fec1 == 1) && 8u * e1 <= lds_soft_bytes && !(a.no_fast & 8);
-    if (!lds_path) {
-        const uint32_t moff = (c.il_off && e1 < c.il_n) ? c.il_off[e1] : ~0u;
-        const bool conv_pre = c.payload_soft && fec1 == 11 && a.vit_scratch && moff != ~0u && 8u * e1 <= lds_soft_bytes && !(a.no_fast & 8) &&
-                              vf::rows_for(8u * fec_enc_len_d(fec0, n0) + 6u) <= a.vit_rows;
-        const bool conv_go = conv_pre;
-        if (c.payload_soft && fec1 == 11 && !a.vit_scratch && a.hint && threadIdx.x == 0) a.hint[HINT_K7_SEEN] = 1u;
-        if (conv_go) {
-            const unsigned long long *g64 = reinterpret_cast<const unsigned long long *>(soft);
-            for (uint32_t i = threadIdx.x; i < e1; i += DK_T) dk_soft[DKP(i)] = g64[i];
-            __syncthreads();
-            const uint4 *mp = reinterpret_cast<const uint4 *>(c.il_map + (size_t)moff * 8);
-            const uint8_t *sb = reinterpret_cast<const uint8_t *>(dk_soft);
-            unsigned long long *o64 = reinterpret_cast<unsigned long long *>(soft);
-            for (uint32_t i = threadIdx.x; i < e1; i += DK_T) {
-                const uint4 m = mp[i];
-                const uint32_t lo = (uint32_t)sb[m.x & 0xffffu] | ((uint32_t)sb[m.x >> 16] << 8) | ((uint32_t)sb[m.y & 0xffffu] << 16) | ((uint32_t)sb[m.y >> 16] << 24);
-                const uint32_t hi = (uint32_t)sb[m.z & 0xffffu] | ((uint32_t)sb[m.z >> 16] << 8) | ((uint32_t)sb[m.w & 0xffffu] << 16) | ((uint32_t)sb[m.w >> 16] << 24);
-                o64[i] = (unsigned long long)lo | ((unsigned long long)hi << 32);
-            }
-        }
-        if (threadIdx.x == 0 && a.gen_list) {
-            uint32_t *gl = as_global(a.gen_list);
-            uint32_t tag = j;
-            if (conv_go) {
-                tag |= 0x80000000u;
-            }
-            gl[1u + atomicAdd(gl, 1u)] = tag;
-        }
-        return;
-    }
-    if (lds_path) {
-        const uint32_t moff_h = (fec1 == 6 && c.il_off && e1 < c.il_n) ? c.il_off[e1] : ~0u;
-        const bool fused = DK_FUSED && moff_h != ~0u;
-        constexpr int SU = 4;
-        const uint2 *mp2 = reinterpret_cast<const uint2 *>(c.il_map + (size_t)(fused ? moff_h : 0u) * 8);
+        DK_TICK()
+        const bool lds = cls == DK_LDS;
+        const bool fused = lds && DK_FUSED && moff != ~0u;
+        if (cls == DK_GENERAL) dk_general(a, cur, lds_soft_bytes, tid);
+        const uint32_t n_msg = cur.n_msg, e1 = cur.e1, fec1 = cur.fec1;
+        const uint32_t crc_len = (cur.crc == 6) ? 4u : 0u, n0 = n_msg + crc_len;
+        unsigned long long *const S = dk_soft + (size_t)half * (lds_soft_bytes / 8);
+        const uint2 *mp2 = reinterpret_cast<const uint2 *>(c.il_map + (size_t)(fused ? moff : 0u) * 8);
         uint2 pm[SU][3];
         if (fused) {
 #pragma unroll
             for (int u = 0; u < SU; u++) {
-                const uint32_t i = threadIdx.x + u * DK_T, ii = i < n0 ? i : 0u;
-#pragma unroll
-                for (int k = 0; k < 3; k++) pm[u][k] = mp2[3u * ii + k];
-            }
-        }
-        const unsigned long long *g64 = reinterpret_cast<const unsigned long long *>(soft);
-        for (uint32_t b0 = 0; b0 < e1; b0 += 8 * DK_T) {
-            unsigned long long v[8];
+                const uint32_t i = tid + u * DK_T, ii = i < n0 ? i : 0u;
+#pragma unroll
+                for (int q = 0; q < 3; q++) pm[u][q] = mp2[3u * ii + q];
+            }
+        }
+        if (lds && !staged) {
+            const unsigned long long *g64 = reinterpret_cast<const unsigned long long *>(a.jsoft + (size_t)cur.j * 8 * c.max_enc_len);
+            for (uint32_t b0 = 0; b0 < e1; b0 += 8 * DK_T) {
+                unsigned long long v[8];
 #pragma unroll
 #if DK_NT_LOAD
-            for (int u = 0; u < 8; u++) { const uint32_t i = b0 + u * DK_T + threadIdx.x; v[u] = __builtin_nontemporal_load(g64 + (i < e1 ? i : 0)); }
+                for (int u = 0; u < 8; u++) { const uint32_t i = b0 + u * DK_T + tid; v[u] = __builtin_nontemporal_load(g64 + (i < e1 ? i : 0)); }
 #else
-            for (int u = 0; u < 8; u++) { const uint32_t i = b0 + u * DK_T + threadIdx.x; v[u] = g64[i < e1 ? i : 0]; }
+                for (int u = 0; u < 8; u++) { const uint32_t i = b0 + u * DK_T + tid; v[u] = g64[i < e1 ? i : 0]; }
 #endif
 #pragma unroll
-            for (int u = 0; u < 8; u++) { const uint32_t i = b0 + u * DK_T + threadIdx.x; if (i < e1) dk_soft[DKP(i)] = v[u]; }
-        }
-        __syncthreads();
+                for (int u = 0; u < 8; u++) { const uint32_t i = b0 + u * DK_T + tid; if (i < e1) S[DKP(i)] = v[u]; }
+            }
+            __syncthreads();
+        }
         DK_TICK()
-        unsigned long long *cur = dk_soft;
-        uint8_t *msg = reinterpret_cast<uint8_t *>(dk_soft) + 2 * lds_soft_bytes;
-        if (fused) {
-            const uint8_t *sb = reinterpret_cast<const uint8_t *>(dk_soft);
-            for (uint32_t b0 = 0; b0 < n0; b0 += SU * DK_T) {
-                if (b0) {
+        const DkJob nxt = dk_job_uniform(nreq);
+        const int cls_n = dk_class(a, nxt, kn, lds_soft_bytes);
+        const uint32_t moff_nv = dk_moff_request(c, nxt, cls_n);
+        bool next_staged = false;
+        uint32_t moff_n = ~0u;
+        if (lds) {
+            unsigned long long *curp = S;
+            if (fused) {
+                const uint8_t *sb = reinterpret_cast<const uint8_t *>(S);
+                for (uint32_t b0 = 0; b0 < n0; b0 += SU * DK_T) {
+                    if (b0) {
+#pragma unroll
+                        for (int u = 0; u < SU; u++) {
+                            const uint32_t i = b0 + tid + u * DK_T, ii = i < n0 ? i : 0u;
+#pragma unroll
+                            for (int q = 0; q < 3; q++) pm[u][q] = mp2[3u * ii + q];
+                        }
+                    }
 #pragma unroll
                     for (int u = 0; u < SU; u++) {
-                        const uint32_t i = b0 + threadIdx.x + u * DK_T, ii = i < n0 ? i : 0u;
-#pragma unroll
-                        for (int k = 0; k < 3; k++) pm[u][k] = mp2[3u * ii + k];
+                        const uint32_t i = b0 + tid + u * DK_T;
+                        if (i >= n0) break;
+                        uint32_t w[3];
+#pragma unroll
+                        for (int q = 0; q < 3; q++) {
+                            const uint2 m = pm[u][q];
+                            w[q] = (uint32_t)sb[m.x & 0xffffu] | ((uint32_t)sb[m.x >> 16] << 8) | ((uint32_t)sb[m.y & 0xffffu] << 16) | ((uint32_t)sb[m.y >> 16] << 24);
+                        }
+                        msg[i] = (uint8_t)h128_dec_soft_words(w[0], w[1], w[2]);
                     }
                 }
-#pragma unroll
-                for (int u = 0; u < SU; u++) {
-                    const uint32_t i = b0 + threadIdx.x + u * DK_T;
-                    if (i >= n0) break;
-                    uint32_t w[3];
-#pragma unroll
-                    for (int k = 0; k < 3; k++) {
-                        const uint2 m = pm[u][k];
-                        w[k] = (uint32_t)sb[m.x & 0xffffu] | ((uint32_t)sb[m.x >> 16] << 8) | ((uint32_t)sb[m.y & 0xffffu] << 16) | ((uint32_t)sb[m.y >> 16] << 24);
+            } else if (fec1 != 1) {
+                const uint32_t moffg = (c.il_off && e1 < c.il_n) ? dk_uni(c.il_off[e1]) : ~0u;
+                if (moffg != ~0u) {
+                    const uint4 *mp = reinterpret_cast<const uint4 *>(c.il_map + (size_t)moffg * 8);
+                    const uint8_t *sb = reinterpret_cast<const uint8_t *>(dk_soft);
+                    unsigned long long *dst = dk_soft + lds_soft_bytes / 8;
+                    for (uint32_t i0 = tid; i0 < e1; i0 += 8 * DK_T) {
+                        uint4 mm[8];
+#pragma unroll
+                        for (int u = 0; u < 8; u++) { const uint32_t i = i0 + u * DK_T; mm[u] = mp[i < e1 ? i : 0]; }
+#pragma unroll
+                        for (int u = 0; u < 8; u++) {
+                            const uint32_t i = i0 + u * DK_T;
+                            if (i >= e1) break;
+                            const uint4 m = mm[u];
+                            const uint32_t lo = (uint32_t)sb[m.x & 0xffffu] | ((uint32_t)sb[m.x >> 16] << 8) | ((uint32_t)sb[m.y & 0xffffu] << 16) | ((uint32_t)sb[m.y >> 16] << 24);
+                            const uint32_t hi = (uint32_t)sb[m.z & 0xffffu] | ((uint32_t)sb[m.z >> 16] << 8) | ((uint32_t)sb[m.w & 0xffffu] << 16) | ((uint32_t)sb[m.w >> 16] << 24);
+                            dst[DKP(i)] = (unsigned long long)lo | ((unsigned long long)hi << 32);
+                        }
                     }
-                    msg[i] = (uint8_t)h128_dec_soft_words(w[0], w[1], w[2]);
-                }
-            }
-        } else if (fec1 != 1) {
-            const uint32_t moff = (c.il_off && e1 < c.il_n) ? c.il_off[e1] : ~0u;
-            if (moff != ~0u) {
-                const uint4 *mp = reinterpret_cast<const uint4 *>(c.il_map + (size_t)moff * 8);
-                const uint8_t *sb = reinterpret_cast<const uint8_t *>(dk_soft);
-                unsigned long long *dst = dk_soft + lds_soft_bytes / 8;
-                for (uint32_t i0 = threadIdx.x; i0 < e1; i0 += 8 * DK_T) {
-                    uint4 mm[8];
-#pragma unroll
-                    for (int u = 0; u < 8; u++) { const uint32_t i = i0 + u * DK_T; mm[u] = mp[i < e1 ? i : 0]; }
+                    curp = dst;
+                    __syncthreads();
+                } else {
+                    unsigned Mi, Ni; il_dims(e1, Mi, Ni);
+                    const unsigned dummy = 2 * (lds_soft_bytes / 8) + msg_bytes / 8;
+                    il_pass_lds(e1, Mi, Ni + 8, 0x33, dummy);
+                    il_pass_lds(e1, Mi, Ni + 4, 0x55, dummy);
+                    il_pass_lds(e1, Mi, Ni + 2, 0x0f, dummy);
+                    il_pass_lds(e1, Mi, Ni, 0xff, dummy);
+                }
+            }
+            DK_TICK()
+            const uint32_t *w32 = reinterpret_cast<const uint32_t *>(curp);
+            auto word = [&](uint32_t w) { return w32[2u * DKP(w >> 1) + (w & 1u)]; };
+            auto slice = [&](uint32_t g) -> unsigned {
+                const unsigned long long v = curp[DKP(g)];
+                unsigned b = 0;
+#pragma unroll
+                for (int kb = 0; kb < 8; kb++) b = (b << 1) | ((((unsigned)(v >> (8 * kb)) & 0xffu) > 127u) ? 1u : 0u);
+                return b;
+            };
+            if (fused) {
+            } else if (fec1 == 6) {
+                for (uint32_t i = tid; i < n0; i += DK_T) msg[i] = (uint8_t)h128_dec_soft_words(word(3 * i), word(3 * i + 1), word(3 * i + 2));
+            } else if (fec1 == 7) {
+                const uint32_t G = n0 / 3, rr = n0 % 3;
+                for (uint32_t g = tid; g < G; g += DK_T) {
+                    const unsigned s0 = golay_dec_sym((slice(6 * g) << 16) | (slice(6 * g + 1) << 8) | slice(6 * g + 2));
+                    const unsigned s1 = golay_dec_sym((slice(6 * g + 3) << 16) | (slice(6 * g + 4) << 8) | slice(6 * g + 5));
+                    msg[3 * g]     = (uint8_t)((s0 >> 4) & 0xff);
+                    msg[3 * g + 1] = (uint8_t)(((s0 << 4) & 0xf0) | ((s1 >> 8) & 0x0f));
+                    msg[3 * g + 2] = (uint8_t)(s1 & 0xff);
+                }
+                if (tid < rr) {
+                    const uint32_t b = 6 * G + 3 * tid;
+                    msg[3 * G + tid] = (uint8_t)(golay_dec_sym((slice(b) << 16) | (slice(b + 1) << 8) | slice(b + 2)) & 0xff);
+                }
+            } else {
+                for (uint32_t i = tid; i < n0; i += DK_T) msg[i] = (uint8_t)slice(i);
+            }
+            const bool by_pos = crc_len && c.crc_pos && n_msg >= 4 && n_msg <= c.crc_pos_n;
+            const bool tree = crc_len && !by_pos;
+            moff_n = dk_uni(moff_nv);
+            next_staged = fused && !tree && cls_n == DK_LDS && DK_FUSED && moff_n != ~0u && nxt.e1 <= 8u * DK_T;
+            unsigned long long nv[8];
+            if (next_staged) {
+                const unsigned long long *g64 = reinterpret_cast<const unsigned long long *>(a.jsoft + (size_t)nxt.j * 8 * c.max_enc_len);
+#pragma unroll
+#if DK_NT_LOAD
+                for (int u = 0; u < 8; u++) { const uint32_t i = u * DK_T + tid; nv[u] = __builtin_nontemporal_load(g64 + (i < nxt.e1 ? i : 0)); }
+#else
+                for (int u = 0; u < 8; u++) { const uint32_t i = u * DK_T + tid; nv[u] = g64[i < nxt.e1 ? i : 0]; }
+#endif
+            }
+            __syncthreads();
+            DK_TICK()
+            {
+                uint32_t *dst = reinterpret_cast<uint32_t *>(a.arena + cur.arena_off);
+                const uint32_t *src = reinterpret_cast<const uint32_t *>(msg);
+                for (uint32_t i = tid; i < (n_msg + 3) / 4; i += DK_T) dst[i] = src[i];
+            }
+            uint32_t *const S32 = reinterpret_cast<uint32_t *>(S);
+            if (by_pos) {
+                uint32_t acc = 0;
+                for (uint32_t i0 = tid; i0 < n_msg; i0 += 8 * DK_T) {
+                    uint32_t t[8];
 #pragma unroll
                     for (int u = 0; u < 8; u++) {
-                        const uint32_t i = i0 + u * DK_T;
-                        if (i >= e1) break;
-                        const uint4 m = mm[u];
-                        const uint32_t lo = (uint32_t)sb[m.x & 0xffffu] | ((uint32_t)sb[m.x >> 16] << 8) | ((uint32_t)sb[m.y & 0xffffu] << 16) | ((uint32_t)sb[m.y >> 16] << 24);
-                        const uint32_t hi = (uint32_t)sb[m.z & 0xffffu] | ((uint32_t)sb[m.z >> 16] << 8) | ((uint32_t)sb[m.w & 0xffffu] << 16) | ((uint32_t)sb[m.w >> 16] << 24);
-                        dst[DKP(i)] = (unsigned long long)lo | ((unsigned long long)hi << 32);
+                        const uint32_t i = i0 + u * DK_T, ii = i < n_msg ? i : n_msg - 1;
+                        const uint32_t b = (uint32_t)msg[ii] ^ (ii < 4 ? 0xffu : 0u);
+                        t[u] = c.crc_pos[(size_t)(n_msg - 1 - ii) * 256 + b];
                     }
-                }
-                cur = dst;
-                __syncthreads();
-            } else {
-                unsigned Mi, Ni; il_dims(e1, Mi, Ni);
-                const unsigned dummy = 2 * (lds_soft_bytes / 8) + msg_bytes / 8;
-                il_pass_lds(e1, Mi, Ni + 8, 0x33, dummy);
-                il_pass_lds(e1, Mi, Ni + 4, 0x55, dummy);
-                il_pass_lds(e1, Mi, Ni + 2, 0x0f, dummy);
-                il_pass_lds(e1, Mi, Ni, 0xff, dummy);
-            }
-        }
-        DK_TICK()
-        const uint32_t *w32 = reinterpret_cast<const uint32_t *>(cur);
-        auto word = [&](uint32_t w) { return w32[2u * DKP(w >> 1) + (w & 1u)]; };
-        auto slice = [&](uint32_t g) -> unsigned {
-            const unsigned long long v = cur[DKP(g)];
-            unsigned b = 0;
-#pragma unroll
-            for (int kb = 0; kb < 8; kb++) b = (b << 1) | ((((unsigned)(v >> (8 * kb)) & 0xffu) > 127u) ? 1u : 0u);
-            return b;
-        };
-        if (fused) {
-        } else if (fec1 == 6) {
-            for (uint32_t i = threadIdx.x; i < n0; i += DK_T) msg[i] = (uint8_t)h128_dec_soft_words(word(3 * i), word(3 * i + 1), word(3 * i + 2));
-        } else if (fec1 == 7) {
-            const uint32_t G = n0 / 3, rr = n0 % 3;
-            for (uint32_t g = threadIdx.x; g < G; g += DK_T) {
-                const unsigned s0 = golay_dec_sym((slice(6 * g) << 16) | (slice(6 * g + 1) << 8) | slice(6 * g + 2));
-                const unsigned s1 = golay_dec_sym((slice(6 * g + 3) << 16) | (slice(6 * g + 4) << 8) | slice(6 * g + 5));
-                msg[3 * g]     = (uint8_t)((s0 >> 4) & 0xff);
-                msg[3 * g + 1] = (uint8_t)(((s0 << 4) & 0xf0) | ((s1 >> 8) & 0x0f));
-                msg[3 * g + 2] = (uint8_t)(s1 & 0xff);
-            }
-            if (threadIdx.x < rr) {
-                const uint32_t b = 6 * G + 3 * threadIdx.x;
-                msg[3 * G + threadIdx.x] = (uint8_t)(golay_dec_sym((slice(b) << 16) | (slice(b + 1) << 8) | slice(b + 2)) & 0xff);
-            }
-        } else {
-            for (uint32_t i = threadIdx.x; i < n0; i += DK_T) msg[i] = (uint8_t)slice(i);
-        }
-        __syncthreads();
-        DK_TICK()
-        {
-            uint32_t *dst = reinterpret_cast<uint32_t *>(a.arena + a.jobs[j].arena_off);
-            const uint32_t *src = reinterpret_cast<const uint32_t *>(msg);
-            for (uint32_t i = threadIdx.x; i < (n_msg + 3) / 4; i += DK_T) dst[i] = src[i];
-        }
-        const bool by_pos = crc_len && c.crc_pos && n_msg >= 4 && n_msg <= c.crc_pos_n;
-        if (by_pos) {
-            uint32_t acc = 0;
-            for (uint32_t i0 = threadIdx.x; i0 < n_msg; i0 += 8 * DK_T) {
-                uint32_t t[8];
-#pragma unroll
-                for (int u = 0; u < 8; u++) {
-                    const uint32_t i = i0 + u * DK_T, ii = i < n_msg ? i : n_msg - 1;
-                    const uint32_t b = (uint32_t)msg[ii] ^ (ii < 4 ? 0xffu : 0u);
-                    t[u] = c.crc_pos[(size_t)(n_msg - 1 - ii) * 256 + b];
-                }
-#pragma unroll
-                for (int u = 0; u < 8; u++) if (i0 + u * DK_T < n_msg) acc ^= t[u];
-            }
-            acc = wave_xor_u32(acc);
-            if ((threadIdx.x & (WV - 1)) == 0) reinterpret_cast<uint32_t *>(dk_soft)[256 + threadIdx.x / WV] = acc;
-        }
-        reinterpret_cast<uint32_t *>(dk_soft)[threadIdx.x] = c.cod.crc_byte[threadIdx.x];
-        __syncthreads();
-        if (threadIdx.x >= WV) return;
-    }
-    bool valid = true;
-    if (crc_len) {
-        const uint8_t *msg = reinterpret_cast<const uint8_t *>(dk_soft) + 2 * lds_soft_bytes;
-        const uint32_t key = ((uint32_t)msg[n_msg] << 24) | ((uint32_t)msg[n_msg + 1] << 16) |
-                             ((uint32_t)msg[n_msg + 2] << 8) | (uint32_t)msg[n_msg + 3];
-        const bool by_pos = c.crc_pos && n_msg >= 4 && n_msg <= c.crc_pos_n;
-        if (by_pos) {
-            const uint32_t *part = reinterpret_cast<const uint32_t *>(dk_soft) + 256;
-            uint32_t tot = 0;
-#pragma unroll
-            for (int wv = 0; wv < DK_T / WV; wv++) tot ^= part[wv];
-            valid = ~tot == key;
-        } else valid = crc32_tree(c.cod, 0u, 2 * lds_soft_bytes, n_msg) == key;
-    }
-    DK_TICK()
-    Walker<1> w(a, ch);
-    const PayloadJob job = a.jobs[j];
-    if (!w.bind_job(j, job)) return;
-    const int64_t nsym = (int64_t)((w.s.mod_len + (uint32_t)c.M_data - 1) / (uint32_t)c.M_data);
-    w.emit(w.s.cur + (int64_t)w.s.timer - 1 + (nsym - 1) * (int64_t)c.L, true, valid, false, false);
-    DK_TICK()
-    if (prof && threadIdx.x == 0) printf("[prof] decode wg7 cycles: stage %lld  passes %lld  h128 %lld  crc %lld  emit %lld\n", tk[1]-tk[0], tk[2]-tk[1], tk[3]-tk[2], tk[4]-tk[3], tk[5]-tk[4]);
+#pragma unroll
+                    for (int u = 0; u < 8; u++) if (i0 + u * DK_T < n_msg) acc ^= t[u];
+                }
+                {
+                    const int bp = (int)(((tid & (WV - 1)) ^ 32u) << 2);
+#define MCRX_XSTEP(H) acc ^= __builtin_bit_cast(uint32_t, xor_lane<H>(__builtin_bit_cast(float, acc), bp));
+                    MCRX_XSTEP(1) MCRX_XSTEP(2) MCRX_XSTEP(4) MCRX_XSTEP(8) MCRX_XSTEP(16) MCRX_XSTEP(32)
+#undef MCRX_XSTEP
+                }
+                if ((tid & (WV - 1)) == 0) S32[256 + tid / WV] = acc;
+                if (tid == 0) S32[256 + DK_T / WV] = ((uint32_t)msg[n_msg] << 24) | ((uint32_t)msg[n_msg + 1] << 16) | ((uint32_t)msg[n_msg + 2] << 8) | (uint32_t)msg[n_msg + 3];
+            } else if (tree) S32[tid] = c.cod.crc_byte[tid];
+            if (next_staged) {
+                unsigned long long *const O = dk_soft + (size_t)(half ^ 1u) * (lds_soft_bytes / 8);
+#pragma unroll
+                for (int u = 0; u < 8; u++) { const uint32_t i = u * DK_T + tid; if (i < nxt.e1) O[DKP(i)] = nv[u]; }
+            }
+            __syncthreads();
+            DK_TICK()
+            if (tid < WV) {
+                bool valid = true;
+                if (by_pos) {
+                    uint32_t tot = 0;
+#pragma unroll
+                    for (int wv = 0; wv < DK_T / WV; wv++) tot ^= S32[256 + wv];
+                    valid = ~tot == S32[256 + DK_T / WV];
+                } else if (tree) {
+                    const uint32_t key = ((uint32_t)msg[n_msg] << 24) | ((uint32_t)msg[n_msg + 1] << 16) | ((uint32_t)msg[n_msg + 2] << 8) | (uint32_t)msg[n_msg + 3];
+                    valid = crc32_tree(c.cod, half * lds_soft_bytes, 2 * lds_soft_bytes, n_msg, (int)(tid & (WV - 1))) == key;
+                }
+                const DkRec rq = dk_rec_request(a, cur.j);
+                dk_emit(a, cur, rq, valid, tid);
+            }
+            DK_TICK()
+            if (prof && tid == 0) printf("[prof] decode wg cycles (frame 7, staged %d): stage %lld  passes %lld  h128 %lld  crc %lld  emit %lld\n", (int)staged, tk[1]-tk[0], tk[2]-tk[1], tk[3]-tk[2], tk[4]-tk[3], tk[5]-tk[4]);
+        } else moff_n = dk_uni(moff_nv);
 #undef DK_TICK
-}
-__global__ __launch_bounds__(DK_T) void decode_kernel(SyncArgs a, uint32_t lds_soft_bytes, uint32_t msg_bytes)
-{
-    launder(a);
-    uint32_t nl = a.live[0];
-    if (nl > a.max_jobs) nl = a.max_jobs;
-    for (uint32_t k = blockIdx.x; k < nl; k += gridDim.x) {
-        const uint32_t j = a.live[1u + k];
-        if (a.dec_phase && j < a.max_jobs) {
-            const uint32_t mod = a.jobs[j].s.mod_scheme;
-            const bool main_frame = k < a.live_off && (mod == 39 || mod == 40);
-            if (main_frame != (a.dec_phase == 1)) continue;
-        }
-        decode_frame(a, j, lds_soft_bytes, msg_bytes);
-        __syncthreads();
+        if (kn >= nl) break;
+        if (!next_staged) __syncthreads();
+        k = kn; cur = nxt; cls = cls_n; moff = moff_n; jn_v = j2_v;
+        staged = next_staged; half = next_staged ? half ^ 1u : 0u;
     }
 }
 
@@ -3096,10 +3194,28 @@
     in.vit_waves = a.vit_waves; in.enc_hint = a.enc_hint; in.payload_lds_pad = a.payload_lds_pad;
     in.have_qam_list = a.qam_list != nullptr; in.have_vit_scratch = a.vit_scratch != nullptr;
     in.scout = a.scout; in.no_fast = a.no_fast; in.payload_fr = a.payload_fr; in.payload_lean = a.payload_lean; in.payload_xb = a.payload_xb;
-    in.split_rest = a.split_rest; in.dec_phase = a.dec_phase;
+    in.split_rest = a.split_rest; in.dec_phase = a.dec_phase; in.dec_resident = a.dec_resident;
     return in;
 }
 bool sync_payload_splits(const SyncArgs &a) { return sync_payload_splits(sy_payload_inputs(a)); }
+
+hipError_t sync_decode_resident(const SyncArgs &a, uint32_t *lds, uint32_t *resident)
+{
+    const SyncPayloadPlan p = sync_payload_plan(sy_payload_inputs(a), SYNC_DECODE);
+    if (p.status != SYNC_LAUNCH || p.n < 1 || p.l[0].k != SK_DECODE || (uint32_t)p.l[0].lds == *lds) return hipSuccess;
+    int dev = 0, cus = 0, per_cu = 0;
+    hipError_t e = hipGetDevice(&dev);
+    if (e == hipSuccess) e = hipDeviceGetAttribute(&cus, hipDeviceAttributeMultiprocessorCount, dev);
+    if (e == hipSuccess) e = hipOccupancyMaxActiveBlocksPerMultiprocessor(&per_cu, decode_kernel, DK_T, p.l[0].lds);
+    hipFuncAttributes fa;
+    if (e == hipSuccess) e = hipFuncGetAttributes(&fa, reinterpret_cast<const void *>(decode_kernel));
+    if (e != hipSuccess) return e;
+    const int regs = (fa.numRegs + 7) & ~7, by_regs = regs > 0 ? 512 / regs : per_cu;
+    if (per_cu > by_regs) per_cu = by_regs;
+    *lds = (uint32_t)p.l[0].lds;
+    *resident = (per_cu > 0 && cus > 0) ? (uint32_t)per_cu * (uint32_t)cus : 0u;
+    return hipSuccess;
+}
 
 hipError_t sync_launch_payload(const SyncArgs &a0, SyncStage stage, hipStream_t st)
 {
diff --git a/liquid-usrp_amd/csrc/rx_plan.hpp b/liquid-usrp_amd/csrc/rx_plan.hpp
--- a/liquid-usrp_amd/csrc/rx_plan.hpp
+++ b/liquid-usrp_amd/csrc/rx_plan.hpp
@@ -43,6 +43,7 @@
     int acq_mode = 0;
     bool spec = false;
     int lean_build = 1;
+    uint32_t decoder_build = 0;
     int seg_walker = 1;
     bool scout = true;
     uint32_t round_lds_pad = 0;
@@ -100,6 +101,7 @@
     if (sb > 2) MCRX_REFUSE(MCRX_EINVAL, "scout_build out of range");
     if (sb == 1) r.lean_build = 0;
     if (sb == 2) r.seg_walker = 0;
+    r.decoder_build = cfg.decoder_build;
     if (dv.serial) r.pipelined = false;
     r.scout = dv.no_scout == nullptr;
     if (!r.scout || dv.no_spec) r.spec = false;
diff --git a/liquid-usrp_amd/csrc/sync_plan.hpp b/liquid-usrp_amd/csrc/sync_plan.hpp
--- a/liquid-usrp_amd/csrc/sync_plan.hpp
+++ b/liquid-usrp_amd/csrc/sync_plan.hpp
@@ -96,6 +96,7 @@
     uint32_t nch, max_jobs, frames_hint, grid_hint0, grid_hint2, vit_waves, enc_hint, payload_lds_pad;
     bool have_qam_list, have_vit_scratch;
     int scout, no_fast, payload_fr, payload_lean, payload_xb, split_rest, dec_phase;
+    uint32_t dec_resident;
 };
 struct SyncPayloadPlan {
     SyncStatus status = SYNC_NOTHING;
@@ -162,6 +163,7 @@
     else if (stage == SYNC_DECODE) {
         r.soft_lds = r.dec_lds_soft; r.msg_lds = (uint32_t)(((size_t)in.d.max_payload_len + 4 + 15) & ~(size_t)15);
         r.l[0].k = SK_DECODE; r.l[0].grid = ngrid; r.l[0].block = DK_T; r.l[0].lds = 2 * (size_t)r.soft_lds + r.msg_lds + 16;
+        if (in.dec_resident && r.l[0].grid > in.dec_resident) r.l[0].grid = in.dec_resident;
     } else if (stage == SYNC_DECODE_GENERAL) {
         unsigned ggrid = in.grid_hint2 ? (nj < 4096 ? nj : 4096) : SY_GEN_FLOOR;
         if (in.have_vit_scratch && ggrid > in.vit_waves) ggrid = in.vit_waves;
```

New measurement: 193,400 (median of 6 runs). About the same (+0.5%).
